# semihkacmaz/CoNFiLD

Measured on AMD Instinct MI355X. Metric: generated fields/sec (256-step sample + CNF decode), Case4 latent, 1/2/4/8 GPU, higher is better.
Workload: dtype f32

## Files before the change

confild_amd/_lib.py:

```python
from __future__ import annotations

import ctypes as C
import os
import threading

_HERE = os.path.dirname(os.path.abspath(__file__))
LIB_PATH = os.path.join(_HERE, "lib", "libconfild_hip.so")
if os.environ.get("CFD_LIB"):
    LIB_PATH = os.path.join(_HERE, "lib", os.path.basename(os.environ["CFD_LIB"]))

_lock = threading.Lock()
_lib = None

c_f32p = C.POINTER(C.c_float)
c_i64p = C.POINTER(C.c_int64)


class CfdError(RuntimeError):
    pass


class UNetCfg(C.Structure):
    _fields_ = [("image_size", C.c_int), ("in_channels", C.c_int), ("model_channels", C.c_int),
                ("out_channels", C.c_int), ("num_res_blocks", C.c_int), ("n_mult", C.c_int),
                ("channel_mult", C.c_int * 8), ("n_attn", C.c_int), ("attention_ds", C.c_int * 8),
                ("num_heads", C.c_int), ("num_head_channels", C.c_int)]


class SirenCfg(C.Structure):
    _fields_ = [("in_coord_features", C.c_int), ("in_latent_features", C.c_int), ("out_features", C.c_int),
                ("num_hidden_layers", C.c_int), ("hidden_features", C.c_int), ("w0", C.c_float)]


_SIGS = {
    "cfd_last_error": (C.c_char_p, []),
    "cfd_version": (C.c_char_p, []),
    "cfd_unet_create": (C.c_int, [C.POINTER(UNetCfg), C.c_int, C.POINTER(C.c_void_p)]),
    "cfd_unet_destroy": (None, [C.c_void_p]),
    "cfd_unet_num_params": (C.c_int, [C.c_void_p, C.POINTER(C.c_int)]),
    "cfd_unet_param_info": (C.c_int, [C.c_void_p, C.c_int, C.POINTER(C.c_char_p), C.POINTER(C.c_int),
                                      C.c_int64 * 4]),
    "cfd_unet_set_param": (C.c_int, [C.c_void_p, C.c_char_p, C.c_void_p, C.c_size_t]),
    "cfd_unet_set_time_freqs": (C.c_int, [C.c_void_p, C.c_void_p, C.c_int]),
    "cfd_unet_ready": (C.c_int, [C.c_void_p]),
    "cfd_unet_load_flat": (C.c_int, [C.c_void_p, C.c_void_p, C.c_size_t, C.c_void_p]),
    "cfd_unet_set_compute": (C.c_int, [C.c_void_p, C.c_int]),
    "cfd_unet_set_plan_batch": (C.c_int, [C.c_void_p, C.c_int]),
    "cfd_device_cu_count": (C.c_int, [C.c_int, C.POINTER(C.c_int)]),
    "cfd_stream_create_cu_range": (C.c_int, [C.c_int, C.c_int, C.c_int, C.POINTER(C.c_void_p)]),
    "cfd_stream_destroy": (C.c_int, [C.c_void_p]),
    "cfd_unet_check_finite": (C.c_int, [C.c_void_p, C.POINTER(C.c_int), C.c_void_p]),
    "cfd_upsample_conv": (C.c_int, [C.c_void_p, C.c_void_p, C.c_void_p, C.c_void_p, C.c_int, C.c_int, C.c_int,
                                    C.c_int, C.c_int, C.c_int, C.c_int, C.POINTER(C.c_int), C.c_void_p]),
    "cfd_unet_workspace_bytes": (C.c_int, [C.c_void_p, C.c_int, C.POINTER(C.c_size_t)]),
    "cfd_unet_forward": (C.c_int, [C.c_void_p, C.c_void_p, C.c_void_p, C.c_void_p, C.c_int, C.c_void_p,
                                   C.c_size_t, C.c_void_p]),
    "cfd_unet_tape_bytes": (C.c_int, [C.c_void_p, C.c_int, C.POINTER(C.c_size_t)]),
    "cfd_unet_vjp_workspace_bytes": (C.c_int, [C.c_void_p, C.c_int, C.POINTER(C.c_size_t)]),
    "cfd_unet_forward_tape": (C.c_int, [C.c_void_p, C.c_void_p, C.c_void_p, C.c_void_p, C.c_int, C.c_void_p,
                                        C.c_size_t, C.c_void_p, C.c_size_t, C.c_void_p]),
    "cfd_unet_input_vjp": (C.c_int, [C.c_void_p, C.c_void_p, C.c_void_p, C.c_int, C.c_void_p, C.c_size_t,
                                     C.c_void_p, C.c_size_t, C.c_void_p]),
    "cfd_unet_set_tape_mode": (C.c_int, [C.c_void_p, C.c_int]),
    "cfd_sched_create": (C.c_int, [C.c_void_p, C.c_int, C.c_int, C.POINTER(C.c_void_p)]),
    "cfd_sched_destroy": (None, [C.c_void_p]),
    "cfd_sched_step": (C.c_int, [C.c_void_p, C.c_int, C.c_int, C.c_void_p, C.c_void_p, C.c_void_p, C.c_void_p,
                                 C.c_uint64, C.c_uint64, C.c_uint64, C.c_void_p, C.c_void_p, C.c_int64, C.c_int,
                                 C.c_void_p]),
    "cfd_sched_step_known": (C.c_int, [C.c_void_p, C.c_int, C.c_int, C.c_void_p, C.c_void_p, C.c_void_p, C.c_void_p,
                                       C.c_uint64, C.c_uint64, C.c_uint64, C.c_void_p, C.c_void_p, C.c_int64,
                                       C.c_int, C.c_void_p, C.c_int64, C.c_void_p, C.c_int64, C.c_void_p,
                                       C.c_void_p, C.c_uint64, C.c_void_p]),
    "cfd_sched_step_jump": (C.c_int, [C.c_void_p, C.c_int, C.c_int, C.c_void_p, C.c_void_p, C.c_void_p, C.c_void_p,
                                      C.c_uint64, C.c_uint64, C.c_uint64, C.c_void_p, C.c_void_p, C.c_int64,
                                      C.c_int, C.c_void_p, C.c_int64, C.c_void_p, C.c_int64, C.c_void_p,
                                      C.c_void_p, C.c_uint64, C.c_float, C.c_float, C.c_void_p, C.c_uint64,
                                      C.c_void_p]),
    "cfd_sampler_set_jumps": (C.c_int, [C.c_void_p, C.c_void_p]),
    "cfd_sampler_set_known": (C.c_int, [C.c_void_p, C.c_void_p, C.c_int64, C.c_void_p, C.c_int64, C.c_void_p,
                                        C.c_void_p]),
    "cfd_sampler_captures": (C.c_int, [C.c_void_p, C.POINTER(C.c_uint64)]),
    "cfd_dps_latent_residual_workspace_bytes": (C.c_int, [C.c_int64, C.c_int, C.POINTER(C.c_size_t)]),
    "cfd_dps_latent_residual": (C.c_int, [C.c_void_p, C.c_int, C.c_void_p, C.c_void_p, C.c_void_p, C.c_void_p,
                                          C.c_int64, C.c_void_p, C.c_int64, C.c_void_p, C.c_void_p, C.c_void_p,
                                          C.c_int64, C.c_int, C.c_void_p, C.c_size_t, C.c_void_p]),
    "cfd_sampler_create": (C.c_int, [C.c_void_p, C.c_void_p, C.c_int, C.c_int, C.c_int, C.c_int64, C.c_int,
                                     C.c_void_p, C.c_void_p, C.c_int, C.c_int, C.POINTER(C.c_void_p)]),
    "cfd_sampler_destroy": (None, [C.c_void_p]),
    "cfd_sampler_run": (C.c_int, [C.c_void_p, C.c_void_p, C.c_void_p, C.c_int, C.c_int, C.c_uint64, C.c_uint64,
                                  C.c_void_p]),
    "cfd_randn": (C.c_int, [C.c_void_p, C.c_int64, C.c_uint64, C.c_uint64, C.c_uint64, C.c_void_p]),
    "cfd_sine_probe": (C.c_int, [C.c_void_p, C.c_void_p, C.c_int64, C.c_int, C.c_void_p]),
    "cfd_latent_denorm": (C.c_int, [C.c_void_p, C.c_void_p, C.c_int64, C.c_void_p, C.c_void_p, C.c_int64,
                                    C.c_void_p]),
    "cfd_dps_residual": (C.c_int, [C.c_void_p, C.c_int64, C.c_void_p, C.c_void_p, C.c_void_p, C.c_int64, C.c_int,
                                   C.c_void_p]),
    "cfd_dps_latent_grad": (C.c_int, [C.c_void_p, C.c_int, C.c_void_p, C.c_void_p, C.c_void_p, C.c_void_p,
                                      C.c_void_p, C.c_void_p, C.c_int64, C.c_void_p, C.c_void_p, C.c_int64, C.c_int,
                                      C.c_void_p]),
    "cfd_dps_update": (C.c_int, [C.c_void_p, C.c_void_p, C.c_void_p, C.c_float, C.c_void_p, C.c_int64,
                                 C.c_void_p]),
    "cfd_dps_update_known": (C.c_int, [C.c_void_p, C.c_void_p, C.c_void_p, C.c_float, C.c_void_p, C.c_void_p,
                                       C.c_int64, C.c_int, C.c_void_p, C.c_int64, C.c_void_p, C.c_int64, C.c_void_p,
                                       C.c_void_p, C.c_uint64, C.c_uint64, C.c_uint64, C.c_void_p]),
    "cfd_siren_create": (C.c_int, [C.POINTER(SirenCfg), C.c_int, C.POINTER(C.c_void_p)]),
    "cfd_siren_destroy": (None, [C.c_void_p]),
    "cfd_siren_num_params": (C.c_int, [C.c_void_p, C.POINTER(C.c_int)]),
    "cfd_siren_param_info": (C.c_int, [C.c_void_p, C.c_int, C.POINTER(C.c_char_p), C.POINTER(C.c_int),
                                       C.c_int64 * 4]),
    "cfd_siren_set_param": (C.c_int, [C.c_void_p, C.c_char_p, C.c_void_p, C.c_size_t]),
    "cfd_siren_ready": (C.c_int, [C.c_void_p]),
    "cfd_siren_workspace_bytes": (C.c_int, [C.c_void_p, C.c_int, C.POINTER(C.c_size_t)]),
    "cfd_siren_set_compute": (C.c_int, [C.c_void_p, C.c_int]),
    "cfd_siren_get_compute": (C.c_int, [C.c_void_p, C.POINTER(C.c_int)]),
    "cfd_siren_forward": (C.c_int, [C.c_void_p, C.c_void_p, C.c_int64, C.c_void_p, C.c_int, C.c_void_p,
                                    C.c_void_p, C.c_void_p, C.c_void_p, C.c_int64, C.c_void_p, C.c_void_p,
                                    C.c_size_t, C.c_void_p]),
    "cfd_siren_jacobian_workspace_bytes": (C.c_int, [C.c_void_p, C.c_int, C.POINTER(C.c_size_t)]),
    "cfd_siren_forward_jacobian": (C.c_int, [C.c_void_p, C.c_void_p, C.c_int64, C.c_void_p, C.c_int, C.c_void_p,
                                             C.c_void_p, C.c_void_p, C.c_void_p, C.c_int64, C.c_void_p, C.c_void_p,
                                             C.c_void_p, C.c_size_t, C.c_void_p]),
    "cfd_siren_forward_jacobian_split": (C.c_int, [C.c_void_p, C.c_void_p, C.c_int64, C.c_void_p, C.c_int,
                                                   C.c_void_p, C.c_void_p, C.c_void_p, C.c_void_p, C.c_int64,
                                                   C.c_void_p, C.c_void_p, C.c_void_p, C.c_size_t, C.c_void_p]),
    "cfd_siren_hessian_workspace_bytes": (C.c_int, [C.c_void_p, C.c_int, C.POINTER(C.c_size_t)]),
    "cfd_siren_forward_hessian": (C.c_int, [C.c_void_p, C.c_void_p, C.c_int64, C.c_void_p, C.c_int, C.c_void_p,
                                            C.c_void_p, C.c_void_p, C.c_void_p, C.c_int64, C.c_void_p, C.c_void_p,
                                            C.c_void_p, C.c_int, C.c_void_p, C.c_size_t, C.c_void_p]),
    "cfd_siren_forward_hessian_split": (C.c_int, [C.c_void_p, C.c_void_p, C.c_int64, C.c_void_p, C.c_int,
                                                  C.c_void_p, C.c_void_p, C.c_void_p, C.c_void_p, C.c_int64,
                                                  C.c_void_p, C.c_void_p, C.c_void_p, C.c_int, C.c_void_p,
                                                  C.c_size_t, C.c_void_p]),
    "cfd_siren_vjp_workspace_bytes": (C.c_int, [C.c_void_p, C.c_int64, C.c_int, C.POINTER(C.c_size_t)]),
    "cfd_siren_tape_forward": (C.c_int, [C.c_void_p, C.c_void_p, C.c_int64, C.c_void_p, C.c_int, C.c_void_p,
                                         C.c_void_p, C.c_void_p, C.c_void_p, C.c_int64, C.c_void_p, C.c_void_p,
                                         C.c_size_t, C.c_void_p]),
    "cfd_siren_tape_vjp": (C.c_int, [C.c_void_p, C.c_void_p, C.c_int64, C.c_int, C.c_void_p, C.c_void_p,
                                     C.c_int64, C.c_void_p, C.c_void_p, C.c_size_t, C.c_void_p]),
    "cfd_siren_jtape_workspace_bytes": (C.c_int, [C.c_void_p, C.c_int64, C.c_int, C.POINTER(C.c_size_t)]),
    "cfd_siren_jtape_forward": (C.c_int, [C.c_void_p, C.c_void_p, C.c_int64, C.c_void_p, C.c_int, C.c_void_p,
                                          C.c_void_p, C.c_void_p, C.c_void_p, C.c_int64, C.c_void_p, C.c_void_p,
                                          C.c_void_p, C.c_size_t, C.c_void_p]),
    "cfd_siren_jtape_vjp": (C.c_int, [C.c_void_p, C.c_void_p, C.c_void_p, C.c_int64, C.c_int, C.c_void_p,
                                      C.c_void_p, C.c_int64, C.c_void_p, C.c_void_p, C.c_size_t, C.c_void_p]),
    "cfd_dps_residual_linear": (C.c_int, [C.c_void_p, C.c_int, C.c_void_p, C.c_void_p, C.c_void_p, C.c_int,
                                          C.c_void_p, C.c_int, C.c_void_p, C.c_void_p, C.c_void_p, C.c_void_p,
                                          C.c_int64, C.c_int, C.c_int, C.c_int, C.c_int, C.c_int, C.c_void_p]),
    "cfd_siren_dense_plan": (C.c_int, [C.POINTER(SirenCfg), C.c_int64, C.c_int, C.c_size_t, C.c_int, C.c_int,
                                       C.POINTER(C.c_size_t), C.POINTER(C.c_int64), C.POINTER(C.c_int)]),
    "cfd_siren_dense_workspace_bytes": (C.c_int, [C.c_void_p, C.c_int64, C.c_int, C.c_size_t,
                                                  C.POINTER(C.c_size_t)]),
    "cfd_siren_dense_grad": (C.c_int, [C.c_void_p, C.c_void_p, C.c_int64, C.c_void_p, C.c_int, C.c_int, C.c_void_p,
                                       C.c_void_p, C.c_void_p, C.c_void_p, C.c_int64, C.c_void_p, C.c_int,
                                       C.c_void_p, C.c_int, C.c_void_p, C.c_void_p, C.c_void_p, C.c_size_t,
                                       C.c_size_t, C.c_void_p]),
    "cfd_siren_dense_set_form": (C.c_int, [C.c_void_p, C.c_int, C.c_int]),
    "cfd_siren_jdense_plan": (C.c_int, [C.POINTER(SirenCfg), C.c_int64, C.c_int, C.c_int, C.c_size_t,
                                        C.POINTER(C.c_size_t), C.POINTER(C.c_int64), C.POINTER(C.c_int)]),
    "cfd_siren_jdense_workspace_bytes": (C.c_int, [C.c_void_p, C.c_int64, C.c_int, C.c_int, C.c_size_t,
                                                   C.POINTER(C.c_size_t)]),
    "cfd_siren_jdense_grad": (C.c_int, [C.c_void_p, C.c_void_p, C.c_int64, C.c_void_p, C.c_int, C.c_int, C.c_void_p,
                                        C.c_void_p, C.c_void_p, C.c_void_p, C.c_int64, C.c_void_p, C.c_int,
                                        C.c_void_p, C.c_int, C.c_int, C.c_void_p, C.c_int, C.c_void_p, C.c_int,
                                        C.c_void_p, C.c_void_p, C.c_void_p, C.c_size_t, C.c_size_t, C.c_void_p]),
    "cfd_siren_train_workspace_bytes": (C.c_int, [C.c_void_p, C.c_int64, C.c_int, C.POINTER(C.c_size_t)]),
    "cfd_siren_train_grad": (C.c_int, [C.c_void_p, C.c_void_p, C.c_int64, C.c_void_p, C.c_void_p, C.c_int,
                                       C.c_void_p, C.c_float, C.c_void_p, C.c_void_p, C.c_void_p, C.c_void_p,
                                       C.c_size_t, C.c_void_p]),
    "cfd_unet_param_grad_workspace_bytes": (C.c_int, [C.c_void_p, C.c_int, C.POINTER(C.c_size_t)]),
    "cfd_unet_param_grad": (C.c_int, [C.c_void_p, C.c_void_p, C.c_void_p, C.c_int, C.c_void_p, C.c_size_t,
                                      C.c_void_p, C.c_void_p, C.c_size_t, C.c_void_p]),
    "cfd_eps_mse": (C.c_int, [C.c_void_p, C.c_void_p, C.c_void_p, C.c_void_p, C.c_int64, C.c_int, C.c_float,
                              C.c_void_p, C.c_void_p]),
    "cfd_ema_update": (C.c_int, [C.c_void_p, C.c_void_p, C.c_int64, C.c_double, C.c_void_p]),
    "cfd_q_sample": (C.c_int, [C.c_void_p, C.c_void_p, C.c_void_p, C.c_void_p, C.c_void_p, C.c_int64, C.c_int,
                               C.c_void_p]),
    "cfd_adam_step": (C.c_int, [C.c_void_p, C.c_void_p, C.c_void_p, C.c_void_p, C.c_int64, C.c_double, C.c_double,
                                C.c_double, C.c_double, C.c_double, C.c_int64, C.c_void_p]),
}

EXPORTS = tuple(_SIGS)


def load(path: str = LIB_PATH):
    global _lib
    with _lock:
        if _lib is not None:
            return _lib
        if not os.path.exists(path):
            raise CfdError(f"{path} is missing: build it with `python -c 'import __graft_entry__ as g; g.build()'` "
                           "(or `make -C confild_amd/csrc`)")
        lib = C.CDLL(path)
        for name, (res, args) in _SIGS.items():
            if os.environ.get("CFD_LIB") and not hasattr(lib, name):
                continue
            fn = getattr(lib, name)
            fn.restype = res
            fn.argtypes = args
        _lib = lib
        return lib


def lib():
    import torch
    if not torch.cuda.is_available():
        raise CfdError("confild_amd needs an AMD GPU (MI355X); no HIP device is visible and there is no CPU path")
# ... 20 lines not shown
```

confild_amd/csrc/conv_x.hip:

```cpp
#include <algorithm>
#include <type_traits>

#include "k1h_lds.hpp"
#include "unet_kernels.hpp"

namespace cfd {

typedef float f16v __attribute__((ext_vector_type(16)));
typedef float f2 __attribute__((ext_vector_type(2)));
typedef _Float16 h2 __attribute__((ext_vector_type(2)));
typedef unsigned u4 __attribute__((ext_vector_type(4)));

__device__ __forceinline__ int xswz(int row, int chunk) { return row * 64 + ((chunk ^ ((row >> 2) & 3)) << 4); }

__device__ __forceinline__ void split4_mix_x(const f4& x, uint2& hi, uint2& lo) {
    hi.x = __builtin_bit_cast(unsigned, __builtin_convertvector((f2){x[0], x[1]}, h2));
    hi.y = __builtin_bit_cast(unsigned, __builtin_convertvector((f2){x[2], x[3]}, h2));
    asm("v_fma_mixlo_f16 %0, %1, 1.0, -%2 op_sel_hi:[0,0,1]" : "=&v"(lo.x) : "v"(x[0]), "v"(hi.x));
    asm("v_fma_mixhi_f16 %0, %1, 1.0, -%2 op_sel:[0,0,1] op_sel_hi:[0,0,1]" : "+v"(lo.x) : "v"(x[1]), "v"(hi.x));
    asm("v_fma_mixlo_f16 %0, %1, 1.0, -%2 op_sel_hi:[0,0,1]" : "=&v"(lo.y) : "v"(x[2]), "v"(hi.y));
    asm("v_fma_mixhi_f16 %0, %1, 1.0, -%2 op_sel:[0,0,1] op_sel_hi:[0,0,1]" : "+v"(lo.y) : "v"(x[3]), "v"(hi.y));
}

__device__ __forceinline__ float phase_scale(const ConvArgs& a, int ph) {
// ... 126 lines not shown
#pragma unroll
        for (int it = 0; it < AIT; ++it) {
            const int off = xswz(a_row[it], kq >> 1) + (kq & 1) * 8;
            uint2 hv, lv;
            split4_mix_x(ra[set][it], hv, lv);
            *(uint2*)(base + off) = hv;
            *(uint2*)(base + ABYTES + off) = lv;
        }
#pragma unroll
        for (int it = 0; it < BIT; ++it) {
            const int off = xswz(b_row[it], kq >> 1) + (kq & 1) * 8;
            *(uint2*)(base + 2 * ABYTES + off) = rbh[set][it];
            *(uint2*)(base + 2 * ABYTES + BBYTES + off) = rbl[set][it];
        }
    };

    f16v acc[TM][TN];
#pragma unroll
    for (int i = 0; i < TM; ++i)
#pragma unroll
        for (int j = 0; j < TN; ++j)
#pragma unroll
            for (int e = 0; e < 16; ++e) acc[i][j][e] = 0.f;

    const int l32 = lane & 31, hsel = lane >> 5;
    const int arow0 = wm * WTM + l32, brow0 = wn * WTN + l32;
    auto kstep = [&](int kt, int cur, int lset, int sset) __attribute__((always_inline)) {
            const bool more = kt + 1 < kt1;
            if (kt + PF < kt1) load_tile(kt + PF, lset);
            const char* base = lds + cur * STAGE;
#pragma unroll
            for (int s = 0; s < 2; ++s) {
                const int ch = 2 * s + hsel;
                h8v fah[TM], fal[TM], fbh[TN], fbl[TN];
#pragma unroll
                for (int i = 0; i < TM; ++i) {
                    const int off = xswz(arow0 + 32 * i, ch);
                    fah[i] = *(const h8v*)(base + off);
                    fal[i] = *(const h8v*)(base + ABYTES + off);
                }
#pragma unroll
                for (int j = 0; j < TN; ++j) {
                    const int off = xswz(brow0 + 32 * j, ch);
                    fbh[j] = *(const h8v*)(base + 2 * ABYTES + off);
                    fbl[j] = *(const h8v*)(base + 2 * ABYTES + BBYTES + off);
                }
#pragma unroll
                for (int i = 0; i < TM; ++i)
#pragma unroll
                    for (int j = 0; j < TN; ++j) {
                        acc[i][j] = __builtin_amdgcn_mfma_f32_32x32x16_f16(fal[i], fbh[j], acc[i][j], 0, 0, 0);
                        acc[i][j] = __builtin_amdgcn_mfma_f32_32x32x16_f16(fah[i], fbl[j], acc[i][j], 0, 0, 0);
                        acc[i][j] = __builtin_amdgcn_mfma_f32_32x32x16_f16(fah[i], fbh[j], acc[i][j], 0, 0, 0);
                    }
            }
            if (more) store_tile(cur ^ 1, sset);
            __syncthreads();
    };
    if (kt0 < kt1) {
        load_tile(kt0, 0);
        if constexpr (PF == 2) {
            if (kt0 + 1 < kt1) load_tile(kt0 + 1, 1);
        }
        store_tile(0, 0);
        __syncthreads();
        CFD_STAMP(a.stamps, 2, a.seq, 2);
        if constexpr (PF == 1) {
            int cur = 0;
            for (int kt = kt0; kt < kt1; ++kt) {
                kstep(kt, cur, 0, 0);
                cur ^= 1;
            }
        } else {
            for (int kt = kt0; kt < kt1; kt += 2) {
                kstep(kt, 0, 0, 1);
                if (kt + 1 < kt1) kstep(kt + 1, 1, 1, 0);
            }
        }
    }

    CFD_STAMP(a.stamps, 2, a.seq, 3);
#pragma unroll
    for (int i = 0; i < TM; ++i)
#pragma unroll
        for (int j = 0; j < TN; ++j) acc[i][j] *= PH ? phase_scale(a, ph) : a.acc_scale;
    const int n_base = n0 + wn * WTN + l32;
    const int m_base = m0 + wm * WTM + 4 * hsel;
    auto orow = [&](int mm, int& bb) __attribute__((always_inline)) {
        bb = mm / HWm;
        if constexpr (!PH) return mm;
        const int rem = mm - bb * HWm, y = rem / Wm, x = rem - y * Wm;
        return (bb * a.Hout + 2 * y + py) * a.Wout + 2 * x + px;
    };
    if (gridDim.z > 1) {
        float* part = a.part + (int64_t)bz * a.M * a.Cout;
#pragma unroll
        for (int i = 0; i < TM; ++i)
#pragma unroll
            for (int e = 0; e < 16; ++e) {
                const int mm = m_base + 32 * i + 8 * (e >> 2) + (e & 3);
                if (mm >= Mm) continue;
                int bb;
                const int m = orow(mm, bb);
#pragma unroll
                for (int j = 0; j < TN; ++j) {
                    const int n = n_base + 32 * j;
                    if (n < a.Cout) part[(int64_t)m * a.Cout + n] = acc[i][j][e];
                }
            }
#ifdef CFD_STAMPS
        __builtin_amdgcn_s_waitcnt(0);
#endif
        CFD_STAMP(a.stamps, 2, a.seq, 4);
        return;
    }
#pragma unroll
    for (int i = 0; i < TM; ++i)
#pragma unroll
        for (int e = 0; e < 16; ++e) {
            const int mm = m_base + 32 * i + 8 * (e >> 2) + (e & 3);
            if (mm >= Mm) continue;
            int bb;
            const int m = orow(mm, bb);
#pragma unroll
            for (int j = 0; j < TN; ++j) {
                const int n = n_base + 32 * j;
                if (n >= a.Cout) continue;
                float v = a.bias ? acc[i][j][e] + a.bias[n] : acc[i][j][e];
                if (a.emb) v = v + a.emb[(int64_t)bb * a.emb_stride + n];
                if (a.res) v = a.res[(int64_t)m * a.Cout + n] + v;
                a.out[(int64_t)m * a.Cout + n] = v;
            }
        }
}

template <int V>
using IC = std::integral_constant<int, V>;

struct Tile3 {
    int x, y, z;
};
__device__ __forceinline__ Tile3 xcd_tile_v(int order) {
    if (!order) return Tile3{(int)blockIdx.x, (int)blockIdx.y, (int)blockIdx.z};
    const unsigned gx = gridDim.x, gy = gridDim.y, gz = gridDim.z;
    const unsigned T = gx * gy * gz, L = blockIdx.x + gx * (blockIdx.y + gy * blockIdx.z);
    const unsigned q = T >> 3, r = T & 7, x = L & 7, sl = L >> 3;
    const unsigned Lp = x < r ? x * (q + 1) + sl : r * (q + 1) + (x - r) * q + sl;
    const bool o2 = order == 2;
    const unsigned d1 = o2 ? gx : gz, d2 = o2 ? gz : gy;
    const unsigned lo = Lp % d1, rest = Lp / d1, mid = rest % d2, hi = rest / d2;
    return o2 ? Tile3{(int)lo, (int)hi, (int)mid} : Tile3{(int)hi, (int)mid, (int)lo};
}

template <int BM, int TW, int BN, bool PH>
__device__ __forceinline__ void conv_h16_body(const ConvArgs& a) {
    constexpr int WGN = BN / 64, WGM = BM / 64, NTG = 64 * WGM * WGN;
    static_assert(BN == 64 || BN == 128, "K1h: 64 or 128 output channels per workgroup");
    static_assert(TW == 16 || TW == 32 || TW == 64, "K1h: a 16-pixel fragment block lies in one tile row");
    constexpr int HWD = TW + 2;
    constexpr int TR = BM / TW, NPX = k1h_npx(BM, TW), NPXD = k1h_npx_staged(BM, TW);
    constexpr int HPLANE = NPX * 64;
    constexpr int HIT = (NPXD * 8 + NTG - 1) / NTG;
    constexpr int NTAP = PH ? 4 : 9, TXN = PH ? 2 : 3;
    constexpr int BPLANE = BN * 64, BSTAGE = 2 * BPLANE;
    constexpr int BIT = BN * 4 / NTG;
    constexpr int GBYTES = 2 * HPLANE + 2 * BSTAGE;
    static_assert(BM % TW == 0 && BIT == 1 && BM % 64 == 0, "tile");
    static_assert(k1h_a_imm(TW, 3, 2) + HPLANE + 3 * 64 + 64 < 65536, "fragment offsets are instruction offsets");
    __shared__ __attribute__((aligned(16))) char lds[GBYTES];

    CFD_STAMP(a.stamps, 3, a.seq, 0);
    const int tid = threadIdx.x, lane = tid & 63;
    const int wave = __builtin_amdgcn_readfirstlane(tid >> 6);
    const int wm = wave / WGN, wn = wave % WGN;
    const int gt = tid;
    char* const halo = lds;
    char* const ring = halo + 2 * HPLANE;
    const Tile3 wg = xcd_tile_v(a.xcd);
    int bx = wg.x;
    const int by = wg.y, bz = wg.z;
    const int ph = PH ? bx & 3 : 0, py = ph >> 1, px = ph & 1;
    if constexpr (PH) bx >>= 2;
    const int n0 = by * BN;
    const int W = PH ? a.Win : a.Wout, Hh = PH ? a.Hin : a.Hout, HWo = Hh * W;
    const int tps = HWo / BM, tpr = W / TW;
    const int bimg = bx / tps, tl = bx - bimg * tps;
    const int y0 = (tl / tpr) * TR, x0 = (tl - (tl / tpr) * tpr) * TW;
    const int64_t mrow0 = PH ? ((int64_t)bimg * a.Hout + 2 * y0 + py) * a.Wout + 2 * x0 + px
                             : (int64_t)bimg * HWo + (int64_t)y0 * W + x0;
    CFD_DASSERT(mrow0 + (int64_t)(PH ? 2 : 1) * ((int64_t)(TR - 1) * a.Wout + TW - 1) < a.M && HWo % BM == 0 &&
                W % TW == 0);

    const int srows = __builtin_amdgcn_readfirstlane(a.Hin * a.Win * (a.M / (a.Hout * a.Wout)));
    const __amdgpu_buffer_rsrc_t rs1 = __builtin_amdgcn_make_buffer_rsrc((void*)a.src1, 0, srows * a.C1 * 4, 0x00020000);
    const __amdgpu_buffer_rsrc_t rs2 = __builtin_amdgcn_make_buffer_rsrc(
        (void*)(a.src2 ? (const void*)a.src2 : (const void*)a.src1), 0, a.src2 ? srows * a.C2 * 4 : 0, 0x00020000);
    const int wbytes = a.Cout * NTAP * a.Ctot * 2;
    const char* const wh0 = PH ? (const char*)a.wph + (int64_t)ph * wbytes : (const char*)a.wbf;
    const char* const wl0 = PH ? (const char*)a.wpl + (int64_t)ph * wbytes : (const char*)a.wlo;
    const __amdgpu_buffer_rsrc_t rwh = __builtin_amdgcn_make_buffer_rsrc((void*)wh0, 0, wbytes, 0x00020000);
    const __amdgpu_buffer_rsrc_t rwl = __builtin_amdgcn_make_buffer_rsrc((void*)wl0, 0, wbytes, 0x00020000);

    const int kq = gt & 7;
    int hpix[HIT], hst[HIT];
#pragma unroll
    for (int it = 0; it < HIT; ++it) {
        const int hp = (gt + it * NTG) >> 3;
        int pix = -1;
        hst[it] = 0;
        if (hp < NPXD) {
            const int hr = hp / HWD, hc = hp - hr * HWD;
            const int iy = y0 - 1 + hr + py, ix = x0 - 1 + hc + px;
            if ((!PH || (hc < TW + 1 && hr < TR + 1)) && iy >= 0 && iy < Hh && ix >= 0 && ix < W)
                pix = a.up && !PH ? (bimg * a.Hin + (iy >> 1)) * a.Win + (ix >> 1) : (bimg * a.Hin + iy) * a.Win + ix;
            hst[it] = k1h_stage_off(TW, hp, kq);
            CFD_DASSERT(hst[it] >= 0 && hst[it] + 8 <= HPLANE);
        }
        CFD_DASSERT(pix < srows);
        hpix[it] = pix;
    }
    const int bq = gt & 3;
    const int nrow = n0 + (gt >> 2);
    const unsigned bvoff = nrow < a.Cout ? (unsigned)((nrow * NTAP * a.Ctot + 8 * bq) * 2) : 0x80000000u;
    const int wst = k1h_wstage_off(gt >> 2, bq);

    const int nch = a.Ctot / 32;
    const int per = (nch + gridDim.z - 1) / gridDim.z;
    const int c0 = bz * per, cend = min(nch, c0 + per);
    const int nrounds = max(cend - c0, 0);

    f4 rh[HIT];
    u4 wx_h, wx_l, wy_h, wy_l;
    auto load_halo = [&](int c) __attribute__((always_inline)) {
        const int cb = 32 * c;
        const bool second = cb >= a.C1;
        const unsigned csrc = 4u * (unsigned)(second ? a.C2 + 0 : a.C1 + 0);
        const unsigned cofs = c < nch ? 4u * ((second ? cb - a.C1 : cb) + 4 * kq) : 0x80000000u;
        if (second) {
#pragma unroll
            for (int it = 0; it < HIT; ++it) {
                const unsigned off = hpix[it] >= 0 ? __umul24((unsigned)hpix[it], csrc) + cofs : 0x80000000u;
                rh[it] = __builtin_bit_cast(f4, __builtin_amdgcn_raw_buffer_load_b128(rs2, off, 0, 0));
            }
        } else {
#pragma unroll
            for (int it = 0; it < HIT; ++it) {
                const unsigned off = hpix[it] >= 0 ? __umul24((unsigned)hpix[it], csrc) + cofs : 0x80000000u;
                rh[it] = __builtin_bit_cast(f4, __builtin_amdgcn_raw_buffer_load_b128(rs1, off, 0, 0));
            }
        }
    };
    auto store_halo = [&]() __attribute__((always_inline)) {
#pragma unroll
        for (int it = 0; it < HIT; ++it) {
            if (gt + it * NTG < NPXD * 8) {
                uint2 hv, lv;
                split4_mix_x(rh[it], hv, lv);
                *(uint2*)(halo + hst[it]) = hv;
                *(uint2*)(halo + HPLANE + hst[it]) = lv;
            }
        }
    };
    auto load_w = [&](int c, int t, u4& rbh, u4& rbl) __attribute__((always_inline)) {
        const int soff = (t * a.Ctot + 32 * min(c, cend - 1)) * 2;
        rbh = __builtin_bit_cast(u4, __builtin_amdgcn_raw_buffer_load_b128(rwh, bvoff, soff, 0));
        rbl = __builtin_bit_cast(u4, __builtin_amdgcn_raw_buffer_load_b128(rwl, bvoff, soff, 0));
    };
    auto store_w = [&](int stage, const u4& rbh, const u4& rbl) __attribute__((always_inline)) {
        char* base = ring + stage * BSTAGE + wst;
        *(u4*)base = rbh;
        *(u4*)(base + BPLANE) = rbl;
    };

    f4 acc[4][4];
#pragma unroll
    for (int i = 0; i < 4; ++i)
#pragma unroll
        for (int j = 0; j < 4; ++j) acc[i][j] = f4{0.f, 0.f, 0.f, 0.f};

    const int li = lane & 15, g = lane >> 4;
    const char* abase[TXN];
#pragma unroll
    for (int tx = 0; tx < TXN; ++tx) abase[tx] = halo + k1h_a_base(TW, wm, li, g, tx);
    const char* const bbase = ring + k1h_b_base(wn, li, g);
    CFD_DASSERT(k1h_a_base(TW, wm, li, g, TXN - 1) + k1h_a_imm(TW, 3, PH ? 1 : 2) + 16 <= HPLANE);

    auto step = [&](int r, auto tc, auto qc, u4& ldh, u4& ldl, const u4& sth, const u4& stl)
        __attribute__((always_inline)) {
        constexpr int T = decltype(tc)::value, Q = decltype(qc)::value;
        constexpr int ty = PH ? T >> 1 : T / 3, tx = PH ? T & 1 : T - 3 * ty;
        const int c = c0 + r;
        load_w(T + 2 < NTAP ? c : c + 1, (T + 2) % NTAP, ldh, ldl);
        if constexpr (T == 0) load_halo(r + 1 < nrounds ? c + 1 : nch);
        const char* const ap = abase[tx];
        const char* const bp = bbase + Q * BSTAGE;
        h8v fbh[4], fbl[4];
#pragma unroll
        for (int j = 0; j < 4; ++j) {
            fbh[j] = *(const h8v*)(bp + k1h_b_imm(j));
            fbl[j] = *(const h8v*)(bp + BPLANE + k1h_b_imm(j));
        }
#pragma unroll
        for (int i = 0; i < 4; ++i) {
            const h8v fah = *(const h8v*)(ap + k1h_a_imm(TW, i, ty));
            const h8v fal = *(const h8v*)(ap + HPLANE + k1h_a_imm(TW, i, ty));
#pragma unroll
            for (int j = 0; j < 4; ++j) acc[i][j] = __builtin_amdgcn_mfma_f32_16x16x32_f16(fal, fbh[j], acc[i][j], 0, 0, 0);
#pragma unroll
            for (int j = 0; j < 4; ++j) acc[i][j] = __builtin_amdgcn_mfma_f32_16x16x32_f16(fah, fbl[j], acc[i][j], 0, 0, 0);
#pragma unroll
            for (int j = 0; j < 4; ++j) acc[i][j] = __builtin_amdgcn_mfma_f32_16x16x32_f16(fah, fbh[j], acc[i][j], 0, 0, 0);
        }
        store_w(Q ^ 1, sth, stl);
        __syncthreads();
        if constexpr (T == NTAP - 1) {
            store_halo();
            __syncthreads();
        }
        __builtin_amdgcn_sched_barrier(0);
    };
    auto round = [&](int r, auto q0c) __attribute__((always_inline)) {
        constexpr int Q0 = decltype(q0c)::value;
        auto tap = [&](auto tc) __attribute__((always_inline)) {
            constexpr int Q = (Q0 + decltype(tc)::value) & 1;
            if constexpr (Q == 0) step(r, tc, IC<0>{}, wx_h, wx_l, wy_h, wy_l);
            else step(r, tc, IC<1>{}, wy_h, wy_l, wx_h, wx_l);
        };
        tap(IC<0>{}), tap(IC<1>{}), tap(IC<2>{}), tap(IC<3>{});
        if constexpr (!PH) tap(IC<4>{}), tap(IC<5>{}), tap(IC<6>{}), tap(IC<7>{}), tap(IC<8>{});
    };

    if (nrounds > 0) {
        load_w(c0, 0, wx_h, wx_l);
        load_w(c0, 1, wy_h, wy_l);
        load_halo(c0);
        store_w(0, wx_h, wx_l);
        store_halo();
        __syncthreads();
        CFD_STAMP(a.stamps, 3, a.seq, 2);
        if constexpr (NTAP & 1) {
            int r = 0;
            for (; r + 2 <= nrounds; r += 2) {
                round(r, IC<0>{});
                round(r + 1, IC<1>{});
            }
            if (r < nrounds) round(r, IC<0>{});
        } else {
            for (int r = 0; r < nrounds; ++r) round(r, IC<0>{});
        }
    }

    CFD_STAMP(a.stamps, 3, a.seq, 3);
    const float scl = PH ? phase_scale(a, ph) : a.acc_scale;
#pragma unroll
    for (int i = 0; i < 4; ++i)
#pragma unroll
        for (int j = 0; j < 4; ++j) acc[i][j] *= scl;
    auto pix_of = [&](int p) __attribute__((always_inline)) {
        if constexpr (PH) return mrow0 + (int64_t)(p / TW) * (2 * a.Wout) + 2 * (p % TW);
        else return mrow0 + (int64_t)(p / TW) * W + (p % TW);
    };
    if (a.ldsepi) {
        static_assert(64 * BN * 4 <= GBYTES, "epilogue stage fits the LDS");
        float* stg = (float*)lds;
        const bool split = gridDim.z > 1;
        float* dstb = split ? a.part + (int64_t)bz * a.M * a.Cout : a.out;
        constexpr int Q = BN / 4;
        __syncthreads();
        for (int r = 0; r < WGM; ++r) {
            if (wm == r) {
#pragma unroll
                for (int i = 0; i < 4; ++i)
#pragma unroll
                    for (int j = 0; j < 4; ++j)
#pragma unroll
                        for (int e = 0; e < 4; ++e)
                            stg[k1h_epi(BN, 16 * i + 4 * g + e, wn * 64 + 16 * j + li)] = acc[i][j][e];
            }
            __syncthreads();
            for (int q = tid; q < 64 * Q; q += NTG) {
                const int p = q / Q, c = (q - p * Q) * 4;
                const int n = n0 + c;
                if (n < a.Cout) {
                    const int64_t m = pix_of(r * 64 + p);
                    f4 v = *(const f4*)(stg + k1h_epi(BN, p, c));
                    if (!split) {
                        if (a.bias) v = v + *(const f4*)(a.bias + n);
                        if (a.emb) v = v + *(const f4*)(a.emb + (int64_t)bimg * a.emb_stride + n);
                        if (a.res) v = *(const f4*)(a.res + m * a.Cout + n) + v;
                    }
                    *(f4*)(dstb + m * a.Cout + n) = v;
                }
            }
            __syncthreads();
        }
#ifdef CFD_STAMPS
        __builtin_amdgcn_s_waitcnt(0);
#endif
        CFD_STAMP(a.stamps, 3, a.seq, 4);
        return;
    }
    const int n_base = n0 + wn * 64 + li;
    const int p_base = wm * 64 + 4 * g;
    if (gridDim.z > 1) {
        float* part = a.part + (int64_t)bz * a.M * a.Cout;
#pragma unroll
        for (int i = 0; i < 4; ++i)
#pragma unroll
            for (int e = 0; e < 4; ++e) {
                const int64_t m = pix_of(p_base + 16 * i + e);
#pragma unroll
                for (int j = 0; j < 4; ++j) {
                    const int n = n_base + 16 * j;
                    if (n < a.Cout) part[m * a.Cout + n] = acc[i][j][e];
                }
            }
#ifdef CFD_STAMPS
        __builtin_amdgcn_s_waitcnt(0);
#endif
        CFD_STAMP(a.stamps, 3, a.seq, 4);
        return;
    }
#pragma unroll
    for (int i = 0; i < 4; ++i)
#pragma unroll
        for (int e = 0; e < 4; ++e) {
            const int64_t m = pix_of(p_base + 16 * i + e);
#pragma unroll
            for (int j = 0; j < 4; ++j) {
                const int n = n_base + 16 * j;
                if (n >= a.Cout) continue;
                float v = a.bias ? acc[i][j][e] + a.bias[n] : acc[i][j][e];
                if (a.emb) v = v + a.emb[(int64_t)bimg * a.emb_stride + n];
                if (a.res) v = a.res[m * a.Cout + n] + v;
                a.out[m * a.Cout + n] = v;
            }
        }
#ifdef CFD_STAMPS
    __builtin_amdgcn_s_waitcnt(0);
#endif
    CFD_STAMP(a.stamps, 3, a.seq, 4);
}

template <int BM, int TW, bool BF = false, bool SB = false, int BN = 128, bool PH = false, int SHAPE = 32>
__global__ __launch_bounds__(BM * (BN / 64), 1) void conv_h_kernel(ConvArgs a) {
    static_assert(SHAPE == 32 || (SHAPE == 16 && !BF && !SB), "K1h: 16x16x32 is the split-f16 form's");
    if constexpr (SHAPE == 16) {
        conv_h16_body<BM, TW, BN, PH>(a);
        return;
    }
    static_assert(!SB || BF, "a bf16 source needs the bf16 kernel");
    static_assert(!PH || !BF, "the phase form is split-f16 only");
    constexpr unsigned SES = SB ? 2u : 4u;
    constexpr int WGN = BN / 64, WGM = BM / 64, NTG = 64 * WGM * WGN;
    static_assert(BN == 64 || BN == 128, "K1h: 64 or 128 output channels per workgroup");
    constexpr int PL = BF ? 1 : 2;
    constexpr int HW2 = TW < 32 ? (TW + 2 + 3) / 4 * 4 : TW + 2;
    constexpr int TR = BM / TW, NPX = (TR + 2) * HW2;
    auto hswz = [](int px, int hr, int chunk) __attribute__((always_inline)) {
        if constexpr (TW == 16) return px * 64 + ((chunk ^ (((px >> 2) + 3 * hr) & 3)) << 4);
        else return xswz(px, chunk);
    };
    constexpr int HPLANE = NPX * 64;
    constexpr int HIT = (NPX * 8 + NTG - 1) / NTG;
    constexpr int NTAP = PH ? 4 : 9;
    constexpr int TG = BF ? 3 : 1, SPR = NTAP / TG;
    constexpr int BPLANE = BN * 64, BSTAGE = PL * BPLANE * TG;
    constexpr int BIT = BN * 4 / NTG;
    constexpr int GBYTES = PL * HPLANE + 2 * BSTAGE;
    static_assert(BM % TW == 0 && BIT >= 1, "tile");
    __shared__ __attribute__((aligned(16))) char lds[GBYTES];

    CFD_STAMP(a.stamps, 3, a.seq, 0);
    const int tid = threadIdx.x, lane = tid & 63;
    const int wave = __builtin_amdgcn_readfirstlane(tid >> 6);
    const int wm = wave / WGN, wn = wave % WGN;
    const int gt = tid;
    char* const halo = lds;
    char* const ring = halo + PL * HPLANE;
    int bx, by, bz;
    xcd_tile(a.xcd, bx, by, bz);
    const int ph = PH ? bx & 3 : 0, py = ph >> 1, px = ph & 1;
    if constexpr (PH) bx >>= 2;
    const int n0 = by * BN;
    const int W = PH ? a.Win : a.Wout, Hh = PH ? a.Hin : a.Hout, HWo = Hh * W;
    const int tps = HWo / BM, tpr = W / TW;
    const int bimg = bx / tps, tl = bx - bimg * tps;
    const int y0 = (tl / tpr) * TR, x0 = (tl - (tl / tpr) * tpr) * TW;
    const int64_t mrow0 = PH ? ((int64_t)bimg * a.Hout + 2 * y0 + py) * a.Wout + 2 * x0 + px
                             : (int64_t)bimg * HWo + (int64_t)y0 * W + x0;
    CFD_DASSERT(mrow0 + (int64_t)(PH ? 2 : 1) * ((int64_t)(TR - 1) * a.Wout + TW - 1) < a.M && HWo % BM == 0 &&
                W % TW == 0);

    const int srows = __builtin_amdgcn_readfirstlane(a.Hin * a.Win * (a.M / (a.Hout * a.Wout)));
    const __amdgpu_buffer_rsrc_t rs1 = __builtin_amdgcn_make_buffer_rsrc((void*)a.src1, 0, srows * a.C1 * SES, 0x00020000);
    const __amdgpu_buffer_rsrc_t rs2 = __builtin_amdgcn_make_buffer_rsrc(
        (void*)(a.src2 ? (const void*)a.src2 : (const void*)a.src1), 0, a.src2 ? srows * a.C2 * SES : 0, 0x00020000);
    const int wbytes = a.Cout * NTAP * a.Ctot * 2;
    const char* const wh0 = PH ? (const char*)a.wph + (int64_t)ph * wbytes : (const char*)a.wbf;
    const char* const wl0 = PH ? (const char*)a.wpl + (int64_t)ph * wbytes : (const char*)a.wlo;
    const __amdgpu_buffer_rsrc_t rwh = __builtin_amdgcn_make_buffer_rsrc((void*)wh0, 0, wbytes, 0x00020000);
    const __amdgpu_buffer_rsrc_t rwl = __builtin_amdgcn_make_buffer_rsrc((void*)wl0, 0, wbytes, 0x00020000);

    const int kq = gt & 7;
    int hpix[HIT];
#pragma unroll
    for (int it = 0; it < HIT; ++it) {
        const int hp = (gt + it * NTG) >> 3;
        int pix = -1;
        if (hp < NPX) {
            const int hr = hp / HW2, hc = hp - hr * HW2;
            const int iy = y0 - 1 + hr + py, ix = x0 - 1 + hc + px;
            if (hc < TW + (PH ? 1 : 2) && (!PH || hr < TR + 1) && iy >= 0 && iy < Hh && ix >= 0 && ix < W)
                pix = a.up && !PH ? (bimg * a.Hin + (iy >> 1)) * a.Win + (ix >> 1) : (bimg * a.Hin + iy) * a.Win + ix;
        }
        CFD_DASSERT(pix < srows);
        hpix[it] = pix;
    }
    const int bq = gt & 3;
    unsigned bvoff[BIT];
#pragma unroll
    for (int it = 0; it < BIT; ++it) {
        const int n = n0 + (gt >> 2) + it * (NTG / 4);
        bvoff[it] = n < a.Cout ? (unsigned)((n * NTAP * a.Ctot + 8 * bq) * 2) : 0x80000000u;
    }

    const int nch = a.Ctot / 32;
    const int per = (nch + gridDim.z - 1) / gridDim.z;
    const int c0 = bz * per, cend = min(nch, c0 + per);
    const int nrounds = max(cend - c0, 0);
    auto chunk_of = [&](int r) __attribute__((always_inline)) { return c0 + r; };

    typedef typename std::conditional<SB, uint2, f4>::type HT;
    HT rh[HIT];
    constexpr int BW = BIT * TG;
    u4 wx_h[BW], wx_l[BW], wy_h[BW], wy_l[BW];
    auto load_halo = [&](int c) __attribute__((always_inline)) {
        const int cb = 32 * c;
        const bool second = cb >= a.C1;
        const unsigned csrc = SES * (unsigned)(second ? a.C2 + 0 : a.C1 + 0);
        const unsigned cofs = SES * ((second ? cb - a.C1 : cb) + 4 * kq);
        if (second) {
#pragma unroll
            for (int it = 0; it < HIT; ++it) {
                const unsigned off = hpix[it] >= 0 ? __umul24((unsigned)hpix[it], csrc) + cofs : 0x80000000u;
                if constexpr (SB)
                    rh[it] = __builtin_bit_cast(uint2, __builtin_amdgcn_raw_buffer_load_b64(rs2, off, 0, 0));
// ... 28 lines not shown
                    *(uint2*)(halo + HPLANE + off) = lv;
                }
            }
        }
    };
    auto load_w = [&](int s, u4 (&rbh)[BW], u4 (&rbl)[BW]) __attribute__((always_inline)) {
        const int r = s / SPR, c = chunk_of(r);
        if (c >= cend) return;
#pragma unroll
        for (int u = 0; u < TG; ++u) {
            const int soff = (((s - SPR * r) * TG + u) * a.Ctot + 32 * c) * 2;
#pragma unroll
            for (int it = 0; it < BIT; ++it) {
                rbh[u * BIT + it] = __builtin_bit_cast(u4, __builtin_amdgcn_raw_buffer_load_b128(rwh, bvoff[it], soff, 0));
                if constexpr (!BF)
                    rbl[u * BIT + it] = __builtin_bit_cast(u4, __builtin_amdgcn_raw_buffer_load_b128(rwl, bvoff[it], soff, 0));
            }
        }
    };
    auto store_w = [&](int stage, const u4 (&rbh)[BW], const u4 (&rbl)[BW]) __attribute__((always_inline)) {
#pragma unroll
        for (int u = 0; u < TG; ++u) {
            char* base = ring + stage * BSTAGE + u * PL * BPLANE;
#pragma unroll
            for (int it = 0; it < BIT; ++it) {
                const int off = xswz((gt >> 2) + it * (NTG / 4), bq);
                *(u4*)(base + off) = rbh[u * BIT + it];
                if constexpr (!BF) *(u4*)(base + BPLANE + off) = rbl[u * BIT + it];
            }
        }
    };

    f16v acc[2][2];
#pragma unroll
    for (int i = 0; i < 2; ++i)
#pragma unroll
        for (int j = 0; j < 2; ++j)
#pragma unroll
            for (int e = 0; e < 16; ++e) acc[i][j][e] = 0.f;

    const int l32 = lane & 31, hsel = lane >> 5;
    int hb[2], hrb[2];
#pragma unroll
    for (int i = 0; i < 2; ++i) {
        const int p = wm * 64 + 32 * i + l32;
        hb[i] = (p / TW) * HW2 + (p % TW);
        hrb[i] = p / TW;
    }
    const int brow0 = wn * 64 + l32;
    const int nsteps = nrounds * SPR;

    auto step = [&](int s, u4 (&ldh)[BW], u4 (&ldl)[BW], const u4 (&sth)[BW], const u4 (&stl)[BW])
        __attribute__((always_inline)) {
        const int r = s / SPR, t = s - SPR * r;
        const int c = chunk_of(r);
        if (s + 2 < nsteps) load_w(s + 2, ldh, ldl);
        if (t == 0 && chunk_of(r + 1) < cend) load_halo(chunk_of(r + 1));
        if (c < cend) {
            const char* wb = ring + (s & 1) * BSTAGE;
            if constexpr (BF) {
                const int ty = t;
#pragma unroll
                for (int u = 0; u < TG; ++u) {
                    const int tofs = ty * HW2 + u;
                    const char* wbu = wb + u * BPLANE;
#pragma unroll
                    for (int s2 = 0; s2 < 2; ++s2) {
                        const int ch = 2 * s2 + hsel;
                        bf16x8 fa[2], fb[2];
#pragma unroll
                        for (int i = 0; i < 2; ++i) fa[i] = *(const bf16x8*)(halo + hswz(hb[i] + tofs, hrb[i] + ty, ch));
#pragma unroll
                        for (int jj = 0; jj < 2; ++jj) fb[jj] = *(const bf16x8*)(wbu + xswz(brow0 + 32 * jj, ch));
#pragma unroll
                        for (int i = 0; i < 2; ++i)
#pragma unroll
                            for (int jj = 0; jj < 2; ++jj)
                                acc[i][jj] = __builtin_amdgcn_mfma_f32_32x32x16_bf16(fa[i], fb[jj], acc[i][jj], 0, 0, 0);
                    }
                }
            } else {
            const int ty = PH ? t >> 1 : t / 3;
            const int tofs = ty * HW2 + (PH ? t & 1 : t - 3 * ty);
#pragma unroll
            for (int s2 = 0; s2 < 2; ++s2) {
                const int ch = 2 * s2 + hsel;
                h8v fah[2], fal[2], fbh[2], fbl[2];
#pragma unroll
                for (int i = 0; i < 2; ++i) {
                    CFD_DASSERT(hb[i] + tofs < NPX);
                    const int off = hswz(hb[i] + tofs, hrb[i] + ty, ch);
                    fah[i] = *(const h8v*)(halo + off);
                    fal[i] = *(const h8v*)(halo + HPLANE + off);
                }
#pragma unroll
                for (int jj = 0; jj < 2; ++jj) {
                    const int off = xswz(brow0 + 32 * jj, ch);
                    fbh[jj] = *(const h8v*)(wb + off);
                    fbl[jj] = *(const h8v*)(wb + BPLANE + off);
                }
#pragma unroll
                for (int i = 0; i < 2; ++i)
#pragma unroll
                    for (int jj = 0; jj < 2; ++jj) {
                        acc[i][jj] = __builtin_amdgcn_mfma_f32_32x32x16_f16(fal[i], fbh[jj], acc[i][jj], 0, 0, 0);
                        acc[i][jj] = __builtin_amdgcn_mfma_f32_32x32x16_f16(fah[i], fbl[jj], acc[i][jj], 0, 0, 0);
                        acc[i][jj] = __builtin_amdgcn_mfma_f32_32x32x16_f16(fah[i], fbh[jj], acc[i][jj], 0, 0, 0);
                    }
            }
            }
        }
        if (s + 1 < nsteps && chunk_of((s + 1) / SPR) < cend) store_w((s + 1) & 1, sth, stl);
        __syncthreads();
        if (t == SPR - 1 && s + 1 < nsteps) {
            if (chunk_of(r + 1) < cend) store_halo();
            __syncthreads();
        }
    };

    if (nsteps > 0) {
        load_w(0, wx_h, wx_l);
        if (nsteps > 1) load_w(1, wy_h, wy_l);
        load_halo(chunk_of(0));
        store_w(0, wx_h, wx_l);
        store_halo();
        __syncthreads();
        CFD_STAMP(a.stamps, 3, a.seq, 2);
        for (int s = 0; s < nsteps; s += 2) {
            step(s, wx_h, wx_l, wy_h, wy_l);
            if (s + 1 < nsteps) step(s + 1, wy_h, wy_l, wx_h, wx_l);
        }
    }

    CFD_STAMP(a.stamps, 3, a.seq, 3);
    if constexpr (!BF) {
#pragma unroll
        for (int i = 0; i < 2; ++i)
#pragma unroll
            for (int j = 0; j < 2; ++j) acc[i][j] *= PH ? phase_scale(a, ph) : a.acc_scale;
    }
    const int n_base = n0 + wn * 64 + l32;
    const int p_base = wm * 64 + 4 * hsel;
    auto pix_of = [&](int p) __attribute__((always_inline)) {
        if constexpr (PH) return mrow0 + (int64_t)(p / TW) * (2 * a.Wout) + 2 * (p % TW);
        else return mrow0 + (int64_t)(p / TW) * W + (p % TW);
    };
    {
        if (a.ldsepi) {
            static_assert(64 * BN * 4 <= (int)sizeof(lds), "epilogue stage fits the LDS");
            float* stg = (float*)lds;
            const bool split = gridDim.z > 1;
            float* dstb = split ? a.part + (int64_t)bz * a.M * a.Cout : a.out;
            constexpr int Q = BN / 4;
            __syncthreads();
            for (int r = 0; r < WGM; ++r) {
                if (wm == r) {
#pragma unroll
                    for (int i = 0; i < 2; ++i)
#pragma unroll
                        for (int e = 0; e < 16; ++e)
#pragma unroll
                            for (int j = 0; j < 2; ++j)
                                stg[(32 * i + 8 * (e >> 2) + (e & 3) + 4 * hsel) * BN + wn * 64 + 32 * j + l32] =
                                    acc[i][j][e];
                }
                __syncthreads();
                for (int q = tid; q < 64 * Q; q += NTG) {
                    const int p = q / Q, c = (q - p * Q) * 4;
                    const int n = n0 + c;
                    if (n < a.Cout) {
                        const int64_t m = pix_of(r * 64 + p);
                        f4 v = *(const f4*)(stg + p * BN + c);
                        if (!split) {
                            if (a.bias) v = v + *(const f4*)(a.bias + n);
                            if (a.emb) v = v + *(const f4*)(a.emb + (int64_t)bimg * a.emb_stride + n);
                            if (a.res) v = *(const f4*)(a.res + m * a.Cout + n) + v;
                        }
                        *(f4*)(dstb + m * a.Cout + n) = v;
                    }
                }
                __syncthreads();
            }
#ifdef CFD_STAMPS
            __builtin_amdgcn_s_waitcnt(0);
#endif
            CFD_STAMP(a.stamps, 3, a.seq, 4);
            return;
        }
    }
    if (gridDim.z > 1) {
        float* part = a.part + (int64_t)bz * a.M * a.Cout;
#pragma unroll
        for (int i = 0; i < 2; ++i)
#pragma unroll
            for (int e = 0; e < 16; ++e) {
                const int64_t m = pix_of(p_base + 32 * i + 8 * (e >> 2) + (e & 3));
#pragma unroll
                for (int j = 0; j < 2; ++j) {
                    const int n = n_base + 32 * j;
                    if (n < a.Cout) part[(int64_t)m * a.Cout + n] = acc[i][j][e];
                }
            }
#ifdef CFD_STAMPS
        __builtin_amdgcn_s_waitcnt(0);
#endif
        CFD_STAMP(a.stamps, 3, a.seq, 4);
        return;
    }
#pragma unroll
    for (int i = 0; i < 2; ++i)
#pragma unroll
        for (int e = 0; e < 16; ++e) {
            const int64_t m = pix_of(p_base + 32 * i + 8 * (e >> 2) + (e & 3));
#pragma unroll
            for (int j = 0; j < 2; ++j) {
                const int n = n_base + 32 * j;
                if (n >= a.Cout) continue;
                float v = a.bias ? acc[i][j][e] + a.bias[n] : acc[i][j][e];
                if (a.emb) v = v + a.emb[(int64_t)bimg * a.emb_stride + n];
                if (a.res) v = a.res[(int64_t)m * a.Cout + n] + v;
                a.out[(int64_t)m * a.Cout + n] = v;
            }
        }
#ifdef CFD_STAMPS
    __builtin_amdgcn_s_waitcnt(0);
#endif
    CFD_STAMP(a.stamps, 3, a.seq, 4);
}

int conv_h_tw(const ConvArgs& a) {
    const bool geo = !a.tmode && a.ks == 3 && a.stride == 1 && a.pad == 1 && a.C1 % 32 == 0 && a.C2 % 32 == 0 &&
                     (a.up ? a.Hout == 2 * a.Hin && a.Wout == 2 * a.Win : a.Hout == a.Hin && a.Wout == a.Win) &&
                     a.M % (a.Hout * a.Wout) == 0;
    if (!geo) return 0;
    for (int tw = 64; tw >= 16; tw >>= 1)
        if (a.Wout % tw == 0 && a.Hout % (256 / tw) == 0) return tw;
    return 0;
}

int conv_hp_tw(const ConvArgs& a) {
    const bool geo = !a.tmode && a.up && a.ks == 3 && a.stride == 1 && a.pad == 1 && a.C1 % 32 == 0 &&
                     a.C2 % 32 == 0 && a.Hout == 2 * a.Hin && a.Wout == 2 * a.Win && a.M % (a.Hout * a.Wout) == 0;
    if (!geo) return 0;
    for (int tw = 64; tw >= 16; tw >>= 1)
        if (a.Win % tw == 0 && a.Hin % (256 / tw) == 0) return tw;
    return 0;
}

int k1h_shape(int tw, int bn, bool phase, bool adjoint) {
    (void)tw, (void)bn, (void)phase;
#ifdef CFD_K1H_MFMA32
    (void)adjoint;
    return 32;
#else
    return adjoint ? 32 : 16;
#endif
}

template <int BN, bool PH, int SHAPE>
static void launch_h_(const ConvArgs& a, int tw, dim3 g, hipStream_t st) {
    const dim3 blk(256 * (BN / 64));
    if (tw == 64) hipLaunchKernelGGL((conv_h_kernel<256, 64, false, false, BN, PH, SHAPE>), g, blk, 0, st, a);
    else if (tw == 32) hipLaunchKernelGGL((conv_h_kernel<256, 32, false, false, BN, PH, SHAPE>), g, blk, 0, st, a);
    else hipLaunchKernelGGL((conv_h_kernel<256, 16, false, false, BN, PH, SHAPE>), g, blk, 0, st, a);
}
template <int BN, bool PH>
static void launch_h(const ConvArgs& a, int tw, int shape, dim3 g, hipStream_t st) {
    if (shape == 16) launch_h_<BN, PH, 16>(a, tw, g, st);
    else launch_h_<BN, PH, 32>(a, tw, g, st);
}

int launch_conv_x(const ConvArgs& a, int variant, int splits, hipStream_t st, bool adjoint) {
    CFD_REQUIRE(a.wbf && !a.tmode, CFD_ESTATE, "conv_x: split-f16 or bf16 forward only");
    CFD_REQUIRE(a.Ctot % 32 == 0 && a.C1 % 4 == 0 && a.C2 % 4 == 0, CFD_ESHAPE, "conv_x needs channels % 32 == 0");
    CFD_REQUIRE(splits == 1 || a.part, CFD_ESTATE, "split-K needs a partial buffer");
    {
        const int64_t srows = (int64_t)a.Hin * a.Win * (a.M / (a.Hout * a.Wout));
        CFD_REQUIRE(srows < (1 << 24) && srows * std::max(a.C1, a.C2) * 4 < (1ll << 31) &&
                        (int64_t)a.Cout * a.K * 2 < (1ll << 31) && a.ks * a.ks <= 9,
                    CFD_ESHAPE, "conv_x: operands beyond 2 GiB");
    }
    auto grid = [&](int bm, int bn) __attribute__((always_inline)) {
        return dim3((unsigned)ceil_div(a.M, bm), (unsigned)ceil_div(a.Cout, bn), splits);
    };
    if (variant == 22) {
        const int tw = conv_h_tw(a);
        CFD_REQUIRE(tw > 0 && !a.wlo, CFD_ESHAPE, "conv_h bf16: 3x3 stride-1 with a 16/32/64-divisible width");
        const dim3 g = grid(256, 128);
        if (a.src_bf16) {
            if (tw == 64) hipLaunchKernelGGL((conv_h_kernel<256, 64, true, true>), g, dim3(512), 0, st, a);
            else if (tw == 32) hipLaunchKernelGGL((conv_h_kernel<256, 32, true, true>), g, dim3(512), 0, st, a);
            else hipLaunchKernelGGL((conv_h_kernel<256, 16, true, true>), g, dim3(512), 0, st, a);
        } else {
            if (tw == 64) hipLaunchKernelGGL((conv_h_kernel<256, 64, true>), g, dim3(512), 0, st, a);
            else if (tw == 32) hipLaunchKernelGGL((conv_h_kernel<256, 32, true>), g, dim3(512), 0, st, a);
            else hipLaunchKernelGGL((conv_h_kernel<256, 16, true>), g, dim3(512), 0, st, a);
        }
        check_launch("conv_h_kernel");
        return splits;
    }
    CFD_REQUIRE(!a.src_bf16, CFD_ESTATE, "internal: a bf16 convolution source needs the K1hb kernel");
    if (variant == 20 || variant == 32 || variant == 33) {
        const int tw = conv_h_tw(a);
        CFD_REQUIRE(tw > 0 && a.wlo, CFD_ESHAPE, "conv_h: split-f16 3x3 stride-1 with a 16/32/64-divisible width");
        static const int smalln = smalln_below();
        const dim3 g = grid(256, 128);
        const bool n64 = (int64_t)g.x * g.y * g.z < smalln && a.Cout % 64 == 0;
        const int shape = variant == 20 ? k1h_shape(tw, n64 ? 64 : 128, false, adjoint) : variant == 32 ? 32 : 16;
        if (n64) {
            launch_h<64, false>(a, tw, shape, grid(256, 64), st);
            check_launch("conv_h_kernel");
            return splits;
        }
        launch_h<128, false>(a, tw, shape, g, st);
        check_launch("conv_h_kernel");
        return splits;
    }
    CFD_REQUIRE(a.wlo, CFD_ESTATE, "internal: K1x runs split-f16 operands only");
    if ((variant >= 24 && variant <= 26) || variant == 34 || variant == 35) {
        CFD_REQUIRE(a.wph && a.wpl && a.up && a.ks == 3 && a.stride == 1 && a.pad == 1 && a.Hout == 2 * a.Hin &&
                        a.Wout == 2 * a.Win,
                    CFD_ESTATE, "internal: the phase form needs an Upsample convolution and its phase packs");
        if (variant == 24 || variant == 34 || variant == 35) {
            const int tw = conv_hp_tw(a);
            CFD_REQUIRE(tw > 0, CFD_ESHAPE, "conv_h phase form: a 16/32/64-divisible low-resolution width");
            const dim3 g = grid(256, 128);
            launch_h<128, true>(a, tw, variant == 24 ? k1h_shape(tw, 128, true, adjoint) : variant == 34 ? 32 : 16, g, st);
            check_launch("conv_h_kernel (phase)");
            return splits;
        }
        const int bm = variant == 26 ? 256 : 128;
        const dim3 g(4u * (unsigned)ceil_div(a.M / 4, bm), (unsigned)ceil_div(a.Cout, 128), splits);
        if (variant == 26) hipLaunchKernelGGL((conv_x_kernel<256, 128, 4, 2, 1, true>), g, dim3(512), 0, st, a);
        else hipLaunchKernelGGL((conv_x_kernel<128, 128, 2, 2, 1, true>), g, dim3(256), 0, st, a);
        check_launch("conv_x_kernel (phase)");
        return splits;
    }
    switch (variant) {
        case 1: hipLaunchKernelGGL((conv_x_kernel<128, 128, 2, 2>), grid(128, 128), dim3(256), 0, st, a); break;
        case 2: hipLaunchKernelGGL((conv_x_kernel<256, 128, 4, 2>), grid(256, 128), dim3(512), 0, st, a); break;
        default: CFD_REQUIRE(false, CFD_EARG, "conv_x variant");
    }
    check_launch("conv_x_kernel");
    return splits;
}

}
```

confild_amd/csrc/unet.hip:

```cpp
#include <algorithm>
#include <cstring>
#include <cmath>
#include <functional>
#include <map>
#include <string>
#include <vector>

#include "sampler.hpp"
#include "unet_kernels.hpp"
#include "unet_train.hpp"

namespace cfd {

enum class Pack { Raw, Conv3, Conv1, EmbW, EmbB };

struct UParam {
    std::string key;
    std::vector<int64_t> shape;
    Pack pack = Pack::Raw;
    size_t offset = 0;
    size_t count = 0;
    int emb_row = 0;
    bool set = false;
    int tpack = 0;
// ... 130 lines not shown
    const auto& c = h->cfg;
    const int mc = c.model_channels;
    h->tdim = 4 * mc;
    add_param(h, "time_embed.0.weight", {h->tdim, mc}, Pack::Raw);
    add_param(h, "time_embed.0.bias", {h->tdim}, Pack::Raw);
    add_param(h, "time_embed.2.weight", {h->tdim, h->tdim}, Pack::Raw);
    add_param(h, "time_embed.2.bias", {h->tdim}, Pack::Raw);
    int ch = c.channel_mult[0] * mc;
    add_conv(h, "input_blocks.0.0", c.in_channels, ch, 3);
    h->steps.push_back({cfd::Step::In, 0, "input_blocks.0.0", c.in_channels, ch});
    h->steps.push_back({cfd::Step::Push});
    std::vector<int> chans{ch};
    int ds = 1, idx = 1;
    for (int level = 0; level < c.n_mult; ++level) {
        for (int r = 0; r < c.num_res_blocks; ++r) {
            const int cout = c.channel_mult[level] * mc;
            const std::string pre = "input_blocks." + std::to_string(idx);
            int ri = add_res(h, pre + ".0", ch, cout);
            h->steps.push_back({cfd::Step::Res, ri});
            ch = cout;
            if (has_attn(h, ds)) h->steps.push_back({cfd::Step::Attn, add_attn(h, pre + ".1", ch)});
            h->steps.push_back({cfd::Step::Push});
            chans.push_back(ch);
            ++idx;
        }
        if (level != c.n_mult - 1) {
            const std::string pre = "input_blocks." + std::to_string(idx) + ".0.op";
            add_conv(h, pre, ch, ch, 3);
            h->steps.push_back({cfd::Step::Down, 0, pre, ch, ch});
            h->steps.push_back({cfd::Step::Push});
            chans.push_back(ch);
            ds *= 2;
            ++idx;
        }
    }
    h->steps.push_back({cfd::Step::Res, add_res(h, "middle_block.0", ch, ch)});
    h->steps.push_back({cfd::Step::Attn, add_attn(h, "middle_block.1", ch)});
    h->steps.push_back({cfd::Step::Res, add_res(h, "middle_block.2", ch, ch)});
    idx = 0;
    for (int level = c.n_mult - 1; level >= 0; --level) {
        for (int i = 0; i < c.num_res_blocks + 1; ++i) {
            const int ich = chans.back();
            chans.pop_back();
            const int cout = mc * c.channel_mult[level];
            const std::string pre = "output_blocks." + std::to_string(idx);
            h->steps.push_back({cfd::Step::Cat});
            h->steps.push_back({cfd::Step::Res, add_res(h, pre + ".0", ch + ich, cout)});
            ch = cout;
            int j = 1;
            if (has_attn(h, ds)) {
                h->steps.push_back({cfd::Step::Attn, add_attn(h, pre + ".1", ch)});
                j = 2;
            }
            if (level && i == c.num_res_blocks) {
                const std::string up = pre + "." + std::to_string(j) + ".conv";
                add_conv(h, up, ch, ch, 3, false, true);
                h->steps.push_back({cfd::Step::Up, 0, up, ch, ch});
                ds /= 2;
            }
            ++idx;
        }
    }
    add_norm(h, "out.0", ch);
    add_conv(h, "out.2", c.channel_mult[0] * mc, c.out_channels, 3);
    h->steps.push_back({cfd::Step::Out, 0, "out", ch, c.out_channels});
    size_t off = 0;
    for (auto& p : h->params) {
        if (p.pack == Pack::EmbW || p.pack == Pack::EmbB) continue;
        p.offset = off;
        off += (p.count + 3) & ~size_t(3);
    }
    h->arena_floats = off;
    size_t toff = 0;
    for (auto& p : h->params) {
        if (!p.tpack) continue;
        p.toffset = toff;
        toff += ((p.tpack == 2 ? p.count / 9 * 16 : p.count) + 3) & ~size_t(3);
    }
    h->arena_t_floats = toff;
    size_t poff = 0;
    for (auto& p : h->params) {
        if (p.tpack != 2 || p.shape[0] < cfd::kPhaseMinCout) continue;
        p.phase = true;
        p.poffset = poff;
        poff += (p.count / 9 * 16 + 7) & ~size_t(7);
    }
    h->arena_p_elems = poff;
}

const void* PB(const cfd_unet* h, const std::string& key) {
    if (h->compute == CFD_COMPUTE_F32) return nullptr;
    auto it = h->index.find(key);
    CFD_REQUIRE(it != h->index.end(), CFD_EKEY, "internal: missing param " + key);
    return (h->compute == CFD_COMPUTE_BF16 ? h->arena_bf : h->arena_hi) + h->params[it->second].offset;
}

const void* PL(const cfd_unet* h, const std::string& key, float* inv) {
    *inv = 1.f;
    if (h->compute != CFD_COMPUTE_SPLIT_F16) return nullptr;
    auto it = h->index.find(key);
    CFD_REQUIRE(it != h->index.end(), CFD_EKEY, "internal: missing param " + key);
    *inv = h->params[it->second].split_inv;
    return h->arena_lo + h->params[it->second].offset;
}

uint16_t to_bf16(float f) {
    uint32_t u;
    std::memcpy(&u, &f, 4);
    if ((u & 0x7fffffffu) > 0x7f800000u) return (uint16_t)((u >> 16) | 0x40u);
    return (uint16_t)((u + 0x7fffu + ((u >> 16) & 1u)) >> 16);
}

void PTS(const cfd_unet* h, const std::string& key, cfd::ConvArgs* a) {
    if (h->compute != CFD_COMPUTE_SPLIT_F16) return;
    auto it = h->index.find(key);
    CFD_REQUIRE(it != h->index.end() && h->params[it->second].tpack, CFD_EKEY, "internal: missing conv " + key);
    const auto& p = h->params[it->second];
    a->wbf = h->arena_thi + p.toffset;
    a->wlo = h->arena_tlo + p.toffset;
    a->acc_scale = p.tsplit_inv;
}

void PP(const cfd_unet* h, const std::string& key, cfd::ConvArgs* a) {
    if (h->compute != CFD_COMPUTE_SPLIT_F16) return;
    auto it = h->index.find(key);
    CFD_REQUIRE(it != h->index.end(), CFD_EKEY, "internal: missing param " + key);
    const auto& p = h->params[it->second];
    if (!p.phase) return;
    a->wph = h->arena_phi + p.poffset;
    a->wpl = h->arena_plo + p.poffset;
    for (int ph = 0; ph < 4; ++ph) a->ph_scale[ph] = p.psplit_inv[ph];
}

const float* PT(const cfd_unet* h, const std::string& key) {
    auto it = h->index.find(key);
    CFD_REQUIRE(it != h->index.end() && h->params[it->second].tpack, CFD_EKEY, "internal: missing conv " + key);
    return h->arena_t + h->params[it->second].toffset;
}

const float* P(const cfd_unet* h, const std::string& key) {
    auto it = h->index.find(key);
    CFD_REQUIRE(it != h->index.end(), CFD_EKEY, "internal: missing param " + key);
    return h->arena + h->params[it->second].offset;
}

struct Act {
    const float* a = nullptr;
    int Ca = 0;
    const float* b = nullptr;
    int Cb = 0;
    int H = 0, W = 0;
    int C() const { return Ca + Cb; }
    bool bf16 = false;
};

struct Workspace {
    char* base;
    size_t off = 0;
    bool dry;
    float* take(size_t nfloats) {
        off = (off + 255) & ~size_t(255);
        float* p = dry ? nullptr : (float*)(base + off);
        off += nfloats * sizeof(float);
        return p;
    }
};

struct Rec {
    Act in;
    const float* h1 = nullptr;
    float *ss1 = nullptr, *st1 = nullptr;
    float *ss2 = nullptr, *st2 = nullptr;
    float *qkv = nullptr, *o = nullptr, *lse = nullptr;
    const float *act1 = nullptr, *act2 = nullptr;
    unsigned *amx1 = nullptr, *amx2 = nullptr;
    int skip_hs = -1;
    int push_hs = -1;
};

struct Tape {
    Workspace* tws;
    std::vector<Rec>* recs;
    bool keep_gnout = false;
    float* temb = nullptr;
    float* th1 = nullptr;
    float* emb = nullptr;
};

struct Sizes {
    size_t max_act = 0, max_qkv = 0, max_cat = 0, max_att = 0;
    size_t max_kvf = 0;
    size_t max_abw = 0;
    size_t max_apart = 0;
    std::vector<size_t> hs;
};

int plan_batch(const cfd_unet* h);

Sizes sizes(const cfd_unet* h) {
    const auto& c = h->cfg;
    const int mc = c.model_channels, S = c.image_size;
    Sizes z;
    int ch = c.channel_mult[0] * mc, hw = S, cmax = 0;
    z.max_act = (size_t)hw * hw * ch;
    z.hs.push_back((size_t)hw * hw * ch);
    for (int l = 0; l < c.n_mult; ++l) cmax = std::max(cmax, c.channel_mult[l] * mc);
    for (int l = 0; l < c.n_mult; ++l) {
        const int co = c.channel_mult[l] * mc;
        z.max_act = std::max(z.max_act, (size_t)hw * hw * std::max(co, ch));
        z.max_qkv = std::max(z.max_qkv, (size_t)hw * hw * 3 * co);
        z.max_cat = std::max(z.max_cat, (size_t)hw * hw * (co + cmax));
        z.max_att = std::max(z.max_att, (size_t)hw * hw * co);
        z.max_kvf = std::max(z.max_kvf, cfd::attention_split_floats(hw * hw, co));
        if (has_attn(h, 1 << l) || l == c.n_mult - 1) {
            z.max_abw = std::max(z.max_abw, cfd::attention_bwd_split_floats(hw * hw, co));
            const int heads = c.num_head_channels == -1 ? c.num_heads : co / c.num_head_channels;
            z.max_apart = std::max(z.max_apart, cfd::attention_part_floats(hw * hw, co, co / heads, plan_batch(h)));
        }
        for (int r = 0; r < c.num_res_blocks; ++r) z.hs.push_back((size_t)hw * hw * co);
        ch = co;
        if (l != c.n_mult - 1) {
            hw /= 2;
            z.hs.push_back((size_t)hw * hw * ch);
        }
    }
    z.max_cat = std::max(z.max_cat, z.max_act);
    return z;
}

constexpr size_t kSplitPer8 = size_t(16) << 20;
int plan_batch(const cfd_unet* h) { return h->plan_b > 0 ? h->plan_b : 8; }
size_t split_cap(const cfd_unet* h, int B) {
    const int pb = plan_batch(h);
    return kSplitPer8 * (size_t)std::max(1, (B + pb - 1) / pb);
}

cfd::ConvPlan plan_checked(const cfd_unet* h, const cfd::ConvArgs& a0, size_t slab_floats) {
    cfd::ConvArgs a = a0;
    a.plan_b = plan_batch(h);
    const cfd::ConvPlan p = cfd::plan_conv(a, kSplitPer8);
    CFD_REQUIRE(p.splits == 1 || (size_t)p.splits * a.M * a.Cout <= slab_floats, CFD_ESTATE,
                "internal: split-K slab too small");
    return p;
}

void run(const cfd_unet* h, const float* x, const int64_t* t, float* eps, int B, Workspace& ws, hipStream_t st,
         Tape* tape = nullptr, bool launch_req = true) {
    const auto& c = h->cfg;
    const int mc = c.model_channels, S = c.image_size;
    const Sizes z = sizes(h);
    const bool launch = launch_req && !ws.dry && !(tape && tape->tws->dry);
    const size_t kSplitCap = split_cap(h, B);
    float* temb = tape ? tape->tws->take((size_t)B * mc) : ws.take((size_t)B * mc);
    float* h1 = tape ? tape->tws->take((size_t)B * h->tdim) : ws.take((size_t)B * h->tdim);
    float* emb = tape ? tape->tws->take((size_t)B * h->tdim) : ws.take((size_t)B * h->tdim);
    if (tape) {
        tape->temb = temb;
        tape->th1 = h1;
        tape->emb = emb;
    }
    float* embo = ws.take((size_t)B * h->emb_total);
    double* gnpart = (double*)ws.take((size_t)B * cfd::kGnMaxChunks * 32 * 2 * 2);
    float* gnss = ws.take((size_t)B * 1024 * 2);
    float* nbuf = ws.take((size_t)B * z.max_cat);
    float* splitk = ws.take(kSplitCap);
    float* kvws = ws.take((size_t)B * z.max_kvf);
    float* apart = z.max_apart ? ws.take((size_t)B * z.max_apart) : nullptr;
    float* pool[3];
    for (auto& p : pool) p = ws.take((size_t)B * z.max_act);
    float* tmp = ws.take((size_t)B * z.max_act);
    float* skipb = ws.take((size_t)B * z.max_act);
    float* qkv = tape ? nullptr : ws.take((size_t)B * z.max_qkv);
    float* abuf = tape ? nullptr : ws.take((size_t)B * z.max_act);
    std::vector<float*> hsbuf;
    for (size_t n : z.hs) hsbuf.push_back(tape ? tape->tws->take((size_t)B * n) : ws.take((size_t)B * n));
    constexpr int kGnSlots = 256;
    unsigned* gslots = tape ? (unsigned*)tape->tws->take(kGnSlots) : nullptr;
    int ngs = 0;
    if (ws.dry && !tape) return;
    auto keep = [&](size_t nfloats) -> float* { return tape->tws->take(nfloats); };
    if (tape && tape->keep_gnout && launch) CFD_HIP(hipMemsetAsync(gslots, 0, sizeof(unsigned) * kGnSlots, st));
    std::vector<Rec>* recs = tape ? tape->recs : nullptr;
    if (recs) recs->assign(h->steps.size(), Rec{});

    auto pick = [&](const float* busy1, const float* busy2) -> float* {
        if (!launch && (ws.dry || !busy1)) return pool[0];
        for (auto p : pool)
            if (p != busy1 && p != busy2) return p;
        throw cfd::Error{CFD_ESTATE, "internal: buffer pool exhausted"};
    };

    if (launch) {
        cfd::launch_temb(t, h->freqs, temb, mc, B, st);
        cfd::launch_linear(temb, P(h, "time_embed.0.weight"), P(h, "time_embed.0.bias"), h1, B, mc, h->tdim, 0, st);
        cfd::launch_linear(h1, P(h, "time_embed.2.weight"), P(h, "time_embed.2.bias"), emb, B, h->tdim, h->tdim, 1,
                           st);
        cfd::launch_linear(emb, h->emb_w, h->emb_b, embo, B, h->tdim, h->emb_total, 1, st);
    }

    struct Pending {
        cfd::ConvArgs a{};
        int splits = 0;
    } pend;
    auto flush = [&]() {
        if (pend.splits > 1 && launch) cfd::launch_splitk_reduce(pend.a, pend.splits, st);
        pend.splits = 0;
    };

    auto gn = [&](const Act& in, const std::string& pre, int silu, float** ss, float** stats,
                  bool keep_raw = true, bool bf16_out = false, const float** actp = nullptr,
                  unsigned** amxp = nullptr) -> Act {
        cfd::GnArgs g{};
        g.src1 = in.a;
        g.src2 = in.b;
        g.gamma = P(h, pre + ".weight");
        g.beta = P(h, pre + ".bias");
        g.part = gnpart;
        g.ss = gnss;
        if (tape) {
            *ss = g.ss = keep((size_t)B * in.C() * 2);
            *stats = g.stats = keep((size_t)B * 64);
        }
        g.out = nbuf;
        if (tape && actp && tape->keep_gnout) {
            CFD_REQUIRE(!bf16_out && ngs < kGnSlots, CFD_ESTATE, "internal: kept GroupNorm output");
            g.out = keep((size_t)B * in.H * in.W * in.C());
            g.amax_out = gslots + ngs++;
            *actp = g.out;
            *amxp = g.amax_out;
        }
        g.C1 = in.Ca;
        g.C2 = in.Cb;
        g.Ctot = in.C();
        g.HW = in.H * in.W;
        g.eps = 1e-5f;
        g.plan_b = plan_batch(h);
        g.silu = silu;
        if (pend.splits > 1 && pend.a.out == in.a && pend.a.Cout == in.Ca && cfd::gn_takes_splitk(g, B)) {
            g.kpart = pend.a.part;
            g.ksplits = pend.splits;
            g.kbias = pend.a.bias;
            g.kemb = pend.a.emb;
            g.kemb_stride = pend.a.emb_stride;
            g.kres = pend.a.res;
            g.kx = keep_raw || cfd::gn2_applies(g) ? pend.a.out : nullptr;
            pend.splits = 0;
        } else {
            flush();
        }
        static const int gn_log = getenv("CFD_CONV_LOG") ? atoi(getenv("CFD_CONV_LOG")) : 0;
        if (gn_log && launch)
            fprintf(stderr, "GN %s %dx%d C=%d+%d ksplits=%d kres=%d kx=%d silu=%d\n", pre.c_str(), in.H, in.W, g.C1,
                    g.C2, g.kpart ? g.ksplits : 0, g.kres ? 1 : 0, g.kx ? 1 : 0, silu);
        g.out_bf16 = bf16_out ? 1 : 0;
        if (launch) cfd::launch_gn(g, B, st);
        Act r{g.out, in.C(), nullptr, 0, in.H, in.W};
        r.bf16 = bf16_out;
        return r;
    };
    auto conv_args = [&](const Act& in, const std::string& pre, int cout, int ks, int stride, int up,
                         const float* embp, const float* resp, float* out) {
        cfd::ConvArgs a{};
        a.src1 = in.a;
        a.src2 = in.b;
        a.C1 = in.Ca;
        a.C2 = in.Cb;
        a.Ctot = in.C();
        a.w = P(h, pre + ".weight");
        a.wbf = PB(h, pre + ".weight");
        a.wlo = PL(h, pre + ".weight", &a.acc_scale);
        if (up) PP(h, pre + ".weight", &a);
        a.bias = P(h, pre + ".bias");
        a.emb = embp;
        a.emb_stride = h->emb_total;
        a.res = resp;
        a.out = out;
        a.part = splitk;
        a.Hin = in.H;
        a.Win = in.W;
        a.Hout = up ? in.H * 2 : (stride == 2 ? (in.H + 1) / 2 : in.H);
        a.Wout = up ? in.W * 2 : (stride == 2 ? (in.W + 1) / 2 : in.W);
        a.stride = stride;
        a.ks = ks;
        a.pad = ks == 3 ? 1 : 0;
        a.up = up;
        a.Cout = cout;
        a.M = B * a.Hout * a.Wout;
        a.K = ks * ks * a.Ctot;
        a.src_bf16 = in.bf16 ? 1 : 0;
        return a;
    };
    static const int gn_bf16out = getenv("CFD_GN_BF16OUT") ? atoi(getenv("CFD_GN_BF16OUT")) : 1;
    auto feeds_k1hb = [&](const Act& in, const std::string& pre, int cout) -> bool {
        if (!gn_bf16out || h->compute != CFD_COMPUTE_BF16) return false;
        Act n{nbuf, in.C(), nullptr, 0, in.H, in.W};
        const cfd::ConvArgs a = conv_args(n, pre, cout, 3, 1, 0, nullptr, nullptr, nullptr);
        return a.wbf && !a.wlo && cfd::conv_runs_k1hb(a, plan_checked(h, a, kSplitCap));
    };
    using Tweak = std::function<void(cfd::ConvArgs&, const cfd::ConvPlan&)>;
    auto conv = [&](const Act& in, const std::string& pre, int cout, int ks, int stride, int up,
                    const float* embp, const float* resp, float* out, const Tweak& tweak = {}) {
        cfd::ConvArgs a = conv_args(in, pre, cout, ks, stride, up, embp, resp, out);
        flush();
        const cfd::ConvPlan plan = plan_checked(h, a, kSplitCap);
        if (tweak) tweak(a, plan);
        CFD_REQUIRE(!a.src_bf16 || cfd::conv_runs_k1hb(a, plan), CFD_ESTATE,
                    "internal: bf16 GroupNorm output feeds a convolution other than K1hb at " + pre);
        static const int conv_log = getenv("CFD_CONV_LOG") ? atoi(getenv("CFD_CONV_LOG")) : 0;
        if (conv_log && launch)
            fprintf(stderr, "CONV %s %dx%d C=%d+%d->%d ks=%d s=%d up=%d M=%d kx=%d bm=%d bn=%d nw=%d splits=%d\n",
                    pre.c_str(), a.Hin, a.Win, a.C1, a.C2, a.Cout, a.ks, a.stride, a.up, a.M, plan.kx, plan.bm,
                    plan.bn, plan.nw, plan.splits);
        if (launch) {
            const int sp = cfd::launch_conv(a, plan, st, true);
            if (sp > 1) {
                pend.a = a;
                pend.splits = sp;
            }
        }
    };

    std::vector<std::pair<Act, int>> stack;
    Act cur;
    size_t hs_i = 0;
    int pending_skip = -1;
    for (size_t si = 0; si < h->steps.size(); ++si) {
        const auto& s = h->steps[si];
        Rec rec;
        rec.in = cur;
        const bool to_skip = si + 1 < h->steps.size() && h->steps[si + 1].kind == cfd::Step::Push;
        auto dest = [&](const float* busy1, const float* busy2, size_t nfl) -> float* {
            if (to_skip) return hsbuf[hs_i];
            return tape ? keep(nfl) : pick(busy1, busy2);
        };
        switch (s.kind) {
            case cfd::Step::In: {
                cfd::ConvArgs a{};
                a.src1 = x;
                a.C1 = c.in_channels;
                a.Ctot = c.in_channels;
                a.w = P(h, s.conv + ".weight");
                a.bias = P(h, s.conv + ".bias");
                a.out = hsbuf[0];
                a.Hin = a.Hout = S;
                a.Win = a.Wout = S;
                a.Cout = s.cout;
                a.M = B * S * S;
                if (launch) cfd::launch_conv_in(a, st);
                cur = Act{hsbuf[0], s.cout, nullptr, 0, S, S};
                break;
            }
            case cfd::Step::Push: {
                float* dst = hsbuf[hs_i];
                if (cur.a != dst) {
                    flush();
                    if (launch)
                        CFD_HIP(hipMemcpyAsync(dst, cur.a, sizeof(float) * (size_t)B * cur.H * cur.W * cur.Ca,
                                               hipMemcpyDeviceToDevice, st));
                    cur.a = dst;
                }
                rec.push_hs = (int)hs_i;
                stack.push_back({cur, (int)hs_i});
                ++hs_i;
                break;
            }
            case cfd::Step::Cat: {
                const auto skip = stack.back();
                stack.pop_back();
                CFD_REQUIRE(cur.b == nullptr && skip.first.H == cur.H, CFD_ESTATE, "internal: concat shape");
                cur.b = skip.first.a;
                cur.Cb = skip.first.Ca;
                pending_skip = skip.second;
                break;
            }
            case cfd::Step::Res: {
                const auto& r = h->res[s.idx];
                CFD_REQUIRE(cur.C() == r.cin, CFD_ESTATE, "internal: ResBlock input channels at " + r.pre);
                rec.skip_hs = pending_skip;
                pending_skip = -1;
                const size_t nout = (size_t)B * cur.H * cur.W * r.cout;
                const Act xin = gn(cur, r.pre + ".in_layers.0", 1, &rec.ss1, &rec.st1, true,
                                   feeds_k1hb(cur, r.pre + ".in_layers.2", r.cout), &rec.act1, &rec.amx1);
                const float* resp = nullptr;
                if (r.cin != r.cout) {
                    resp = skipb;
                } else {
                    CFD_REQUIRE(cur.b == nullptr, CFD_ESTATE, "identity skip on a concatenated input");
                    resp = cur.a;
                }
                float* hb = tape ? keep(nout) : tmp;
                conv(xin, r.pre + ".in_layers.2", r.cout, 3, 1, 0, embo + r.emb_off, nullptr, hb);
                rec.h1 = hb;
                const Act th{hb, r.cout, nullptr, 0, cur.H, cur.W};
                const Act hn = gn(th, r.pre + ".out_layers.0", 1, &rec.ss2, &rec.st2, tape != nullptr,
                                  feeds_k1hb(th, r.pre + ".out_layers.3", r.cout), &rec.act2, &rec.amx2);
                float* out = dest(cur.a, cur.b, nout);
                if (r.cin != r.cout)
                    conv(cur, r.pre + ".skip_connection", r.cout, 1, 1, 0, nullptr, nullptr, skipb);
                conv(hn, r.pre + ".out_layers.3", r.cout, 3, 1, 0, nullptr, resp, out);
                cur = Act{out, r.cout, nullptr, 0, cur.H, cur.W};
                break;
            }
            case cfd::Step::Attn: {
                const auto& at = h->attn[s.idx];
                const int T = cur.H * cur.W;
                const Act xn = gn(cur, at.pre + ".norm", 0, &rec.ss1, &rec.st1, true, false, &rec.act1, &rec.amx1);
                float* qb = tape ? keep((size_t)B * T * 3 * at.C) : qkv;
                float* ob = tape ? keep((size_t)B * T * at.C) : abuf;
                const float attn_scale = (float)(1.0 / std::sqrt(std::sqrt((double)at.ch)));
                const bool split_attn = h->compute != CFD_COMPUTE_F32 && (at.ch == 32 || at.ch == 64 || at.ch == 128);
                bool kv_packed = false;
                conv(xn, at.pre + ".qkv", 3 * at.C, 1, 1, 0, nullptr, nullptr, qb,
                     [&](cfd::ConvArgs& a, const cfd::ConvPlan& plan) {
                         if (!split_attn || h->compute == CFD_COMPUTE_F32 || !cfd::conv_kv_pack_ok(a, plan, T))
                             return;
                         a.kvf = kvws;
                         a.kv_voff = cfd::attention_split_voff(T, at.ch, at.heads, B);
                         a.kv_ch = at.ch;
                         a.kv_heads = at.heads;
                         a.kv_T = T;
                         a.kv_scale = attn_scale;
                         kv_packed = true;
                     });
                cfd::AttnArgs aa{qb, ob, T, at.C, attn_scale, nullptr};
                aa.part = apart;
                if (tape) aa.lse = keep((size_t)B * at.heads * T);
                rec.qkv = qb;
                rec.o = ob;
                rec.lse = aa.lse;
                flush();
                if (launch) {
                    if (split_attn)
                        cfd::launch_attention_split(aa, at.ch, at.heads, B, plan_batch(h), kvws, st, kv_packed);
                    else
                        cfd::launch_attention(aa, at.ch, at.heads, B, st);
                }
                float* out = dest(cur.a, nullptr, (size_t)B * T * at.C);
                conv(Act{ob, at.C, nullptr, 0, cur.H, cur.W}, at.pre + ".proj_out", at.C, 1, 1, 0, nullptr, cur.a,
                     out);
                cur = Act{out, at.C, nullptr, 0, cur.H, cur.W};
                break;
            }
            case cfd::Step::Down: {
                const int Ho = (cur.H + 1) / 2, Wo = (cur.W + 1) / 2;
                float* out = dest(cur.a, nullptr, (size_t)B * Ho * Wo * s.cout);
                conv(cur, s.conv, s.cout, 3, 2, 0, nullptr, nullptr, out);
                cur = Act{out, s.cout, nullptr, 0, Ho, Wo};
                break;
            }
            case cfd::Step::Up: {
                float* out = tape ? keep((size_t)B * 4 * cur.H * cur.W * s.cout) : pick(cur.a, nullptr);
                conv(cur, s.conv, s.cout, 3, 1, 1, nullptr, nullptr, out);
                cur = Act{out, s.cout, nullptr, 0, cur.H * 2, cur.W * 2};
                break;
            }
            case cfd::Step::Out: {
                const Act on = gn(cur, "out.0", 1, &rec.ss1, &rec.st1, true, false, &rec.act1, &rec.amx1);
                cfd::ConvArgs a{};
                a.src1 = on.a;
                a.C1 = on.Ca;
                a.Ctot = on.Ca;
                a.w = P(h, "out.2.weight");
                a.bias = P(h, "out.2.bias");
                a.out = eps;
                a.Hin = a.Hout = cur.H;
                a.Win = a.Wout = cur.W;
                a.Cout = c.out_channels;
                a.M = B * cur.H * cur.W;
                a.K = 9 * cur.Ca;
                a.nonfinite = h->nonfinite;
                flush();
                if (launch) cfd::launch_conv_out(a, st);
                break;
            }
        }
        if (recs) (*recs)[si] = rec;
    }
    flush();
}


struct ParamGrad {
    float* grad = nullptr;
    const float* x = nullptr;
    const float *temb = nullptr, *th1 = nullptr, *emb = nullptr;
};

constexpr int kRangeSlots = 1024;

void run_vjp(const cfd_unet* h, const float* d_eps, float* d_x, int B, const std::vector<Rec>& recs, Workspace& ws,
             hipStream_t st, const ParamGrad* pg = nullptr, bool pg_ws = false) {
    const auto& c = h->cfg;
    const int S = c.image_size;
    const Sizes z = sizes(h);
    const size_t kSplitCap = split_cap(h, B);
    float* splitk = ws.take(kSplitCap);
    double* gnpart = (double*)ws.take((size_t)B * cfd::kGnMaxChunks * 32 * 2 * 2);
    float* gnfin = ws.take((size_t)B * 64);
    float* gpool[4];
    for (auto& p : gpool) p = ws.take((size_t)B * z.max_cat);
    float* dqkv = ws.take((size_t)B * z.max_qkv);
    float* dd = ws.take((size_t)B * z.max_att);
    float* abws = ws.take((size_t)B * z.max_abw);
    std::vector<float*> dhs;
    for (size_t n : z.hs) dhs.push_back(ws.take((size_t)B * n));
    float *wpart = nullptr, *cpart = nullptr, *crow = nullptr, *demb = nullptr, *dth1 = nullptr, *gpp = nullptr;
    float* wact = nullptr;
    unsigned* wamax = nullptr;
    float* wbpart = nullptr;
    size_t wcap = 0, ccap = 0, bcap = 0;
    if (pg_ws) {
        int cmax = 0;
        for (int l = 0; l < c.n_mult; ++l) cmax = std::max(cmax, c.channel_mult[l] * c.model_channels);
        wcap = (size_t)16 * 3 * cmax * 2 * cmax * 9;
        ccap = (size_t)(256 + B) * std::max(3 * cmax, h->tdim);
        wpart = ws.take(wcap);
        cpart = ws.take(ccap);
        wact = ws.take((size_t)B * z.max_cat);
        crow = ws.take((size_t)B * std::max(3 * cmax, h->tdim));
        demb = ws.take((size_t)B * h->tdim);
        dth1 = ws.take((size_t)B * h->tdim);
        gpp = ws.take((size_t)B * cfd::kGnMaxChunks * 2 * cmax * 2);
        wamax = (unsigned*)ws.take(kRangeSlots);
        bcap = (size_t)64 * 3 * cmax;
        wbpart = ws.take(bcap);
    }
    if (ws.dry) return;
    for (size_t si = 0; si < h->steps.size(); ++si)
        CFD_REQUIRE(h->steps[si].kind != cfd::Step::Attn || (recs[si].in.H * recs[si].in.W) % 16 == 0, CFD_ESHAPE,
                    "attention backward needs T % 16 == 0");
    std::vector<size_t> goff;
    {
        size_t o = 0;
        for (const auto& p : h->params) {
            goff.push_back(o);
            o += p.count;
        }
    }
    auto GP = [&](const std::string& key) -> float* {
        auto it = h->index.find(key);
        CFD_REQUIRE(it != h->index.end(), CFD_EKEY, "internal: no parameter " + key);
        return pg->grad + goff[it->second];
    };
    int nslot = 0;
    const bool split_w = pg && h->compute == CFD_COMPUTE_SPLIT_F16;
    auto slot = [&]() -> unsigned* {
        if (!split_w) return nullptr;
        CFD_REQUIRE(nslot < kRangeSlots, CFD_ESTATE, "internal: range slots exhausted");
        return wamax + nslot++;
    };
    auto wgrad = [&](const float* dy, int cout, const Act& X, const float* ss, int silu, int Hout, int Wout, int ks,
                     int stride, int pad, int up, const std::string& pre, unsigned* ymax = nullptr,
                     unsigned* xmax = nullptr) -> unsigned* {
        CFD_REQUIRE(pg_ws && cfd::colsum_part_floats((int64_t)B * Hout * Wout, cout, 1) <= ccap &&
                        (size_t)cout * X.C() * ks * ks <= wcap && (size_t)X.H * X.W * X.C() <= z.max_cat,
                    CFD_ESTATE, "internal: weight-gradient scratch");
        cfd::WgradArgs a{};
        a.part_cap = (int64_t)wcap;
        a.act = wact;
        a.dy = dy;
        a.src1 = X.a;
        a.src2 = X.b;
        a.C1 = X.Ca;
        a.C2 = X.Cb;
        a.Ctot = X.C();
        a.ss = ss;
        a.silu = silu;
        a.part = wpart;
        if (split_w) {
            a.xmax_known = xmax ? 1 : 0;
            a.amax_x = xmax ? xmax : slot();
            a.ymax_known = ymax ? 1 : 0;
            a.amax_y = ymax ? ymax : slot();
        }
        a.P = (int64_t)B * Hout * Wout;
        a.Cout = cout;
        a.Hin = X.H;
        a.Win = X.W;
        a.Hout = Hout;
        a.Wout = Wout;
        a.ks = ks;
        a.stride = stride;
        a.pad = pad;
        a.up = up;
        a.bpart = wbpart;
        a.bpart_cap = (int64_t)bcap;
        a.Gb = GP(pre + ".bias");
        if (!cfd::launch_conv_wgrad(a, GP(pre + ".weight"), st)) {
            cfd::launch_colsum(dy, a.P, cout, 1, cpart, crow, st);
            cfd::launch_rows_accum(crow, 1, cout, GP(pre + ".bias"), st);
        }
        return a.amax_y;
    };
    if (pg) CFD_HIP(hipMemsetAsync(demb, 0, sizeof(float) * B * h->tdim, st));
    if (split_w) CFD_HIP(hipMemsetAsync(wamax, 0, sizeof(unsigned) * kRangeSlots, st));

    auto gfree = [&](const float* b1, const float* b2 = nullptr, const float* b3 = nullptr) -> float* {
        for (auto p : gpool)
            if (p != b1 && p != b2 && p != b3) return p;
        throw cfd::Error{CFD_ESTATE, "internal: gradient pool exhausted"};
    };
    auto dconv = [&](const float* dy, int cin, int Hin, int Win, const std::string& key, int cout, int Hout, int Wout,
                     int ks, int stride, int pad, int tmode, float* out) {
        {
            auto it = h->index.find(key);
            CFD_REQUIRE(it != h->index.end(), CFD_EKEY, "internal: missing conv " + key);
// ... 686 lines not shown
            CFD_HIP(hipMalloc(&h->rp_part, sizeof(float) * 2 * blocks));
            size_t nup = 0;
            for (const auto& p : h->params) nup += p.phase ? 1 : 0;
            CFD_HIP(hipMalloc(&h->rp_amax, sizeof(float) * (2 * np + 4 * nup)));
            CFD_HIP(hipMemcpy(h->rp_desc, desc.data(), sizeof(cfd::RepackDesc) * np, hipMemcpyHostToDevice));
            CFD_HIP(hipMemcpy(h->rp_first, first.data(), sizeof(int64_t) * (np + 1), hipMemcpyHostToDevice));
            h->rp_blocks = blocks;
        }
        const auto* desc = (const cfd::RepackDesc*)h->rp_desc;
        hipLaunchKernelGGL(cfd::rp_amax_kernel, dim3((unsigned)h->rp_blocks), dim3(256), 0, st, flat, desc,
                           h->rp_first, np, h->rp_part);
        cfd::check_launch("rp_amax_kernel");
        hipLaunchKernelGGL(cfd::rp_reduce_kernel, dim3(np), dim3(256), 0, st, h->rp_part, h->rp_first, h->rp_amax);
        cfd::check_launch("rp_reduce_kernel");
        hipLaunchKernelGGL(cfd::rp_pack_kernel, dim3((unsigned)h->rp_blocks), dim3(256), 0, st, flat, desc,
                           h->rp_first, np, h->rp_amax, h->arena, h->arena_bf, (_Float16*)h->arena_hi,
                           (_Float16*)h->arena_lo, h->arena_t, (_Float16*)h->arena_thi, (_Float16*)h->arena_tlo,
                           h->emb_w, h->emb_b, h->tdim);
        cfd::check_launch("rp_pack_kernel");
        if (h->rp_tiles) {
            hipLaunchKernelGGL(cfd::rp_tpack_kernel, dim3((unsigned)h->rp_tiles), dim3(256), 0, st, flat, desc,
                               h->rp_tfirst, np, h->rp_amax, h->arena_t, (_Float16*)h->arena_thi,
                               (_Float16*)h->arena_tlo);
            cfd::check_launch("rp_tpack_kernel");
        }
        std::vector<int> ups;
        for (int k = 0; k < np; ++k)
            if (h->params[k].phase) ups.push_back(k);
        unsigned* pamax = (unsigned*)(h->rp_amax + 2 * (size_t)np);
        if (!ups.empty()) CFD_HIP(hipMemsetAsync(pamax, 0, sizeof(unsigned) * 4 * ups.size(), st));
        {
            int64_t src = 0;
            size_t u = 0;
            for (int k = 0; k < np; ++k) {
                const auto& p = h->params[k];
                if (p.phase) {
                    const int64_t ci = p.shape[1], np4 = (int64_t)p.count / 9 * 4;
                    const dim3 g((unsigned)std::min<int64_t>(1024, cfd::ceil_div(np4, 256)), 4);
                    hipLaunchKernelGGL(cfd::rp_phase_amax_kernel, g, dim3(256), 0, st, flat + src, ci, np4,
                                       pamax + 4 * u);
                    cfd::check_launch("rp_phase_amax_kernel");
                    hipLaunchKernelGGL(cfd::rp_phase_pack_kernel, g, dim3(256), 0, st, flat + src, ci, np4,
                                       pamax + 4 * u, (_Float16*)h->arena_phi + p.poffset,
                                       (_Float16*)h->arena_plo + p.poffset);
                    cfd::check_launch("rp_phase_pack_kernel");
                    ++u;
                }
                src += (int64_t)p.count;
            }
        }
        std::vector<float> amax(2 * (size_t)np + 4 * ups.size());
        CFD_HIP(hipMemcpyAsync(amax.data(), h->rp_amax, sizeof(float) * amax.size(), hipMemcpyDeviceToHost, st));
        CFD_HIP(hipStreamSynchronize(st));
        for (size_t u = 0; u < ups.size(); ++u)
            for (int ph = 0; ph < 4; ++ph) {
                const float am = amax[2 * (size_t)np + 4 * u + ph];
                int ex = 0;
                if (am > 0.f) std::frexp(am, &ex);
                h->params[ups[u]].psplit_inv[ph] = std::ldexp(1.0f, ex);
            }
        for (int k = 0; k < np; ++k) {
            auto& p = h->params[k];
            if (p.pack == Pack::Conv1 || p.pack == Pack::Conv3) {
                int ex = 0;
                if (amax[2 * k] > 0.f) std::frexp(amax[2 * k], &ex);
                p.split_inv = std::ldexp(1.0f, ex);
            }
            if (p.tpack) {
                int ex = 0;
                if (amax[2 * k + 1] > 0.f) std::frexp(amax[2 * k + 1], &ex);
                p.tsplit_inv = std::ldexp(1.0f, ex);
            }
            p.set = true;
        }
        ++h->version;
    });
}

extern "C" int cfd_upsample_conv(const float* x, const float* w_host, const float* bias_host, float* out, int B,
                                 int H, int W, int Cin, int Cout, int plan_b, int device, int* kx, void* stream) {
    return cfd::guard([&] {
        CFD_REQUIRE(x && w_host && bias_host && out, CFD_EARG, "null argument");
        CFD_REQUIRE(B > 0 && H > 0 && W > 0 && Cin > 0 && Cin % 32 == 0 && Cout > 0 && Cout % 4 == 0 && plan_b >= 0 &&
                        plan_b <= 64,
                    CFD_ESHAPE, "upsample conv: Cin % 32 == 0, Cout % 4 == 0, plan batch 0 .. 64");
        cfd::DeviceGuard dg(device);
        hipStream_t st = (hipStream_t)stream;
        const size_t n = (size_t)Cout * Cin * 9;
        std::vector<float> pk(n);
        for (int64_t o = 0; o < Cout; ++o)
            for (int64_t i = 0; i < Cin; ++i)
                for (int tap = 0; tap < 9; ++tap) pk[(o * 9 + tap) * Cin + i] = w_host[(o * Cin + i) * 9 + tap];
        float amax = 0.f;
        for (float v : pk) amax = std::max(amax, std::fabs(v));
        int ex = 0;
        if (amax > 0.f) std::frexp(amax, &ex);
        const float s = std::ldexp(1.0f, -ex);
        std::vector<_Float16> hi(n), lo(n), phi, plo;
        for (size_t e = 0; e < n; ++e) {
            const float v = pk[e] * s;
            hi[e] = (_Float16)v;
            lo[e] = (_Float16)(v - (float)hi[e]);
        }
        cfd::ConvArgs a{};
        cfd::phase_pack_host(w_host, Cout, Cin, phi, plo, a.ph_scale);
        struct Bufs {
            void* p[7] = {};
            ~Bufs() { for (void* q : p) (void)hipFree(q); }
        } d;
        const size_t bytes[6] = {n * 4, n * 2, n * 2, phi.size() * 2, plo.size() * 2, (size_t)Cout * 4};
        const void* srcs[6] = {pk.data(), hi.data(), lo.data(), phi.data(), plo.data(), bias_host};
        for (int k = 0; k < 6; ++k) {
            CFD_HIP(hipMalloc(&d.p[k], bytes[k]));
            CFD_HIP(hipMemcpy(d.p[k], srcs[k], bytes[k], hipMemcpyHostToDevice));
        }
        a.src1 = x;
        a.C1 = a.Ctot = Cin;
        a.w = (const float*)d.p[0];
        a.wbf = d.p[1];
        a.wlo = d.p[2];
        a.wph = d.p[3];
        a.wpl = d.p[4];
        a.acc_scale = std::ldexp(1.0f, ex);
        a.bias = (const float*)d.p[5];
        a.out = out;
        a.Hin = H;
        a.Win = W;
        a.Hout = 2 * H;
        a.Wout = 2 * W;
        a.stride = 1;
        a.ks = 3;
        a.pad = 1;
        a.up = 1;
        a.Cout = Cout;
        a.M = B * a.Hout * a.Wout;
        a.K = 9 * Cin;
        a.plan_b = plan_b > 0 ? plan_b : 8;
        const cfd::ConvPlan plan = cfd::plan_conv(a, kSplitPer8);
        if (plan.splits > 1) {
            CFD_HIP(hipMalloc(&d.p[6], sizeof(float) * plan.splits * (size_t)a.M * Cout));
            a.part = (float*)d.p[6];
        }
        if (kx) *kx = plan.kx;
        static const int conv_log = getenv("CFD_CONV_LOG") ? atoi(getenv("CFD_CONV_LOG")) : 0;
        if (conv_log)
            fprintf(stderr, "CONV upsample_conv %dx%d C=%d+%d->%d ks=%d s=%d up=%d M=%d kx=%d bm=%d bn=%d nw=%d splits=%d\n",
                    a.Hin, a.Win, a.C1, a.C2, a.Cout, a.ks, a.stride, a.up, a.M, plan.kx, plan.bm, plan.bn, plan.nw,
                    plan.splits);
        cfd::launch_conv(a, plan, st);
        CFD_HIP(hipStreamSynchronize(st));
    });
}

extern "C" int cfd_unet_set_compute(cfd_unet* h, int compute) {
    return cfd::guard([&] {
        CFD_REQUIRE(h, CFD_EARG, "null handle");
        CFD_REQUIRE(compute == CFD_COMPUTE_F32 || compute == CFD_COMPUTE_BF16 || compute == CFD_COMPUTE_SPLIT_F16,
                    CFD_EARG, "unknown compute mode");
        if (h->compute != compute) ++h->version;
        h->compute = compute;
    });
}

extern "C" int cfd_unet_set_plan_batch(cfd_unet* h, int nominal_batch) {
    return cfd::guard([&] {
        CFD_REQUIRE(h, CFD_EARG, "null handle");
        CFD_REQUIRE(nominal_batch >= 0 && nominal_batch <= 64, CFD_EARG, "plan batch must be 0 (default) .. 64");
        if (h->plan_b != nominal_batch) {
            ++h->version;
            h->ws_cache.clear();
        }
        h->plan_b = nominal_batch;
    });
}

extern "C" int cfd_unet_set_time_freqs(cfd_unet* h, const float* host, int n) {
    return cfd::guard([&] {
        CFD_REQUIRE(h && host && n == h->cfg.model_channels / 2, CFD_EARG, "freqs must have model_channels/2 entries");
        cfd::DeviceGuard dg(h->device);
        CFD_HIP(hipMemcpy(h->freqs, host, sizeof(float) * n, hipMemcpyHostToDevice));
    });
}

extern "C" int cfd_unet_ready(const cfd_unet* h) {
    return cfd::guard([&] {
        CFD_REQUIRE(h, CFD_EARG, "null handle");
        for (const auto& p : h->params) CFD_REQUIRE(p.set, CFD_ESTATE, "U-Net parameter not set: " + p.key);
    });
}

namespace cfd {
size_t unet_ws_bytes(const cfd_unet* h, int B) {
    auto it = h->ws_cache.find(B);
    if (it != h->ws_cache.end()) return it->second;
    Workspace ws{nullptr, 0, true};
    run(h, nullptr, nullptr, nullptr, B, ws, nullptr);
    h->ws_cache[B] = ws.off + 256;
    return ws.off + 256;
}
void unet_check_ready(const cfd_unet* h) {
    for (const auto& p : h->params) CFD_REQUIRE(p.set, CFD_ESTATE, "U-Net parameter not set: " + p.key);
}
int unet_compute(const cfd_unet* h) { return h->compute; }
uint64_t unet_version(const cfd_unet* h) { return h->version; }
int unet_device(const cfd_unet* h) { return h->device; }
int* unet_nonfinite(const cfd_unet* h) { return h->nonfinite; }
void unet_forward_raw(const cfd_unet* h, const float* x, const int64_t* t, float* eps, int B, void* workspace,
                      hipStream_t st) {
    Workspace ws{(char*)(((uintptr_t)workspace + 255) & ~uintptr_t(255)), 0, false};
    run(h, x, t, eps, B, ws, st);
}
}

extern "C" int cfd_unet_workspace_bytes(const cfd_unet* h, int B, size_t* bytes) {
    return cfd::guard([&] {
        CFD_REQUIRE(h && bytes && B > 0, CFD_EARG, "bad argument");
        *bytes = cfd::unet_ws_bytes(h, B);
    });
}

extern "C" int cfd_unet_forward(cfd_unet* h, const float* x, const int64_t* t, float* eps, int B, void* workspace,
                                size_t ws_bytes, void* stream) {
    return cfd::guard([&] {
        CFD_REQUIRE(h && x && t && eps && workspace, CFD_EARG, "null argument");
        CFD_REQUIRE(B > 0, CFD_EARG, "B must be positive");
        cfd::unet_check_ready(h);
        CFD_REQUIRE(ws_bytes >= cfd::unet_ws_bytes(h, B), CFD_EARG, "workspace too small");
        cfd::unet_forward_raw(h, x, t, eps, B, workspace, (hipStream_t)stream);
    });
}

namespace {
size_t tape_bytes_mode(const cfd_unet* h, int B, int mode) {
    Workspace ws{nullptr, 0, true}, tws{nullptr, 0, true};
    Tape tape{&tws, nullptr};
    tape.keep_gnout = mode == CFD_TAPE_PARAM_GRAD;
    run(h, nullptr, nullptr, nullptr, B, ws, nullptr, &tape, false);
    return tws.off + 256;
}
}

extern "C" int cfd_unet_tape_bytes(const cfd_unet* h, int B, size_t* bytes) {
    return cfd::guard([&] {
        CFD_REQUIRE(h && bytes && B > 0, CFD_EARG, "bad argument");
        *bytes = tape_bytes_mode(h, B, h->tape_mode);
    });
}

namespace {
constexpr size_t kMaxTapes = 64;

const cfd_unet::TapeRec& tape_rec(const cfd_unet* h, const void* tape, int B, size_t tape_bytes) {
    auto it = h->tapes.find(tape);
    CFD_REQUIRE(it != h->tapes.end(), CFD_ESTATE,
                "tape was not recorded by cfd_unet_forward_tape on this handle (or was forgotten: at most 64 live "
                "tapes per handle)");
    CFD_REQUIRE(it->second.B == B, CFD_EARG, "B differs from the batch the tape was recorded at");
    CFD_REQUIRE(it->second.plan == plan_batch(h), CFD_ESTATE,
                "the planned batch changed since the tape was recorded (cfd_unet_set_plan_batch)");
    CFD_REQUIRE(tape_bytes >= tape_bytes_mode(h, B, it->second.mode), CFD_EARG, "tape too small");
    return it->second;
}
}

extern "C" int cfd_unet_set_tape_mode(cfd_unet* h, int mode) {
    return cfd::guard([&] {
        CFD_REQUIRE(h, CFD_EARG, "null handle");
        CFD_REQUIRE(mode == CFD_TAPE_INPUT_VJP || mode == CFD_TAPE_PARAM_GRAD, CFD_EARG, "unknown tape mode");
        h->tape_mode = mode;
    });
}

extern "C" int cfd_unet_vjp_workspace_bytes(const cfd_unet* h, int B, size_t* bytes) {
    return cfd::guard([&] {
        CFD_REQUIRE(h && bytes && B > 0, CFD_EARG, "bad argument");
        Workspace ws{nullptr, 0, true};
        std::vector<Rec> none;
        run_vjp(h, nullptr, nullptr, B, none, ws, nullptr);
        *bytes = ws.off + 256;
    });
}

namespace {
char* align256(void* p) { return (char*)(((uintptr_t)p + 255) & ~uintptr_t(255)); }

void check_ready(const cfd_unet* h) {
    for (const auto& p : h->params) CFD_REQUIRE(p.set, CFD_ESTATE, "U-Net parameter not set: " + p.key);
}
}

extern "C" int cfd_unet_forward_tape(cfd_unet* h, const float* x, const int64_t* t, float* eps, int B,
                                     void* workspace, size_t ws_bytes, void* tape, size_t tape_bytes, void* stream) {
    return cfd::guard([&] {
        CFD_REQUIRE(h && x && t && eps && workspace && tape, CFD_EARG, "null argument");
        CFD_REQUIRE(h->compute != CFD_COMPUTE_BF16, CFD_ESTATE,
                    "the input-gradient path is fp32-accurate: call cfd_unet_set_compute(h, CFD_COMPUTE_F32) "
                    "or CFD_COMPUTE_SPLIT_F16 first");
        CFD_REQUIRE(B > 0, CFD_EARG, "B must be positive");
        check_ready(h);
        size_t need = 0;
        cfd_unet_workspace_bytes(h, B, &need);
        CFD_REQUIRE(ws_bytes >= need, CFD_EARG, "workspace too small");
        CFD_REQUIRE(tape_bytes >= tape_bytes_mode(h, B, h->tape_mode), CFD_EARG, "tape too small");
        Workspace ws{align256(workspace), 0, false}, tws{align256(tape), 0, false};
        Tape tp{&tws, nullptr};
        tp.keep_gnout = h->tape_mode == CFD_TAPE_PARAM_GRAD;
// ... 81 lines not shown
```

confild_amd/csrc/unet_kernels.hip:

```cpp
#include <algorithm>
#include <cstdlib>

#include "unet_kernels.hpp"

namespace cfd {

__global__ __launch_bounds__(256) void gn_partial_kernel(GnArgs a) {
    const int chunk = blockIdx.x;
    const int64_t b = blockIdx.y;
    const int Ctot = a.Ctot, cq = Ctot / 4, cpg = Ctot / 32;
    const int HW = a.HW;
    const int p0 = (int)((int64_t)HW * chunk / a.nchunks), p1 = (int)((int64_t)HW * (chunk + 1) / a.nchunks);
    const int rows = 256 / cq;
    const int q = threadIdx.x % cq, r0 = threadIdx.x / cq;
    __shared__ double red[2][1024];
    if (r0 < rows) {
        double s[4] = {0, 0, 0, 0}, s2[4] = {0, 0, 0, 0};
        const int c0 = 4 * q;
        for (int p = p0 + r0; p < p1; p += rows) {
            const int64_t pix = b * HW + p;
            const f4 v = c0 < a.C1 ? *(const f4*)(a.src1 + pix * a.C1 + c0)
                                   : *(const f4*)(a.src2 + pix * a.C2 + (c0 - a.C1));
#pragma unroll
            for (int j = 0; j < 4; ++j) {
// ... 266 lines not shown
    if (act) {
        f4 sc, sf;
#pragma unroll
        for (int j = 0; j < 4; ++j) {
            sc[j] = sh[0][4 * q + j];
            sf[j] = sh[1][4 * q + j];
        }
        const int64_t dst = b * HW * Ctot + c;
#pragma unroll
        for (int k = 0; k < IPT; ++k) {
            const int p = r0 + k * rows;
            if (p < HW) {
                f4 y;
#pragma unroll
                for (int j = 0; j < 4; ++j) {
                    y[j] = v[k][j] * sc[j] + sf[j];
                    if (a.silu) y[j] = silu_f(y[j]);
                }
                gn_store4(a, dst + (int64_t)p * Ctot, y);
                mx = fmaxf(mx, amax4(y));
            }
        }
    }
    if (a.amax_out) block_amax_atomic(mx, a.amax_out);
#ifdef CFD_STAMPS
    __builtin_amdgcn_s_waitcnt(0);
#endif
    CFD_STAMP(a.stamps, 4, a.seq, 4);
}

int gn2_chunks(int HW, int plan_b) {
    if (HW > kGn2BigHW) return kGn2BigChunks;
    const int pb = plan_b > 0 ? plan_b : 8;
    const int cap = std::min(kGn2BigChunks, std::max(64, 64 * 8 / pb));
    return (int)std::max<int64_t>(1, std::min<int64_t>(cap, HW / 16));
}

template <int NT>
__global__ __launch_bounds__(NT) void gn2_stats_kernel(GnArgs a) {
    const int chunk = blockIdx.x;
    const int64_t b = blockIdx.y;
    const int Ctot = a.Ctot, cq = Ctot / 4, cpg = Ctot / 32;
    const int HW = a.HW, NC = gridDim.x;
    const int p0 = (int)((int64_t)HW * chunk / NC), p1 = (int)((int64_t)HW * (chunk + 1) / NC);
    const int rows = NT / cq;
    const int q = threadIdx.x % cq, r0 = threadIdx.x / cq;
    const int c0 = 4 * q;
    const bool act = r0 < rows;
    const bool ksrc = a.kpart && c0 < a.C1;
    __shared__ double red[2][4 * NT];
    double s[4] = {0, 0, 0, 0}, s2[4] = {0, 0, 0, 0};
    f4 kb = {0.f, 0.f, 0.f, 0.f}, ke = {0.f, 0.f, 0.f, 0.f};
    if (ksrc) {
#pragma unroll
        for (int j = 0; j < 4; ++j) {
            if (a.kbias) kb[j] = a.kbias[c0 + j];
            if (a.kemb) ke[j] = a.kemb[b * a.kemb_stride + c0 + j];
        }
    }
    const int64_t slab = (int64_t)a.B * HW * a.C1;
    constexpr int U = 4;
    if (act) {
        for (int pb = p0 + r0; pb < p1; pb += U * rows) {
            f4 v[U];
            if (ksrc) {
                f4 rs[U];
#pragma unroll
                for (int u = 0; u < U; ++u) {
                    const int p = pb + u * rows;
                    const int64_t e = (b * HW + p) * a.C1 + c0;
                    rs[u] = a.kres && p < p1 ? *(const f4*)(a.kres + e) : f4{0.f, 0.f, 0.f, 0.f};
                    v[u] = p < p1 ? *(const f4*)(a.kpart + e) : f4{0.f, 0.f, 0.f, 0.f};
                }
                for (int sp = 1; sp < a.ksplits; ++sp) {
                    f4 w[U];
#pragma unroll
                    for (int u = 0; u < U; ++u) {
                        const int p = pb + u * rows;
                        w[u] = p < p1 ? *(const f4*)(a.kpart + sp * slab + (b * HW + p) * a.C1 + c0)
                                      : f4{0.f, 0.f, 0.f, 0.f};
                    }
#pragma unroll
                    for (int u = 0; u < U; ++u) v[u] += w[u];
                }
#pragma unroll
                for (int u = 0; u < U; ++u) {
                    const int p = pb + u * rows;
                    if (p >= p1) continue;
#pragma unroll
                    for (int j = 0; j < 4; ++j) {
                        float y = a.kbias ? v[u][j] + kb[j] : v[u][j];
                        if (a.kemb) y = y + ke[j];
                        if (a.kres) y = rs[u][j] + y;
                        v[u][j] = y;
                    }
                    *(f4*)(a.kx + (b * HW + p) * a.C1 + c0) = v[u];
                }
            } else {
#pragma unroll
                for (int u = 0; u < U; ++u) {
                    const int p = pb + u * rows;
                    const int64_t pix = b * HW + p;
                    v[u] = p >= p1 ? f4{0.f, 0.f, 0.f, 0.f}
                         : c0 < a.C1 ? *(const f4*)(a.src1 + pix * a.C1 + c0)
                                     : *(const f4*)(a.src2 + pix * a.C2 + (c0 - a.C1));
                }
            }
#pragma unroll
            for (int u = 0; u < U; ++u)
#pragma unroll
                for (int j = 0; j < 4; ++j) {
                    s[j] += v[u][j];
                    s2[j] += (double)v[u][j] * v[u][j];
                }
        }
#pragma unroll
        for (int j = 0; j < 4; ++j) {
            red[0][r0 * Ctot + c0 + j] = s[j];
            red[1][r0 * Ctot + c0 + j] = s2[j];
        }
    }
    __syncthreads();
    constexpr int GL = NT / 32;
    const int grp = threadIdx.x / GL, sub = threadIdx.x % GL;
    double ts = 0, ts2 = 0;
    for (int e = sub; e < rows * cpg; e += GL) {
        const int r = e / cpg, c = grp * cpg + (e - r * cpg);
        ts += red[0][r * Ctot + c];
        ts2 += red[1][r * Ctot + c];
    }
#pragma unroll
    for (int o = 1; o < GL; o <<= 1) {
        ts += __shfl_xor(ts, o);
        ts2 += __shfl_xor(ts2, o);
    }
    if (sub == 0) {
        double* dst = a.part + ((b * NC + chunk) * 32 + grp) * 2;
        dst[0] = ts;
        dst[1] = ts2;
    }
}

template <int NT>
__global__ __launch_bounds__(NT) void gn2_apply_kernel(GnArgs a) {
    const int chunk = blockIdx.x;
    const int64_t b = blockIdx.y;
    const int Ctot = a.Ctot, cq = Ctot / 4, cpg = Ctot / 32;
    const int HW = a.HW, NC = gridDim.x;
    __shared__ float ssh[2][1024];
    {
        constexpr int GL = NT / 32;
        const int grp = threadIdx.x / GL, sub = threadIdx.x % GL;
        double S = 0, S2 = 0;
        for (int k = sub; k < NC; k += GL) {
            const double2 v = *(const double2*)(a.part + ((b * NC + k) * 32 + grp) * 2);
            S += v.x;
            S2 += v.y;
        }
#pragma unroll
        for (int o = 1; o < GL; o <<= 1) {
            S += __shfl_xor(S, o);
            S2 += __shfl_xor(S2, o);
        }
        const double n = (double)HW * cpg;
        const double mean = S / n;
        const double var = fmax(S2 / n - mean * mean, 0.0);
        const float mf = (float)mean, rf = (float)(1.0 / sqrt(var + (double)a.eps));
        if (sub < cpg) {
            for (int cc = sub; cc < cpg; cc += GL) {
                const int c = grp * cpg + cc;
                const float sc = rf * a.gamma[c];
                const float sf = a.beta[c] - mf * sc;
                ssh[0][c] = sc;
                ssh[1][c] = sf;
                if (chunk == 0) {
                    a.ss[(b * Ctot + c) * 2 + 0] = sc;
                    a.ss[(b * Ctot + c) * 2 + 1] = sf;
                }
            }
        }
        if (a.stats && chunk == 0 && sub == 0) {
            a.stats[(b * 32 + grp) * 2 + 0] = mf;
            a.stats[(b * 32 + grp) * 2 + 1] = rf;
        }
    }
    __syncthreads();
    const int p0 = (int)((int64_t)HW * chunk / NC), p1 = (int)((int64_t)HW * (chunk + 1) / NC);
    const int rows = NT / cq;
    const int q = threadIdx.x % cq, r0 = threadIdx.x / cq;
    const int c0 = 4 * q;
    float mx = 0.f;
    if (r0 < rows) {
        f4 sc, sf;
#pragma unroll
        for (int j = 0; j < 4; ++j) {
            sc[j] = ssh[0][c0 + j];
            sf[j] = ssh[1][c0 + j];
        }
        const bool kin = a.kpart && c0 < a.C1;
        const float* xs = kin ? a.kx : c0 < a.C1 ? a.src1 : a.src2;
        const int ld = c0 < a.C1 ? a.C1 : a.C2, cx = c0 < a.C1 ? c0 : c0 - a.C1;
        constexpr int U = 4;
        for (int pb = p0 + r0; pb < p1; pb += U * rows) {
            f4 v[U];
#pragma unroll
            for (int u = 0; u < U; ++u) {
                const int p = pb + u * rows;
                v[u] = p < p1 ? *(const f4*)(xs + (b * HW + p) * ld + cx) : f4{0.f, 0.f, 0.f, 0.f};
            }
#pragma unroll
            for (int u = 0; u < U; ++u) {
                const int p = pb + u * rows;
                if (p >= p1) continue;
                f4 y;
#pragma unroll
                for (int j = 0; j < 4; ++j) {
                    y[j] = v[u][j] * sc[j] + sf[j];
                    if (a.silu) y[j] = silu_f(y[j]);
                }
                gn_store4(a, (b * HW + p) * Ctot + c0, y);
                mx = fmaxf(mx, amax4(y));
            }
        }
    }
    if (a.amax_out) block_amax_atomic(mx, a.amax_out);
}

__device__ __forceinline__ int lds_swz(int row, int chunk) { return row * 32 + 4 * (chunk ^ ((row ^ (row >> 1)) & 7)); }

__device__ __forceinline__ int lds_swz_bf(int row, int chunk) {
    return row * 64 + ((chunk + 2 * ((row >> 2) & 1)) & 3) * 16;
}

__device__ __forceinline__ void split4_mix(const f4& x, uint2& hi, uint2& lo) {
    typedef _Float16 h2_ __attribute__((ext_vector_type(2)));
    typedef float f2_ __attribute__((ext_vector_type(2)));
    hi.x = __builtin_bit_cast(unsigned, __builtin_convertvector((f2_){x[0], x[1]}, h2_));
    hi.y = __builtin_bit_cast(unsigned, __builtin_convertvector((f2_){x[2], x[3]}, h2_));
    asm("v_fma_mixlo_f16 %0, %1, 1.0, -%2 op_sel_hi:[0,0,1]" : "=&v"(lo.x) : "v"(x[0]), "v"(hi.x));
    asm("v_fma_mixhi_f16 %0, %1, 1.0, -%2 op_sel:[0,0,1] op_sel_hi:[0,0,1]" : "+v"(lo.x) : "v"(x[1]), "v"(hi.x));
    asm("v_fma_mixlo_f16 %0, %1, 1.0, -%2 op_sel_hi:[0,0,1]" : "=&v"(lo.y) : "v"(x[2]), "v"(hi.y));
    asm("v_fma_mixhi_f16 %0, %1, 1.0, -%2 op_sel:[0,0,1] op_sel_hi:[0,0,1]" : "+v"(lo.y) : "v"(x[3]), "v"(hi.y));
}


template <int BM, int BN, bool TMODE, int MODE, int NW = 4, bool BUFA = false, int PF = 1>
__global__ __launch_bounds__(64 * NW, NW == 4 ? 2 : 1) void conv_gemm_kernel(ConvArgs a) {
    constexpr bool BF = MODE == 1, SP = MODE == 2;
    constexpr int BK = 32;
    constexpr int WM = BM / (NW / 2), WN = BN / 2;
    constexpr int TM = WM / 16, TN = WN / 16;
    constexpr int RPP = 8 * NW;
    constexpr int AIT = BM / RPP, BIT = BN / RPP;
    static_assert(AIT >= 1 && BIT >= 1 && TM >= 1, "tile too small for the wave count");
    constexpr int AFL = BF ? BM * BK / 2 : BM * BK, BFL = BF ? BN * BK / 2 : BN * BK;
    __shared__ __attribute__((aligned(16))) float smem_ab[2 * AFL + 2 * BFL];
    float(*const As)[AFL] = (float(*)[AFL])smem_ab;
    float(*const Bs)[BFL] = (float(*)[BFL])(smem_ab + 2 * AFL);
    constexpr int EPI_FL = 2 * AFL + 2 * BFL;
    constexpr int EPI_PASSES = (BM * BN + EPI_FL - 1) / EPI_FL;
    constexpr bool LDSEPI_FITS = BM % EPI_PASSES == 0 && (BM / EPI_PASSES) % WM == 0 &&
                                 (BM / EPI_PASSES) * BN <= EPI_FL && (BM / EPI_PASSES) * BN / 4 % (64 * NW) == 0;
    __shared__ int pixtab[BUFA ? 9 * BM : 1];

    CFD_STAMP(a.stamps, 1, a.seq, 0);
    const int tid = threadIdx.x, lane = tid & 63, wave = tid >> 6;
    const int wm = wave >> 1, wn = wave & 1;
    int bx, by, bz;
    xcd_tile(a.xcd, bx, by, bz);
    const int m0 = bx * BM, n0 = by * BN;
    const int HWo = a.Hout * a.Wout;
    const int kq = tid & 7, rsub = tid >> 3;

    int a_b[AIT], a_oy[AIT], a_ox[AIT];
    bool a_ok[AIT];
#pragma unroll
    for (int it = 0; it < AIT; ++it) {
        const int m = m0 + rsub + it * RPP;
        a_ok[it] = m < a.M;
        const int mm = a_ok[it] ? m : 0;
        a_b[it] = mm / HWo;
        const int rem = mm - a_b[it] * HWo;
        a_oy[it] = rem / a.Wout;
        a_ox[it] = rem - a_oy[it] * a.Wout;
        if (TMODE) {
            a_oy[it] += a.pad;
            a_ox[it] += a.pad;
        } else if (!a.up) {
            a_oy[it] = a_oy[it] * a.stride - a.pad;
            a_ox[it] = a_ox[it] * a.stride - a.pad;
        } else {
            a_oy[it] -= a.pad;
            a_ox[it] -= a.pad;
        }
    }
    const float* wrow[BIT];
    const unsigned short* wrow_bf[BIT];
    const unsigned short* wrow_lo[BIT];
    bool b_ok[BIT];
#pragma unroll
    for (int it = 0; it < BIT; ++it) {
        const int n = n0 + rsub + it * RPP;
        b_ok[it] = n < a.Cout;
        if constexpr (BF || SP)
            wrow_bf[it] = (const unsigned short*)a.wbf + (int64_t)(b_ok[it] ? n : 0) * a.K + 4 * kq;
        else
            wrow[it] = a.w + (int64_t)(b_ok[it] ? n : 0) * a.K + 4 * kq;
        if constexpr (SP) wrow_lo[it] = (const unsigned short*)a.wlo + (int64_t)(b_ok[it] ? n : 0) * a.K + 4 * kq;
    }
    const int nkt = a.K / BK;
// ... 813 lines not shown
        for (int d = 0; d < ND; ++d) O[d] = O[d] * alpha;
        h8v ph, pl;
        split8_f16(p, ph, pl);
        const h8v* vl8 = &ring[stage][KP * 64 + lane];
#pragma unroll
        for (int d = 0; d < ND; ++d) {
            const h8v vh = vl8[(2 * d) * 64], vl = vl8[(2 * d + 1) * 64];
            O[d] = __builtin_amdgcn_mfma_f32_16x16x32_f16(vl, ph, O[d], 0, 0, 0);
            O[d] = __builtin_amdgcn_mfma_f32_16x16x32_f16(vh, pl, O[d], 0, 0, 0);
            O[d] = __builtin_amdgcn_mfma_f32_16x16x32_f16(vh, ph, O[d], 0, 0, 0);
        }
    }
    if (!active) return;
    const int tq = q0 + li;
    if constexpr (SPLIT) {
        if (tq < T) {
            const int64_t row = ((int64_t)kc_i * (gridDim.z / kcs) + b) * heads + h;
            float* op = a.part + (row * T + tq) * CH;
#pragma unroll
            for (int d = 0; d < ND; ++d) *(f4*)(op + 16 * d + 4 * g) = O[d];
            if (g == 0) {
                float* ml = a.part + (int64_t)kcs * (gridDim.z / kcs) * heads * T * CH;
                *(float2*)(ml + 2 * (row * T + tq)) = float2{mrun, lrun};
            }
        }
        return;
    }
    if (a.lse && g == 0 && tq < T)
        a.lse[((int64_t)b * gridDim.y + h) * T + tq] = (mrun + log2f(lrun)) * 0.69314718055994530942f;
    if (tq < T) {
        float* op = a.out + (b * (int64_t)T + tq) * a.C + (int64_t)h * CH;
        const float inv = 1.0f / lrun;
#pragma unroll
        for (int d = 0; d < ND; ++d) {
            f4 v = O[d] * inv;
            *(f4*)(op + 16 * d + 4 * g) = v;
        }
    }
}

template <int CH>
__global__ __launch_bounds__(256) void attn_combine_kernel(AttnArgs a, int heads, int B) {
    constexpr int Q = CH / 4;
    const int64_t i = (int64_t)blockIdx.x * blockDim.x + threadIdx.x;
    const int64_t rows = (int64_t)B * heads * a.T;
    if (i >= rows * Q) return;
    const int d4 = (int)(i % Q);
    const int64_t r = i / Q;
    const int kc = a.kc;
    const float* ml = a.part + (int64_t)kc * rows * CH;
    float M = -INFINITY;
    for (int c = 0; c < kc; ++c) M = fmaxf(M, ml[2 * (c * rows + r)]);
    float L = 0.f;
    f4 o = {0.f, 0.f, 0.f, 0.f};
    for (int c = 0; c < kc; ++c) {
        const float w = __builtin_amdgcn_exp2f(ml[2 * (c * rows + r)] - M);
        L += w * ml[2 * (c * rows + r) + 1];
        o += w * *(const f4*)(a.part + (c * rows + r) * CH + 4 * d4);
    }
    const int tq = (int)(r % a.T);
    const int64_t bh = r / a.T;
    const int h = (int)(bh % heads);
    const int64_t b = bh / heads;
    *(f4*)(a.out + (b * (int64_t)a.T + tq) * a.C + (int64_t)h * CH + 4 * d4) = o * (1.0f / L);
    if (a.lse && d4 == 0) a.lse[bh * a.T + tq] = (M + log2f(L)) * 0.69314718055994530942f;
}

__global__ void temb_kernel(const int64_t* __restrict__ t, const float* __restrict__ freqs, float* __restrict__ out,
                            int dim) {
    const int b = blockIdx.x;
    const int half = dim / 2;
    const float tf = (float)t[b];
    for (int i = threadIdx.x; i < dim; i += blockDim.x) {
        float v = 0.f;
        if (i < half) {
            v = cosf(tf * freqs[i]);
        } else if (i < 2 * half) {
            v = sinf(tf * freqs[i - half]);
        }
        out[(int64_t)b * dim + i] = v;
    }
}

template <int KW>
__global__ __launch_bounds__(256) void linear_kernel(const float* __restrict__ x, const float* __restrict__ W,
                                                     const float* __restrict__ bias, float* __restrict__ y, int B,
                                                     int K, int N, int act) {
    constexpr int BC = 8;
    extern __shared__ __attribute__((aligned(16))) float xs[];
    const int lane = threadIdx.x & 63;
    const int n = blockIdx.x * 4 + (threadIdx.x >> 6);
    const bool live = n < N;
    CFD_DASSERT(K <= 256 * KW && K % 4 == 0);
    f4 w[KW];
#pragma unroll
    for (int i = 0; i < KW; ++i) {
        const int k = 4 * (lane + 64 * i);
        w[i] = live && k < K ? *(const f4*)(W + (int64_t)n * K + k) : f4{0.f, 0.f, 0.f, 0.f};
    }
    const float bn = live ? bias[n] : 0.f;
    for (int b0 = 0; b0 < B; b0 += BC) {
        const int nb = min(BC, B - b0);
        __syncthreads();
        for (int i = threadIdx.x; i < nb * K; i += 256) {
            const float v = x[(int64_t)b0 * K + i];
            xs[i] = act ? silu_f(v) : v;
        }
        __syncthreads();
        if (!live) continue;
        for (int bb = 0; bb < nb; ++bb) {
            float s = 0.f;
#pragma unroll
            for (int i = 0; i < KW; ++i) {
                const int k = 4 * (lane + 64 * i);
                if (k < K) {
                    const f4 v = *(const f4*)(xs + bb * K + k);
                    s = fmaf(w[i][0], v[0], s);
                    s = fmaf(w[i][1], v[1], s);
                    s = fmaf(w[i][2], v[2], s);
                    s = fmaf(w[i][3], v[3], s);
                }
            }
            for (int o = 32; o > 0; o >>= 1) s += __shfl_xor(s, o);
            if (lane == 0) y[(int64_t)(b0 + bb) * N + n] = s + bn;
        }
    }
}

int gn_chunks(int HW) {
    const int64_t small = std::min<int64_t>(64, HW / 16);
    return (int)std::max<int64_t>(1, std::min<int64_t>(kGnMaxChunks, std::max<int64_t>(HW / 64, small)));
}

static unsigned long long* g_stamps = nullptr;
void stamps_set(unsigned long long* buf) { g_stamps = buf; }
unsigned long long* stamps_buf() { return g_stamps; }
static int g_seq = 0;

static int env_int(const char* name, int dflt) {
    const char* e = getenv(name);
    return e ? atoi(e) : dflt;
}

bool gn2_applies(const GnArgs& a) {
    const int pb = a.plan_b > 0 ? a.plan_b : 8;
    return (int64_t)a.HW * 8 >= (int64_t)4096 * pb && a.Ctot % 4 == 0 && a.C1 % 4 == 0 && a.C2 % 4 == 0 &&
           a.Ctot <= 1024;
}

static int gn_reg_ipt(const GnArgs& a) {
    return a.Ctot % 128 == 0 ? (int)ceil_div(a.HW, 512 / (a.Ctot / 128)) : 0;
}

bool gn_takes_splitk(const GnArgs& a, int B) {
    (void)B;
    if (gn2_applies(a)) return a.C1 % 4 == 0;
    if (a.Ctot % 128 != 0 || a.C1 % 4 != 0) return false;
    return gn_reg_ipt(a) <= 16;
}

void launch_gn(const GnArgs& a0, int B, hipStream_t st) {
    CFD_REQUIRE(a0.Ctot % 32 == 0 && a0.C1 % 4 == 0 && a0.C2 % 4 == 0 && a0.Ctot <= 1024, CFD_ESHAPE,
                "GroupNorm32 needs channels % 32 == 0 (<= 1024)");
    GnArgs a = a0;
    a.nchunks = gn_chunks(a.HW);
    a.B = B;
    a.stamps = g_stamps;
    a.seq = g_seq++;
    CFD_REQUIRE(!a.kpart || gn_takes_splitk(a, B), CFD_ESTATE, "internal: split-K source on a GroupNorm path without it");
    if (gn2_applies(a)) {
        CFD_REQUIRE(!a.kpart || a.kx, CFD_ESTATE, "internal: gn2 needs the split-K sum's destination");
        a.nchunks = gn2_chunks(a.HW, a.plan_b);
        if (gn2_threads(a.nchunks) == 1024) {
            hipLaunchKernelGGL(gn2_stats_kernel<1024>, dim3(a.nchunks, B), dim3(1024), 0, st, a);
            check_launch("gn2_stats_kernel");
            hipLaunchKernelGGL(gn2_apply_kernel<1024>, dim3(a.nchunks, B), dim3(1024), 0, st, a);
        } else {
            hipLaunchKernelGGL(gn2_stats_kernel<256>, dim3(a.nchunks, B), dim3(256), 0, st, a);
            check_launch("gn2_stats_kernel");
            hipLaunchKernelGGL(gn2_apply_kernel<256>, dim3(a.nchunks, B), dim3(256), 0, st, a);
        }
        check_launch("gn2_apply_kernel");
        return;
    }
    const int ipt = gn_reg_ipt(a);
    if (ipt > 0 && ipt <= 32) {
        const dim3 grid((unsigned)(32 * B));
        const int nq = a.Ctot / 128, r256 = 256 / nq, i256 = (a.HW + r256 - 1) / r256;
        if (i256 <= 4) {
            if (i256 <= 1)
                hipLaunchKernelGGL((gn_fused_reg_kernel<1, 256>), grid, dim3(256), 0, st, a);
            else if (i256 <= 2)
                hipLaunchKernelGGL((gn_fused_reg_kernel<2, 256>), grid, dim3(256), 0, st, a);
            else
                hipLaunchKernelGGL((gn_fused_reg_kernel<4, 256>), grid, dim3(256), 0, st, a);
            check_launch("gn_fused_reg_kernel");
            return;
        }
        if (ipt <= 4)
            hipLaunchKernelGGL((gn_fused_reg_kernel<2, 1024>), grid, dim3(1024), 0, st, a);
        else if (ipt <= 8)
            hipLaunchKernelGGL((gn_fused_reg_kernel<4, 1024>), grid, dim3(1024), 0, st, a);
        else if (ipt <= 16)
            hipLaunchKernelGGL((gn_fused_reg_kernel<8, 1024>), grid, dim3(1024), 0, st, a);
        else
            hipLaunchKernelGGL(gn_fused_reg_kernel<32>, grid, dim3(512), 0, st, a);
        check_launch("gn_fused_reg_kernel");
        return;
    }
    hipLaunchKernelGGL(gn_partial_kernel, dim3(a.nchunks, B), dim3(256), 0, st, a);
    check_launch("gn_partial_kernel");
    hipLaunchKernelGGL(gn_finalize_kernel, dim3(B), dim3(1024), 0, st, a);
    check_launch("gn_finalize_kernel");
    const int64_t nq = (int64_t)B * a.HW * a.Ctot / 4;
    hipLaunchKernelGGL(gn_apply_kernel, dim3((unsigned)std::min<int64_t>(4096, ceil_div(nq, 256))), dim3(256), 0, st, a);
    check_launch("gn_apply_kernel");
}


static int even_splits(int nch, int splits) {
    if (splits <= 1) return 1;
    const int per = (nch + splits - 1) / splits;
    return (nch + per - 1) / per;
}

constexpr int64_t kK1pMin128 = 144, kK1pMin64 = 192;

ConvPlan plan_conv(const ConvArgs& a, size_t part_cap_floats) {
    const int plan_b = a.plan_b > 0 ? a.plan_b : 8;
    ConvPlan p;
    const int64_t mn = (int64_t)plan_b * a.Hout * a.Wout;
    p.bn = a.Cout >= 128 ? 128 : 64;
    auto tiles = [&](int bm) { return ceil_div(mn, bm) * ceil_div(a.Cout, p.bn); };
    p.bm = 64;
    int wg_per_tile = 1;
    if (p.bn == 128) {
        p.bm = 128;
        p.nw = 8;
        wg_per_tile = 2;
    }
    const int nkt = a.K / 32;
    p.splits = 1;
    while (tiles(p.bm) * wg_per_tile * p.splits < 768 && nkt / (p.splits * 2) >= 4 && p.splits < 16)
        p.splits *= 2;
    if (a.ks == 1 && !a.tmode && tiles(p.bm) >= 128) p.splits = 1;
    while (p.splits > 1 && (size_t)p.splits * mn * a.Cout > part_cap_floats) p.splits /= 2;
    if (conv_p_applies(a) && !(ceil_div(mn, 32) * ceil_div(a.Cout, 64) < 32 && a.K >= 1024)) {
        ConvPlan q;
        const int64_t t128 = ceil_div(mn, 128) * ceil_div(a.Cout, 128), t64 = ceil_div(mn, 64) * ceil_div(a.Cout, 64);
        q.kx = t128 >= kK1pMin128 ? 40 : t64 >= kK1pMin64 ? 41 : 42;
        conv_p_tile(q.kx, q.bm, q.bn, q.nw);
        q.splits = 1;
        return q;
    }
    if (a.wlo && a.ks == 3 && a.stride == 1 && !a.tmode && a.Ctot <= 128 && (int64_t)a.Hout * a.Wout >= 36864)
        return p;
    const int64_t srows = mn / ((int64_t)a.Hout * a.Wout) * a.Hin * a.Win;
    const bool fits32 = srows < (1 << 23) && srows * std::max(a.C1, a.C2) * 4 < (1ll << 30) &&
                        (int64_t)a.Cout * a.K * 2 < (1ll << 31);
    auto halo_splits = [&](int64_t t) {
        const int nch = a.Ctot / 32;
        int sp = 1;
        while (t * sp < 256 && sp * 2 <= nch && sp < 16) sp *= 2;
        while (sp > 1 && (size_t)sp * mn * a.Cout > part_cap_floats) sp /= 2;
        return even_splits(nch, sp);
    };
#ifndef CFD_NO_UPPHASE
    if (a.up && a.wph && a.wpl && a.wbf && a.wlo && !a.tmode && a.ks == 3 && a.stride == 1 && a.pad == 1 &&
        a.Hout == 2 * a.Hin && a.Wout == 2 * a.Win && a.Cout >= kPhaseMinCout && fits32) {
        ConvPlan q;
        q.bn = 128;
        if (conv_hp_tw(a) > 0) {
            q.kx = 24;
            q.bm = 256;
            q.nw = 8;
            const int64_t t = ceil_div(mn, 256) * ceil_div(a.Cout, 128);
            const int nch = a.Ctot / 32;
            int sp = 1;
            while (t * sp * 2 <= 256 && sp * 2 <= nch && sp < 16) sp *= 2;
            while (sp > 1 && (size_t)sp * mn * a.Cout > part_cap_floats) sp /= 2;
            q.splits = even_splits(nch, sp);
            return q;
        }
        q.kx = mn / 4 >= 2048 ? 26 : 25;
        q.bm = q.kx == 26 ? 256 : 128;
        q.nw = q.kx == 26 ? 8 : 4;
        const int64_t t = 4 * ceil_div(mn / 4, q.bm) * ceil_div(a.Cout, 128);
        const int nkp = 4 * a.Ctot / 32;
        q.splits = 1;
        while (t * q.splits * 2 <= 256 && nkp / (q.splits * 2) >= 4 && q.splits < 32) q.splits *= 2;
        while (q.splits > 1 && (size_t)q.splits * mn * a.Cout > part_cap_floats) q.splits /= 2;
        return q;
    }
#endif
    if (a.wbf && !a.wlo && !a.tmode && a.ks == 3 && a.stride == 1 && a.Cout >= 128 && fits32 && conv_h_tw(a) > 0) {
        ConvPlan q;
        q.kx = 22;
        q.bm = 256;
        q.bn = 128;
        q.nw = 8;
        q.splits = halo_splits(ceil_div(mn, 256) * ceil_div(a.Cout, 128));
        return q;
    }
    if (a.wbf && a.wlo && !a.tmode && a.ks == 3 && a.stride == 1 && a.Cout >= 128 && fits32) {
        ConvPlan q;
        if (conv_h_tw(a) > 0) {
            q.kx = 20;
            q.bm = 256;
            q.bn = 128;
            q.nw = 8;
            q.splits = halo_splits(ceil_div(mn, 256) * ceil_div(a.Cout, 128));
            return q;
        }
        q.kx = mn >= 2048 ? 2 : 1;
        q.bm = q.kx == 2 ? 256 : 128;
        q.bn = 128;
        q.nw = q.kx == 2 ? 8 : 4;
        const int64_t t = ceil_div(mn, q.bm) * ceil_div(a.Cout, q.bn);
        q.splits = 1;
        while (t * q.splits < 256 && nkt / (q.splits * 2) >= 4 && q.splits < 32) q.splits *= 2;
        while (q.splits > 1 && (size_t)q.splits * mn * a.Cout > part_cap_floats) q.splits /= 2;
        return q;
    }
    return p;
}

int smalln_below() {
    const int v = env_int("CFD_CONV_SMALLN", 1);
    return v == 1 ? 128 : std::max(v, 0);
}

template <bool TMODE, int MODE, bool BUFA>
static void launch_conv_tiles_(const ConvArgs& a, const ConvPlan& p, dim3 grid, hipStream_t st) {
    if constexpr (MODE != 0 && BUFA) {
        static const int smalln = smalln_below();
        if (!TMODE && p.nw == 8 && p.bm == 128 && p.bn == 128 && (int64_t)grid.x * grid.y * grid.z < smalln &&
            a.Cout % 64 == 0) {
            const dim3 g64(grid.x, (unsigned)ceil_div(a.Cout, 64), grid.z);
            hipLaunchKernelGGL((conv_gemm_kernel<128, 64, false, MODE, 8, true>), g64, dim3(512), 0, st, a);
            return;
        }
        if (p.nw == 8 && p.bm == 128 && p.bn == 128 && p.pf == 2) {
            hipLaunchKernelGGL((conv_gemm_kernel<128, 128, TMODE, MODE, 8, true, 2>), grid, dim3(512), 0, st, a);
            return;
        }
        if (p.nw == 8 && p.bm == 128 && p.bn == 128 && p.pf == 3) {
            hipLaunchKernelGGL((conv_gemm_kernel<128, 128, TMODE, MODE, 8, true, 3>), grid, dim3(512), 0, st, a);
            return;
        }
    }
    if (p.nw == 8 && p.bm == 128 && p.bn == 128)
        hipLaunchKernelGGL((conv_gemm_kernel<128, 128, TMODE, MODE, 8, BUFA>), grid, dim3(512), 0, st, a);
    else if (p.bm == 128 && p.bn == 128)
        hipLaunchKernelGGL((conv_gemm_kernel<128, 128, TMODE, MODE, 4, BUFA>), grid, dim3(256), 0, st, a);
    else if (p.bm == 64 && p.bn == 128)
        hipLaunchKernelGGL((conv_gemm_kernel<64, 128, TMODE, MODE, 4, BUFA>), grid, dim3(256), 0, st, a);
    else if (p.bm == 128 && p.bn == 64)
        hipLaunchKernelGGL((conv_gemm_kernel<128, 64, TMODE, MODE, 4, BUFA>), grid, dim3(256), 0, st, a);
    else
        hipLaunchKernelGGL((conv_gemm_kernel<64, 64, TMODE, MODE, 4, BUFA>), grid, dim3(256), 0, st, a);
}

template <bool TMODE, int MODE>
static void launch_conv_tiles(const ConvArgs& a, const ConvPlan& p, dim3 grid, hipStream_t st) {
    if (a.bufaddr) return launch_conv_tiles_<TMODE, MODE, true>(a, p, grid, st);
    launch_conv_tiles_<TMODE, MODE, false>(a, p, grid, st);
}

void launch_splitk_reduce(const ConvArgs& a, int splits, hipStream_t st) {
    const int64_t total4 = (int64_t)a.M * a.Cout / 4;
    hipLaunchKernelGGL(splitk_reduce_kernel, dim3((unsigned)ceil_div(total4, 256)), dim3(256), 0, st, a, splits);
    check_launch("splitk_reduce_kernel");
}

static bool conv_x_falls_back(const ConvArgs& a) {
    static const int force_k1s = env_int("CFD_CONV_FORCE_K1S", 0);
    const int64_t srows = (int64_t)a.Hin * a.Win * (a.M / (a.Hout * a.Wout));
    return force_k1s || !(srows < (1 << 24) && a.M < (1 << 24) && srows * std::max(a.C1, a.C2) * 4 < (1ll << 31));
}

static bool conv_p_falls_back(const ConvArgs& a) {
    return !conv_p_applies(a) || (int64_t)a.Cout * a.K * 2 >= (1ll << 31);
}

bool conv_runs_k1hb(const ConvArgs& a, const ConvPlan& p) { return p.kx == 22 && !conv_x_falls_back(a); }

bool conv_kv_pack_ok(const ConvArgs& a, const ConvPlan& p, int T) {
    static const int ldsepi = env_int("CFD_CONV_LDSEPI", 1);
    return ldsepi && (p.kx < 0 || p.kx >= 40) && p.splits == 1 && a.wbf && !a.tmode && a.ks == 1 && a.bias &&
           !a.emb && !a.res && a.Cout % 8 == 0 && a.emb_stride % 4 == 0 && T % 32 == 0 && a.M % T == 0;
}

int launch_conv(const ConvArgs& a, const ConvPlan& p0, hipStream_t st, bool defer) {
    ConvPlan p = p0;
    if (p.kx >= 0 && (conv_x_falls_back(a) || (p.kx >= 40 && conv_p_falls_back(a)))) {
        p.kx = -1;
        p.bm = p.bn = 128;
        p.nw = 8;
    }
    CFD_REQUIRE(!a.src_bf16 || p.kx == 22, CFD_ESTATE, "internal: a bf16 convolution source needs the K1hb kernel");
    static const int pf = env_int("CFD_CONV_PF", 2);
    if (p.kx < 0) p.pf = pf >= 1 && pf <= 3 ? pf : 1;
    CFD_REQUIRE(a.Ctot % 32 == 0 && a.C1 % 4 == 0 && a.C2 % 4 == 0, CFD_ESHAPE, "conv_gemm needs channels % 32 == 0");
    CFD_REQUIRE(a.K == a.ks * a.ks * a.Ctot, CFD_ESHAPE, "conv K mismatch");
    CFD_REQUIRE(p.splits == 1 || (a.part && a.Cout % 4 == 0), CFD_ESTATE, "split-K needs a partial buffer");
    CFD_REQUIRE(!a.tmode || ((a.stride == 1 || a.stride == 2) && !a.up), CFD_ESHAPE, "transposed conv: stride 1|2");
    const dim3 grid((unsigned)ceil_div(a.M, p.bm), (unsigned)ceil_div(a.Cout, p.bn), p.splits);
    CFD_REQUIRE(!(a.tmode && a.wbf && !a.wlo), CFD_ESTATE, "bf16 input-gradient convolutions are not built");
    static const int xcd = env_int("CFD_CONV_XCD", 4);
    static const int ldsepi = env_int("CFD_CONV_LDSEPI", 1);
    ConvArgs b = a;
    b.stamps = g_stamps;
    b.seq = g_seq++;
    b.ldsepi = ldsepi && a.Cout % 4 == 0 && a.emb_stride % 4 == 0;
    const int xo = xcd == 4 ? (a.wbf && !a.wlo ? 1 : 3) : xcd;
    b.xcd = xo == 3 ? ((int64_t)a.Hout * a.Wout <= 256 ? 2 : 1) : xo < 0 || xo > 2 ? 1 : xo;
    {
        const int64_t srows = (int64_t)a.Hin * a.Win * (a.M / (a.Hout * a.Wout));
        const int64_t wes = (a.wbf || a.wlo) ? 2 : 4;
        b.bufaddr = a.ks * a.ks <= 9 && srows < (1 << 24) && a.M < (1 << 24) &&
                    srows * std::max(a.C1, a.C2) * 4 < (1ll << 31) && (int64_t)a.Cout * a.K * wes < (1ll << 31);
    }
    const ConvArgs& a_ = b;
    if (p.kx >= 40) {
        CFD_REQUIRE(p.splits == 1, CFD_ESTATE, "internal: K1p does not split over K");
        launch_conv_p(a_, p.kx, st);
        return 1;
    }
    if (p.kx >= 0) {
        launch_conv_x(a_, p.kx, p.splits, st, p.adjoint);
        if (p.splits > 1 && !defer) launch_splitk_reduce(a, p.splits, st);
        return p.splits;
    }
    if (a.tmode && a.wlo)
        launch_conv_tiles<true, 2>(a_, p, grid, st);
    else if (a.tmode)
        launch_conv_tiles<true, 0>(a_, p, grid, st);
    else if (a.wbf && a.wlo)
        launch_conv_tiles<false, 2>(a_, p, grid, st);
    else if (a.wbf)
        launch_conv_tiles<false, 1>(a_, p, grid, st);
    else
        launch_conv_tiles<false, 0>(a_, p, grid, st);
    check_launch("conv_gemm_kernel");
    if (p.splits > 1 && !defer) launch_splitk_reduce(a, p.splits, st);
    return p.splits;
}

void launch_conv_in(const ConvArgs& a, hipStream_t st) {
    if (a.Cout % 4 == 0 && a.C1 <= 4 && (size_t)9 * a.C1 * a.Cout * 4 <= 64 * 1024) {
        const int64_t n = (int64_t)a.M * (a.Cout / 4);
        hipLaunchKernelGGL(conv_in_vec_kernel, dim3((unsigned)std::min<int64_t>(2048, ceil_div(n, 256))), dim3(256),
                           sizeof(float) * 9 * a.C1 * a.Cout, st, a);
        check_launch("conv_in_vec_kernel");
        return;
    }
    const int64_t n = (int64_t)a.M * a.Cout;
    hipLaunchKernelGGL(conv_in_kernel, dim3((unsigned)ceil_div(n, 256)), dim3(256), 0, st, a);
    check_launch("conv_in_kernel");
}

void launch_conv_out(const ConvArgs& a, hipStream_t st) {
    CFD_REQUIRE(a.Cout <= 4, CFD_ESHAPE, "out_channels must be <= 4");
    const int LP = a.Ctot / 4;
    if (a.Ctot % 4 == 0 && a.C1 == a.Ctot && LP >= 1 && LP <= 64 && (LP & (LP - 1)) == 0 &&
        (size_t)a.Cout * a.K * 4 <= 64 * 1024) {
        const int64_t waves = ceil_div(a.M, 64 / LP);
        hipLaunchKernelGGL(conv_out_vec_kernel, dim3((unsigned)std::min<int64_t>(8192, ceil_div(waves, 4))), dim3(256),
                           sizeof(float) * a.Cout * a.K, st, a, LP);
        check_launch("conv_out_vec_kernel");
        return;
    }
    hipLaunchKernelGGL(conv_out_kernel, dim3((unsigned)ceil_div(a.M, 4)), dim3(256), 0, st, a);
    check_launch("conv_out_kernel");
}

void launch_attention(const AttnArgs& a, int CH, int heads, int B, hipStream_t st) {
    const dim3 grid((unsigned)ceil_div(a.T, 64), heads, B);
    switch (CH) {
        case 16: hipLaunchKernelGGL(attention_kernel<16>, grid, dim3(256), 0, st, a); break;
        case 32: hipLaunchKernelGGL(attention_kernel<32>, grid, dim3(256), 0, st, a); break;
        case 64: hipLaunchKernelGGL(attention_kernel<64>, grid, dim3(256), 0, st, a); break;
        case 128: hipLaunchKernelGGL(attention_kernel<128>, grid, dim3(256), 0, st, a); break;
        default: throw Error{CFD_ESHAPE, "attention head channels must be 16, 32, 64 or 128"};
    }
    check_launch("attention_kernel");
}

size_t attention_split_floats(int T, int C) { return (size_t)(T + 31) / 32 * 32 * C * 2; }

int64_t attention_split_voff(int T, int CH, int heads, int B) {
    const int T32 = (T + 31) / 32 * 32;
    return (int64_t)B * heads * (T32 / 16) * (CH / 32) * 128;
}

int attention_kv_chunks(int T, int heads, int plan_b) {
    const int nblk = (T + 31) / 32;
    const int64_t wgs = (int64_t)plan_b * heads * ceil_div(T, 64);
    int kc = 1;
    while (kc * 4 <= nblk && wgs * kc * 2 <= 256) kc *= 2;
    return kc;
}

size_t attention_part_floats(int T, int C, int CH, int plan_b) {
    const int heads = C / CH, kc = attention_kv_chunks(T, heads, plan_b);
    return kc == 1 ? 0 : (size_t)kc * T * (C + 2 * heads);
}

void launch_attention_split(const AttnArgs& a, int CH, int heads, int B, int plan_b, float* kvws, hipStream_t st,
                            bool packed) {
    CFD_REQUIRE(CH == 32 || CH == 64 || CH == 128, CFD_ESHAPE, "split attention needs head channels 32, 64 or 128");
    const int T32 = (a.T + 31) / 32 * 32;
    h8v* kf = (h8v*)kvws;
    h8v* vf = kf + attention_split_voff(a.T, CH, heads, B);
    if (!packed) {
        const int64_t slots = (int64_t)B * heads * ((T32 / 16) * (CH / 32) * 64 + (T32 / 32) * (CH / 16) * 64);
        hipLaunchKernelGGL(attn_kv_split_kernel, dim3((unsigned)ceil_div(slots, 256)), dim3(256), 0, st, a, CH, heads,
                           B, kf, vf);
        check_launch("attn_kv_split_kernel");
    }
    const int kc = attention_kv_chunks(a.T, heads, plan_b);
    if (kc > 1) {
        CFD_REQUIRE(a.part, CFD_ESTATE, "internal: key-chunked attention without a partial buffer");
        AttnArgs a2 = a;
        a2.kc = kc;
        a2.xcdmap = 0;
        const dim3 grid((unsigned)ceil_div(a.T, 64), heads, B * kc);
        switch (CH) {
            case 32: hipLaunchKernelGGL((attention_dma_kernel<32, 4, 3, true>), grid, dim3(256), 0, st, a2, kf, vf); break;
            case 64: hipLaunchKernelGGL((attention_dma_kernel<64, 4, 3, true>), grid, dim3(256), 0, st, a2, kf, vf); break;
            default: hipLaunchKernelGGL((attention_dma_kernel<128, 4, 3, true>), grid, dim3(256), 0, st, a2, kf, vf); break;
        }
        check_launch("attention_dma_kernel (key chunks)");
        const int64_t n = (int64_t)B * heads * a.T * (CH / 4);
        const dim3 g2((unsigned)ceil_div(n, 256));
        switch (CH) {
            case 32: hipLaunchKernelGGL(attn_combine_kernel<32>, g2, dim3(256), 0, st, a2, heads, B); break;
            case 64: hipLaunchKernelGGL(attn_combine_kernel<64>, g2, dim3(256), 0, st, a2, heads, B); break;
            default: hipLaunchKernelGGL(attn_combine_kernel<128>, g2, dim3(256), 0, st, a2, heads, B); break;
        }
        check_launch("attn_combine_kernel");
        return;
    }
    static const int xcdmap = env_int("CFD_ATTN_XCD", 1);
    AttnArgs a2 = a;
    a2.xcdmap = xcdmap && (heads * B) % 8 == 0 ? 1 : 0;
    const int w8 = a.T >= 512 && (int64_t)B * heads * ceil_div(a.T, 128) >= 256;
    const dim3 grid((unsigned)ceil_div(a.T, w8 ? 128 : 64), heads, B);
    const dim3 blk(w8 ? 512 : 256);
    switch (CH * 2 + w8) {
        case 64: hipLaunchKernelGGL((attention_dma_kernel<32, 4>), grid, blk, 0, st, a2, kf, vf); break;
        case 65: hipLaunchKernelGGL((attention_dma_kernel<32, 8>), grid, blk, 0, st, a2, kf, vf); break;
        case 128: hipLaunchKernelGGL((attention_dma_kernel<64, 4>), grid, blk, 0, st, a2, kf, vf); break;
        case 129: hipLaunchKernelGGL((attention_dma_kernel<64, 8>), grid, blk, 0, st, a2, kf, vf); break;
        case 256: hipLaunchKernelGGL((attention_dma_kernel<128, 4>), grid, blk, 0, st, a2, kf, vf); break;
        default: hipLaunchKernelGGL((attention_dma_kernel<128, 8>), grid, blk, 0, st, a2, kf, vf); break;
    }
    check_launch("attention_dma_kernel");
}

void launch_temb(const int64_t* t, const float* freqs, float* out, int dim, int B, hipStream_t st) {
    hipLaunchKernelGGL(temb_kernel, dim3(B), dim3(128), 0, st, t, freqs, out, dim);
    check_launch("temb_kernel");
}

void launch_linear(const float* x, const float* W, const float* bias, float* y, int B, int K, int N, int act,
                   hipStream_t st) {
    CFD_REQUIRE(K % 4 == 0 && K <= 2048, CFD_ESHAPE, "linear: K must be a multiple of 4, at most 2048");
    const dim3 g((unsigned)ceil_div(N, 4));
    const size_t lds = sizeof(float) * 8 * K;
    if (K <= 256) hipLaunchKernelGGL(linear_kernel<1>, g, dim3(256), lds, st, x, W, bias, y, B, K, N, act);
    else if (K <= 512) hipLaunchKernelGGL(linear_kernel<2>, g, dim3(256), lds, st, x, W, bias, y, B, K, N, act);
    else if (K <= 1024) hipLaunchKernelGGL(linear_kernel<4>, g, dim3(256), lds, st, x, W, bias, y, B, K, N, act);
    else hipLaunchKernelGGL(linear_kernel<8>, g, dim3(256), lds, st, x, W, bias, y, B, K, N, act);
    check_launch("linear_kernel");
}

}

extern "C" int cfd_stamps_set(void* buf) {
#ifdef CFD_STAMPS
    cfd::stamps_set((unsigned long long*)buf);
    return CFD_OK;
// ... 7 lines not shown
```

confild_amd/csrc/unet_kernels.hpp:

```cpp
#pragma once
#include <algorithm>
#include <cmath>
#include <vector>

#include "common.hpp"

namespace cfd {

struct GnArgs {
    const float* src1;
    const float* src2;
    const float* gamma;
    const float* beta;
    double* part;
    float* ss;
    float* out;
    float* stats;
    int C1, C2, Ctot, HW;
    float eps;
    int silu;
    int nchunks;
    int B;
    const float* kpart;
    const float* kbias;
    const float* kemb;
    const float* kres;
    float* kx;
    int ksplits, kemb_stride;
    unsigned long long* stamps;
    int seq;
    int out_bf16;
    unsigned* amax_out;
    int plan_b;
};

struct ConvArgs {
    const float* src1;
    const float* src2;
    const float* w;
    const void* wbf;
    const void* wlo;
    float acc_scale;
    const void* wph;
    const void* wpl;
    float ph_scale[4];
    const float* bias;
    const float* emb;
    const float* res;
    float* out;
    float* part;
    int C1, C2, Ctot;
    int Hin, Win, Hout, Wout;
    int stride, ks, pad, up;
    int tmode;
    int Cout;
    int emb_stride;
    int M, K;
    int xcd;
    int bufaddr;
    int ldsepi;
    int* nonfinite;
    int src_bf16;
    void* kvf;
    int64_t kv_voff;
    int kv_ch, kv_heads, kv_T;
    float kv_scale;
    unsigned long long* stamps;
    int seq;
    int plan_b;
};
constexpr int kPhaseMinCout = 128;

__host__ __device__ inline void phase_taps(int p, int t, int& lo, int& hi) {
    lo = t == 0 ? 0 : 1 + p;
    hi = t == 0 ? p : 2;
}
__host__ __device__ inline float phase_value(const float* w, int64_t ci, int ph, int64_t e) {
    const int64_t i = e % ci, ot = e / ci, o = ot >> 2;
    const int tap = (int)(ot & 3);
    int ylo, yhi, xlo, xhi;
    phase_taps(ph >> 1, tap >> 1, ylo, yhi);
    phase_taps(ph & 1, tap & 1, xlo, xhi);
    const float* base = w + (o * ci + i) * 9;
    double v = 0.0;
    for (int dy = ylo; dy <= yhi; ++dy)
        for (int dx = xlo; dx <= xhi; ++dx) v += (double)base[dy * 3 + dx];
    return (float)v;
}

inline void phase_pack_host(const float* w, int64_t co, int64_t ci, std::vector<_Float16>& phi,
                            std::vector<_Float16>& plo, float inv[4]) {
    const int64_t np4 = co * ci * 4;
    phi.resize((size_t)np4 * 4);
    plo.resize((size_t)np4 * 4);
    std::vector<float> pv((size_t)np4);
    for (int ph = 0; ph < 4; ++ph) {
        float amax = 0.f;
        for (int64_t e = 0; e < np4; ++e) {
            pv[e] = phase_value(w, ci, ph, e);
            amax = std::max(amax, std::fabs(pv[e]));
        }
        int ex = 0;
        if (amax > 0.f) std::frexp(amax, &ex);
        const float sc = std::ldexp(1.0f, -ex);
        inv[ph] = std::ldexp(1.0f, ex);
        for (int64_t e = 0; e < np4; ++e) {
            const float v = pv[e] * sc;
            phi[ph * np4 + e] = (_Float16)v;
            plo[ph * np4 + e] = (_Float16)(v - (float)phi[ph * np4 + e]);
        }
    }
}

void stamps_set(unsigned long long* buf);
unsigned long long* stamps_buf();

struct AttnArgs {
    const float* qkv;
    float* out;
    int T, C;
    float scale;
    float* lse;
    int xcdmap;
    int kc;
    float* part;
};

struct GnbArgs {
    const float* x1;
    const float* x2;
    const float* dz;
    const float* ss;
    const float* stats;
    const float* gamma;
    const float* addsrc;
    float* out1;
    float* out2;
    int acc1, acc2;
    double* part;
    float* fin;
    float* ppart;
    unsigned* amax_out;
    int C1, C2, Ctot, HW, silu, nchunks, B;
    int plan_b;
};

struct AttnBwdArgs {
    const float* qkv;
    const float* o;
    const float* dout;
    const float* lse;
    float* dd;
    float* dqkv;
    int T, C;
    float scale;
    h8v* packs;
    float* amax;
    int heads, xcdmap;
};

struct ConvPlan {
    int bm = 128, bn = 128, splits = 1;
    int nw = 4;
    int kx = -1;
    int pf = 1;
    bool adjoint = false;
};

constexpr int kGnMaxChunks = 512;
int gn_chunks(int HW);
constexpr int kGn2BigHW = 16384, kGn2BigChunks = 256;
static_assert(kGn2BigChunks <= kGnMaxChunks, "gn2 partials live in the kGnMaxChunks slab");
int gn2_chunks(int HW, int plan_b);
inline int gn2_threads(int nchunks) { return nchunks > 64 ? 1024 : 256; }
void launch_gn(const GnArgs& a, int B, hipStream_t st);
bool gn_takes_splitk(const GnArgs& a, int B);
bool gn2_applies(const GnArgs& a);
ConvPlan plan_conv(const ConvArgs& a, size_t part_cap_floats);
int launch_conv(const ConvArgs& a, const ConvPlan& p, hipStream_t st, bool defer = false);
void launch_splitk_reduce(const ConvArgs& a, int splits, hipStream_t st);
__device__ __forceinline__ void xcd_tile(int order, int& bx, int& by, int& bz) {
    bx = blockIdx.x;
    by = blockIdx.y;
    bz = blockIdx.z;
    if (!order) return;
    const unsigned gx = gridDim.x, gy = gridDim.y, gz = gridDim.z;
    const unsigned T = gx * gy * gz, L = blockIdx.x + gx * (blockIdx.y + gy * blockIdx.z);
    const unsigned q = T >> 3, r = T & 7, x = L & 7, sl = L >> 3;
    const unsigned Lp = x < r ? x * (q + 1) + sl : r * (q + 1) + (x - r) * q + sl;
    if (order == 2) {
        bx = Lp % gx;
        bz = (Lp / gx) % gz;
        by = Lp / (gx * gz);
    } else {
        bz = Lp % gz;
        by = (Lp / gz) % gy;
        bx = Lp / (gz * gy);
    }
}
int launch_conv_x(const ConvArgs& a, int variant, int splits, hipStream_t st, bool adjoint = false);
int conv_h_tw(const ConvArgs& a);
int conv_hp_tw(const ConvArgs& a);
int k1h_shape(int tw, int bn, bool phase, bool adjoint);
bool conv_p_applies(const ConvArgs& a);
void conv_p_tile(int variant, int& bm, int& bn, int& nw);
void launch_conv_p(const ConvArgs& a, int variant, hipStream_t st);
int smalln_below();
bool conv_runs_k1hb(const ConvArgs& a, const ConvPlan& p);
void launch_conv_in(const ConvArgs& a, hipStream_t st);
void launch_conv_out(const ConvArgs& a, hipStream_t st);
void launch_attention(const AttnArgs& a, int CH, int heads, int B, hipStream_t st);
size_t attention_split_floats(int T, int C);
int attention_kv_chunks(int T, int heads, int plan_b);
size_t attention_part_floats(int T, int C, int CH, int plan_b);
void launch_attention_split(const AttnArgs& a, int CH, int heads, int B, int plan_b, float* kvws, hipStream_t st,
                            bool packed);
int64_t attention_split_voff(int T, int CH, int heads, int B);
bool conv_kv_pack_ok(const ConvArgs& a, const ConvPlan& p, int T);
int launch_gn_bwd(const GnbArgs& a, int B, hipStream_t st);
void launch_attention_bwd(const AttnBwdArgs& a, int CH, int heads, int B, hipStream_t st);
size_t attention_bwd_split_floats(int T, int C);
bool attention_bwd_split_ok(int T, int CH);
void launch_attention_bwd_split(const AttnBwdArgs& a, int CH, int heads, int B, float* ws, hipStream_t st);
void launch_add(float* y, const float* x, int64_t n, hipStream_t st);
void launch_temb(const int64_t* t, const float* freqs, float* out, int dim, int B, hipStream_t st);
void launch_linear(const float* x, const float* W, const float* bias, float* y, int B, int K, int N, int act,
                   hipStream_t st);


__device__ __forceinline__ float kln2(float scale) { return scale * 1.44269504088896340736f; }
__device__ __forceinline__ void split8_f16(const float (&v)[8], h8v& hi, h8v& lo) {
#pragma clang fp contract(off)
#pragma unroll
    for (int t = 0; t < 8; ++t) {
        hi[t] = (_Float16)v[t];
        lo[t] = (_Float16)(v[t] - (float)hi[t]);
    }
}
constexpr int vmcnt_wait(int n) { return (n & 15) | (7 << 4) | (15 << 8) | (((n >> 4) & 3) << 14); }
}
```

include/confild.h:

```cpp
#ifndef CONFILD_H
#define CONFILD_H

#include <stddef.h>
#include <stdint.h>

#ifdef __cplusplus
extern "C" {
#endif

enum { CFD_OK = 0, CFD_EARG = 1, CFD_EHIP = 2, CFD_EKEY = 3, CFD_ESHAPE = 4, CFD_ESTATE = 5 };

const char* cfd_last_error(void);
const char* cfd_version(void);

typedef struct cfd_unet cfd_unet;

typedef struct {
    int image_size;
    int in_channels;
    int model_channels;
    int out_channels;
    int num_res_blocks;
    int n_mult;
    int channel_mult[8];
    int n_attn;
    int attention_ds[8];
    int num_heads;
    int num_head_channels;
} cfd_unet_cfg;

int  cfd_unet_create(const cfd_unet_cfg* cfg, int device, cfd_unet** out);
void cfd_unet_destroy(cfd_unet* h);
int  cfd_unet_num_params(const cfd_unet* h, int* n);
int  cfd_unet_param_info(const cfd_unet* h, int idx, const char** key, int* ndim, int64_t shape[4]);
int  cfd_unet_set_param(cfd_unet* h, const char* key, const float* host_data, size_t n);
int  cfd_unet_set_time_freqs(cfd_unet* h, const float* host_freqs, int n);
int  cfd_unet_ready(const cfd_unet* h);
int  cfd_unet_load_flat(cfd_unet* h, const float* flat, size_t n, void* stream);
int  cfd_unet_workspace_bytes(const cfd_unet* h, int B, size_t* bytes);
#define CFD_COMPUTE_F32       0
#define CFD_COMPUTE_BF16      1
#define CFD_COMPUTE_SPLIT_F16 2
int  cfd_unet_set_compute(cfd_unet* h, int compute);
int  cfd_unet_set_plan_batch(cfd_unet* h, int nominal_batch);
int  cfd_unet_forward(cfd_unet* h, const float* x, const int64_t* t, float* eps, int B,
                      void* workspace, size_t ws_bytes, void* stream);
int  cfd_unet_check_finite(cfd_unet* h, int* nonfinite, void* stream);
int  cfd_upsample_conv(const float* x, const float* w_host, const float* bias_host, float* out, int B, int H,
                       int W, int Cin, int Cout, int plan_b, int device, int* kx, void* stream);

int  cfd_unet_tape_bytes(const cfd_unet* h, int B, size_t* bytes);
int  cfd_unet_vjp_workspace_bytes(const cfd_unet* h, int B, size_t* bytes);
int  cfd_unet_forward_tape(cfd_unet* h, const float* x, const int64_t* t, float* eps, int B,
                           void* workspace, size_t ws_bytes, void* tape, size_t tape_bytes, void* stream);
int  cfd_unet_input_vjp(cfd_unet* h, const float* d_eps, float* d_x, int B, const void* tape,
                        size_t tape_bytes, void* workspace, size_t ws_bytes, void* stream);
#define CFD_TAPE_INPUT_VJP  0
#define CFD_TAPE_PARAM_GRAD 1
int  cfd_unet_set_tape_mode(cfd_unet* h, int mode);

typedef struct cfd_sched cfd_sched;
enum { CFD_COEF_SRA = 0, CFD_COEF_SRM1, CFD_COEF_M1, CFD_COEF_M2, CFD_COEF_SIGMA,
       CFD_COEF_SQRT_ABP, CFD_COEF_DIR, CFD_COEF_SIGMA_DDIM, CFD_NCOEF };
enum { CFD_STEP_DDPM = 0, CFD_STEP_DDIM = 1 };

int  cfd_sched_create(const float* host_coefs, int n_t, int device, cfd_sched** out);
void cfd_sched_destroy(cfd_sched* s);
int  cfd_sched_step(const cfd_sched* s, int kind, int clip, const float* x, const float* eps,
                    const int64_t* t, const float* noise, uint64_t seed, uint64_t counter,
                    uint64_t offset, float* x_out, float* xstart_out, int64_t n_per_sample, int B,
                    void* stream);
int  cfd_sched_step_known(const cfd_sched* s, int kind, int clip, const float* x, const float* eps,
                          const int64_t* t, const float* noise, uint64_t seed, uint64_t counter,
                          uint64_t offset, float* x_out, float* xstart_out, int64_t n_per_sample, int B,
                          const float* known, int64_t known_bstride, const float* mask, int64_t mask_bstride,
                          const float* table, const float* noise2, uint64_t counter2, void* stream);
int  cfd_sched_step_jump(const cfd_sched* s, int kind, int clip, const float* x, const float* eps,
                         const int64_t* t, const float* noise, uint64_t seed, uint64_t counter,
                         uint64_t offset, float* x_out, float* xstart_out, int64_t n_per_sample, int B,
                         const float* known, int64_t known_bstride, const float* mask, int64_t mask_bstride,
                         const float* table, const float* noise2, uint64_t counter2, float ja, float jb,
                         const float* noise3, uint64_t counter3, void* stream);
typedef struct cfd_sampler cfd_sampler;
int  cfd_sampler_create(const cfd_unet* unet, const cfd_sched* sched, int kind, int clip, int B,
                        int64_t n_per_sample, int n_steps, const int64_t* host_tidx, const int64_t* host_tmodel,
                        int graph, int unroll, cfd_sampler** out);
void cfd_sampler_destroy(cfd_sampler* sp);
int  cfd_device_cu_count(int device, int* n_cu);
int  cfd_stream_create_cu_range(int device, int first_cu, int n_cu, void** stream);
int  cfd_stream_destroy(void* stream);
int  cfd_sampler_run(cfd_sampler* sp, const float* x_in, float* x_out, int k0, int k1, uint64_t seed,
                     uint64_t offset, void* stream);
int  cfd_sampler_set_known(cfd_sampler* sp, const float* known, int64_t known_bstride, const float* mask,
                           int64_t mask_bstride, const float* table, void* stream);
int  cfd_sampler_captures(const cfd_sampler* sp, uint64_t* n);
int  cfd_sampler_set_jumps(cfd_sampler* sp, const float* host_jtab);
int  cfd_randn(float* out, int64_t n, uint64_t seed, uint64_t counter, uint64_t offset, void* stream);
int  cfd_sine_probe(const float* x, float* y, int64_t n, int which, void* stream);
int  cfd_latent_denorm(const float* x, float* y, int64_t n, const float* vmax, const float* vmin,
                       int64_t period, void* stream);

int  cfd_dps_residual(const float* y, int64_t y_batch_stride, const float* A, float* g_A, float* norm,
                      int64_t n_per_sample, int B, void* stream);
int  cfd_dps_latent_grad(const cfd_sched* s, int clip, const float* x, const float* eps, const int64_t* t,
                         const float* g_z, const float* vmax, const float* vmin, int64_t period,
                         float* d_eps, float* g_direct, int64_t n_per_sample, int B, void* stream);
int  cfd_dps_update(const float* sample, const float* g_direct, const float* g_unet, float scale,
                    float* x_out, int64_t n, void* stream);
int  cfd_dps_update_known(const float* sample, const float* g_direct, const float* g_unet, float scale,
                          float* x_out, const int64_t* t, int64_t n_per_sample, int B, const float* known,
                          int64_t known_bstride, const float* mask, int64_t mask_bstride, const float* table,
                          const float* noise2, uint64_t seed, uint64_t counter2, uint64_t offset, void* stream);
int  cfd_dps_latent_residual_workspace_bytes(int64_t n_per_sample, int B, size_t* bytes);
int  cfd_dps_latent_residual(const cfd_sched* s, int clip, const float* x, const float* eps, const int64_t* t,
                             const float* y, int64_t y_bstride, const float* mask, int64_t mask_bstride,
                             float* norm, float* d_eps, float* g_direct, int64_t n_per_sample, int B,
                             void* workspace, size_t ws_bytes, void* stream);

typedef struct cfd_siren cfd_siren;

typedef struct {
    int in_coord_features;
    int in_latent_features;
    int out_features;
    int num_hidden_layers;
    int hidden_features;
    float w0;
} cfd_siren_cfg;

int  cfd_siren_create(const cfd_siren_cfg* cfg, int device, cfd_siren** out);
void cfd_siren_destroy(cfd_siren* h);
int  cfd_siren_num_params(const cfd_siren* h, int* n);
int  cfd_siren_param_info(const cfd_siren* h, int idx, const char** key, int* ndim, int64_t shape[4]);
int  cfd_siren_set_param(cfd_siren* h, const char* key, const float* host_data, size_t n);
int  cfd_siren_ready(const cfd_siren* h);
int  cfd_siren_workspace_bytes(const cfd_siren* h, int b, size_t* bytes);
#define CFD_SIREN_F32       0
#define CFD_SIREN_SPLIT_F16 1
int  cfd_siren_set_compute(cfd_siren* h, int compute);
int  cfd_siren_get_compute(const cfd_siren* h, int* compute);
int  cfd_siren_forward(cfd_siren* h, const float* coords, int64_t N, const float* latents, int b,
                       const float* xmax, const float* xmin,
                       const float* ymax, const float* ymin, int64_t y_stride,
                       float* out, void* workspace, size_t ws_bytes, void* stream);
int  cfd_siren_jacobian_workspace_bytes(const cfd_siren* h, int b, size_t* bytes);
int  cfd_siren_forward_jacobian(cfd_siren* h, const float* coords, int64_t N, const float* latents, int b,
                                const float* xmax, const float* xmin,
                                const float* ymax, const float* ymin, int64_t y_stride,
                                float* out, float* jac,
                                void* workspace, size_t ws_bytes, void* stream);
int  cfd_siren_forward_jacobian_split(cfd_siren* h, const float* coords, int64_t N, const float* latents, int b,
                                      const float* xmax, const float* xmin,
                                      const float* ymax, const float* ymin, int64_t y_stride,
                                      float* out, float* jac,
                                      void* workspace, size_t ws_bytes, void* stream);
int  cfd_siren_hessian_workspace_bytes(const cfd_siren* h, int b, size_t* bytes);
int  cfd_siren_forward_hessian(cfd_siren* h, const float* coords, int64_t N, const float* latents, int b,
                               const float* xmax, const float* xmin,
                               const float* ymax, const float* ymin, int64_t y_stride,
                               float* out, float* jac, float* hess, int diag_only,
                               void* workspace, size_t ws_bytes, void* stream);
int  cfd_siren_forward_hessian_split(cfd_siren* h, const float* coords, int64_t N, const float* latents, int b,
                                     const float* xmax, const float* xmin,
                                     const float* ymax, const float* ymin, int64_t y_stride,
                                     float* out, float* jac, float* hess, int diag_only,
                                     void* workspace, size_t ws_bytes, void* stream);

int  cfd_siren_vjp_workspace_bytes(const cfd_siren* h, int64_t Ns, int R, size_t* bytes);
int  cfd_siren_tape_forward(cfd_siren* h, const float* coords, int64_t Ns, const float* latents, int R,
                            const float* xmax, const float* xmin,
                            const float* ymax, const float* ymin, int64_t y_stride,
                            float* out, void* workspace, size_t ws_bytes, void* stream);
int  cfd_siren_tape_vjp(cfd_siren* h, const float* g_out, int64_t Ns, int R,
                        const float* ymax, const float* ymin, int64_t y_stride,
                        float* g_latents, void* workspace, size_t ws_bytes, void* stream);

int  cfd_siren_jtape_workspace_bytes(const cfd_siren* h, int64_t Ns, int R, size_t* bytes);
int  cfd_siren_jtape_forward(cfd_siren* h, const float* coords, int64_t Ns, const float* latents, int R,
                             const float* xmax, const float* xmin,
                             const float* ymax, const float* ymin, int64_t y_stride,
                             float* out, float* jac, void* workspace, size_t ws_bytes, void* stream);
int  cfd_siren_jtape_vjp(cfd_siren* h, const float* g_out, const float* g_jac, int64_t Ns, int R,
                         const float* ymax, const float* ymin, int64_t y_stride,
                         float* g_latents, void* workspace, size_t ws_bytes, void* stream);
int  cfd_dps_residual_linear(const float* y, int y_per_sample, const float* out, const float* jac,
                             const float* wv, int wv_per_sensor, const float* wj, int wj_per_sensor,
                             float* g_out, float* g_jac, float* norm, float* A, int64_t Ns, int M, int c,
                             int d, int rows_per_sample, int B, void* stream);

#define CFD_DENSE_SLAB 64
#define CFD_DENSE_DEFAULT_BUDGET ((size_t)1 << 30)
int  cfd_siren_dense_plan(const cfd_siren_cfg* cfg, int64_t N, int R, size_t budget, int bwd_form,
                          int compute_form, size_t* bytes, int64_t* chunk_points, int* block_rows);
int  cfd_siren_dense_workspace_bytes(const cfd_siren* h, int64_t N, int R, size_t budget, size_t* bytes);
int  cfd_siren_dense_grad(cfd_siren* h, const float* coords, int64_t N,
                          const float* latents, int R, int rows_per_sample,
                          const float* xmax, const float* xmin,
                          const float* ymax, const float* ymin, int64_t y_stride,
                          const float* y, int y_rows,
                          const float* mask, int mask_rows,
                          float* g_latents, float* norm,
                          void* workspace, size_t ws_bytes, size_t budget, void* stream);
// ... 41 lines not shown
```

Measured before the change: 4.262.

## Emit GroupNorm statistics partials from the conv epilogue and skip the stats kernel

The K1h conv epilogue now accumulates per-channel-quad sums and sums of squares in double precision, reduces them across the workgroup in LDS, and writes per-tile partials. The GroupNorm two-pass path reads these partials, including across concatenated skip inputs, instead of launching its separate stats kernel. This removes one full read of the conv output and one kernel launch per eligible GroupNorm. In exchange the epilogue does extra double-precision arithmetic and a block-wide reduction, and the eligible convs are forced onto the LDS epilogue and the 64-wide tile path. A probe entry point is added for testing.

```diff
diff --git a/confild_amd/_lib.py b/confild_amd/_lib.py
--- a/confild_amd/_lib.py
+++ b/confild_amd/_lib.py
@@ -52,6 +52,7 @@
     "cfd_unet_check_finite": (C.c_int, [C.c_void_p, C.POINTER(C.c_int), C.c_void_p]),
     "cfd_upsample_conv": (C.c_int, [C.c_void_p, C.c_void_p, C.c_void_p, C.c_void_p, C.c_int, C.c_int, C.c_int,
                                     C.c_int, C.c_int, C.c_int, C.c_int, C.POINTER(C.c_int), C.c_void_p]),
+    "cfd_conv_gn_probe": (C.c_int, [C.c_void_p] * 11 + [C.c_int] * 9 + [C.POINTER(C.c_int), C.c_void_p]),
     "cfd_unet_workspace_bytes": (C.c_int, [C.c_void_p, C.c_int, C.POINTER(C.c_size_t)]),
     "cfd_unet_forward": (C.c_int, [C.c_void_p, C.c_void_p, C.c_void_p, C.c_void_p, C.c_int, C.c_void_p,
                                    C.c_size_t, C.c_void_p]),
diff --git a/confild_amd/csrc/conv_x.hip b/confild_amd/csrc/conv_x.hip
--- a/confild_amd/csrc/conv_x.hip
+++ b/confild_amd/csrc/conv_x.hip
@@ -302,6 +302,25 @@
     return o2 ? Tile3{(int)lo, (int)hi, (int)mid} : Tile3{(int)hi, (int)mid, (int)lo};
 }
 
+template <int BN, int NTG>
+__device__ __forceinline__ void k1h_gn_partials(char* lds, int tid, const double (&s)[4], const double (&s2)[4],
+                                                double* dst, int nq) {
+    constexpr int Q = BN / 4, R = NTG / Q;
+    static_assert(R == 16, "K1h statistics: 16 thread rows per channel quad");
+    double2* red = (double2*)lds;
+    red[tid] = double2{((s[0] + s[1]) + s[2]) + s[3], ((s2[0] + s2[1]) + s2[2]) + s2[3]};
+    __syncthreads();
+    if (tid < Q && tid < nq) {
+        double2 t = red[tid];
+#pragma unroll
+        for (int r = 1; r < R; ++r) {
+            t.x += red[r * Q + tid].x;
+            t.y += red[r * Q + tid].y;
+        }
+        *(double2*)(dst + 2 * tid) = t;
+    }
+}
+
 template <int BM, int TW, int BN, bool PH>
 __device__ __forceinline__ void conv_h16_body(const ConvArgs& a) {
     constexpr int WGN = BN / 64, WGM = BM / 64, NTG = 64 * WGM * WGN;
@@ -516,6 +535,8 @@
         const bool split = gridDim.z > 1;
         float* dstb = split ? a.part + (int64_t)bz * a.M * a.Cout : a.out;
         constexpr int Q = BN / 4;
+        const bool gst = a.gnp && !split;
+        double gs[4] = {0, 0, 0, 0}, gs2[4] = {0, 0, 0, 0};
         __syncthreads();
         for (int r = 0; r < WGM; ++r) {
             if (wm == r) {
@@ -540,9 +561,23 @@
                         if (a.res) v = *(const f4*)(a.res + m * a.Cout + n) + v;
                     }
                     *(f4*)(dstb + m * a.Cout + n) = v;
+                    if (gst) {
+#pragma unroll
+                        for (int j = 0; j < 4; ++j) {
+                            gs[j] += (double)v[j];
+                            gs2[j] += (double)v[j] * (double)v[j];
+                        }
+                    }
                 }
             }
             __syncthreads();
+        }
+        if (gst) {
+            static_assert(NTG * 16 <= GBYTES, "statistics stage fits the LDS");
+            const int tile = PH ? ph * tps + tl : tl, ntile = PH ? 4 * tps : tps;
+            const int cq = a.Cout >> 2;
+            k1h_gn_partials<BN, NTG>(lds, tid, gs, gs2, a.gnp + (((int64_t)bimg * ntile + tile) * cq + (n0 >> 2)) * 2,
+                                     cq - (n0 >> 2));
         }
 #ifdef CFD_STAMPS
         __builtin_amdgcn_s_waitcnt(0);
@@ -877,6 +912,8 @@
             const bool split = gridDim.z > 1;
             float* dstb = split ? a.part + (int64_t)bz * a.M * a.Cout : a.out;
             constexpr int Q = BN / 4;
+            const bool gst = a.gnp && !split;
+            double gs[4] = {0, 0, 0, 0}, gs2[4] = {0, 0, 0, 0};
             __syncthreads();
             for (int r = 0; r < WGM; ++r) {
                 if (wm == r) {
@@ -902,9 +939,23 @@
                             if (a.res) v = *(const f4*)(a.res + m * a.Cout + n) + v;
                         }
                         *(f4*)(dstb + m * a.Cout + n) = v;
+                        if (gst) {
+#pragma unroll
+                            for (int j = 0; j < 4; ++j) {
+                                gs[j] += (double)v[j];
+                                gs2[j] += (double)v[j] * (double)v[j];
+                            }
+                        }
                     }
                 }
                 __syncthreads();
+            }
+            if (gst) {
+                static_assert(NTG * 16 <= GBYTES, "statistics stage fits the LDS");
+                const int tile = PH ? ph * tps + tl : tl, ntile = PH ? 4 * tps : tps;
+                const int cq = a.Cout >> 2;
+                k1h_gn_partials<BN, NTG>(lds, tid, gs, gs2,
+                                         a.gnp + (((int64_t)bimg * ntile + tile) * cq + (n0 >> 2)) * 2, cq - (n0 >> 2));
             }
 #ifdef CFD_STAMPS
             __builtin_amdgcn_s_waitcnt(0);
@@ -995,10 +1046,13 @@
     else launch_h_<BN, PH, 32>(a, tw, g, st);
 }
 
-int launch_conv_x(const ConvArgs& a, int variant, int splits, hipStream_t st, bool adjoint) {
+int launch_conv_x(const ConvArgs& a, int variant, int splits, hipStream_t st, bool adjoint, int bn) {
     CFD_REQUIRE(a.wbf && !a.tmode, CFD_ESTATE, "conv_x: split-f16 or bf16 forward only");
     CFD_REQUIRE(a.Ctot % 32 == 0 && a.C1 % 4 == 0 && a.C2 % 4 == 0, CFD_ESHAPE, "conv_x needs channels % 32 == 0");
     CFD_REQUIRE(splits == 1 || a.part, CFD_ESTATE, "split-K needs a partial buffer");
+    CFD_REQUIRE(!a.gnp || (splits == 1 && a.ldsepi && a.Cout % 4 == 0 &&
+                           (variant == 20 || variant == 22 || variant == 24 || variant == 36)),
+                CFD_ESTATE, "internal: statistics partials need an unsplit K1h / K1hb launch through the LDS epilogue");
     {
         const int64_t srows = (int64_t)a.Hin * a.Win * (a.M / (a.Hout * a.Wout));
         CFD_REQUIRE(srows < (1 << 24) && srows * std::max(a.C1, a.C2) * 4 < (1ll << 31) &&
@@ -1025,12 +1079,13 @@
         return splits;
     }
     CFD_REQUIRE(!a.src_bf16, CFD_ESTATE, "internal: a bf16 convolution source needs the K1hb kernel");
-    if (variant == 20 || variant == 32 || variant == 33) {
+    if (variant == 20 || variant == 32 || variant == 33 || variant == 36) {
         const int tw = conv_h_tw(a);
         CFD_REQUIRE(tw > 0 && a.wlo, CFD_ESHAPE, "conv_h: split-f16 3x3 stride-1 with a 16/32/64-divisible width");
         static const int smalln = smalln_below();
         const dim3 g = grid(256, 128);
-        const bool n64 = (int64_t)g.x * g.y * g.z < smalln && a.Cout % 64 == 0;
+        const bool n64 = ((int64_t)g.x * g.y * g.z < smalln || ((bn == 64 || variant == 36) && smalln > 0)) &&
+                         a.Cout % 64 == 0;
         const int shape = variant == 20 ? k1h_shape(tw, n64 ? 64 : 128, false, adjoint) : variant == 32 ? 32 : 16;
         if (n64) {
             launch_h<64, false>(a, tw, shape, grid(256, 64), st);
diff --git a/confild_amd/csrc/unet.hip b/confild_amd/csrc/unet.hip
--- a/confild_amd/csrc/unet.hip
+++ b/confild_amd/csrc/unet.hip
@@ -306,6 +306,8 @@
     int H = 0, W = 0;
     int C() const { return Ca + Cb; }
     bool bf16 = false;
+    const double* pa = nullptr;
+    const double* pb = nullptr;
 };
 
 struct Workspace {
@@ -428,6 +430,28 @@
     float* abuf = tape ? nullptr : ws.take((size_t)B * z.max_act);
     std::vector<float*> hsbuf;
     for (size_t n : z.hs) hsbuf.push_back(tape ? tape->tws->take((size_t)B * n) : ws.take((size_t)B * n));
+    std::vector<char> gnw(2 * h->steps.size(), 0);
+    std::vector<double*> gnpb(2 * h->steps.size(), nullptr);
+    {
+        int hw = S;
+        auto part = [&](size_t k, int co) {
+            if (!cfd::gn_partials_wanted(hw * hw, co, plan_batch(h))) return;
+            gnw[k] = 1;
+            gnpb[k] = (double*)ws.take((size_t)B * (hw * hw / 256) * (co / 4) * 4);
+        };
+        for (size_t si = 0; si < h->steps.size(); ++si) {
+            const auto& s = h->steps[si];
+            if (s.kind == cfd::Step::Res) {
+                part(2 * si, h->res[s.idx].cout);
+                part(2 * si + 1, h->res[s.idx].cout);
+            } else if (s.kind == cfd::Step::Down) {
+                hw = (hw + 1) / 2;
+            } else if (s.kind == cfd::Step::Up) {
+                hw *= 2;
+                part(2 * si, s.cout);
+            }
+        }
+    }
     constexpr int kGnSlots = 256;
     unsigned* gslots = tape ? (unsigned*)tape->tws->take(kGnSlots) : nullptr;
     int ngs = 0;
@@ -502,10 +526,14 @@
         } else {
             flush();
         }
+        g.p1 = in.pa;
+        g.p2 = in.pb;
+        g.nt1 = g.nt2 = in.H * in.W / 256;
         static const int gn_log = getenv("CFD_CONV_LOG") ? atoi(getenv("CFD_CONV_LOG")) : 0;
         if (gn_log && launch)
-            fprintf(stderr, "GN %s %dx%d C=%d+%d ksplits=%d kres=%d kx=%d silu=%d\n", pre.c_str(), in.H, in.W, g.C1,
-                    g.C2, g.kpart ? g.ksplits : 0, g.kres ? 1 : 0, g.kx ? 1 : 0, silu);
+            fprintf(stderr, "GN %s %dx%d C=%d+%d ksplits=%d kres=%d kx=%d silu=%d gn2=%d stats=%d\n", pre.c_str(), in.H,
+                    in.W, g.C1, g.C2, g.kpart ? g.ksplits : 0, g.kres ? 1 : 0, g.kx ? 1 : 0, silu,
+                    cfd::gn2_applies(g) ? 1 : 0, cfd::gn2_applies(g) && !cfd::gn_takes_partials(g) ? 1 : 0);
         g.out_bf16 = bf16_out ? 1 : 0;
         if (launch) cfd::launch_gn(g, B, st);
         Act r{g.out, in.C(), nullptr, 0, in.H, in.W};
@@ -553,18 +581,22 @@
     };
     using Tweak = std::function<void(cfd::ConvArgs&, const cfd::ConvPlan&)>;
     auto conv = [&](const Act& in, const std::string& pre, int cout, int ks, int stride, int up,
-                    const float* embp, const float* resp, float* out, const Tweak& tweak = {}) {
+                    const float* embp, const float* resp, float* out, const Tweak& tweak = {}, bool gnw = false,
+                    double* gnpo = nullptr) -> const double* {
         cfd::ConvArgs a = conv_args(in, pre, cout, ks, stride, up, embp, resp, out);
         flush();
+        static double no_buffer[2];
+        a.gnp = gnw ? (gnpo ? gnpo : no_buffer) : nullptr;
         const cfd::ConvPlan plan = plan_checked(h, a, kSplitCap);
+        if (a.gnp && !cfd::conv_emits_gn_partials(a, plan)) a.gnp = nullptr;
         if (tweak) tweak(a, plan);
         CFD_REQUIRE(!a.src_bf16 || cfd::conv_runs_k1hb(a, plan), CFD_ESTATE,
                     "internal: bf16 GroupNorm output feeds a convolution other than K1hb at " + pre);
         static const int conv_log = getenv("CFD_CONV_LOG") ? atoi(getenv("CFD_CONV_LOG")) : 0;
         if (conv_log && launch)
-            fprintf(stderr, "CONV %s %dx%d C=%d+%d->%d ks=%d s=%d up=%d M=%d kx=%d bm=%d bn=%d nw=%d splits=%d\n",
+            fprintf(stderr, "CONV %s %dx%d C=%d+%d->%d ks=%d s=%d up=%d M=%d kx=%d bm=%d bn=%d nw=%d splits=%d gnp=%d\n",
                     pre.c_str(), a.Hin, a.Win, a.C1, a.C2, a.Cout, a.ks, a.stride, a.up, a.M, plan.kx, plan.bm,
-                    plan.bn, plan.nw, plan.splits);
+                    plan.bn, plan.nw, plan.splits, a.gnp ? 1 : 0);
         if (launch) {
             const int sp = cfd::launch_conv(a, plan, st, true);
             if (sp > 1) {
@@ -572,6 +604,7 @@
                 pend.splits = sp;
             }
         }
+        return a.gnp ? gnpo : nullptr;
     };
 
     std::vector<std::pair<Act, int>> stack;
@@ -624,6 +657,7 @@
                 CFD_REQUIRE(cur.b == nullptr && skip.first.H == cur.H, CFD_ESTATE, "internal: concat shape");
                 cur.b = skip.first.a;
                 cur.Cb = skip.first.Ca;
+                cur.pb = skip.first.pa;
                 pending_skip = skip.second;
                 break;
             }
@@ -643,16 +677,19 @@
                     resp = cur.a;
                 }
                 float* hb = tape ? keep(nout) : tmp;
-                conv(xin, r.pre + ".in_layers.2", r.cout, 3, 1, 0, embo + r.emb_off, nullptr, hb);
+                Act th{hb, r.cout, nullptr, 0, cur.H, cur.W};
+                th.pa = conv(xin, r.pre + ".in_layers.2", r.cout, 3, 1, 0, embo + r.emb_off, nullptr, hb, {},
+                             gnw[2 * si], gnpb[2 * si]);
                 rec.h1 = hb;
-                const Act th{hb, r.cout, nullptr, 0, cur.H, cur.W};
                 const Act hn = gn(th, r.pre + ".out_layers.0", 1, &rec.ss2, &rec.st2, tape != nullptr,
                                   feeds_k1hb(th, r.pre + ".out_layers.3", r.cout), &rec.act2, &rec.amx2);
                 float* out = dest(cur.a, cur.b, nout);
                 if (r.cin != r.cout)
                     conv(cur, r.pre + ".skip_connection", r.cout, 1, 1, 0, nullptr, nullptr, skipb);
-                conv(hn, r.pre + ".out_layers.3", r.cout, 3, 1, 0, nullptr, resp, out);
+                const double* po = conv(hn, r.pre + ".out_layers.3", r.cout, 3, 1, 0, nullptr, resp, out, {},
+                                        gnw[2 * si + 1], gnpb[2 * si + 1]);
                 cur = Act{out, r.cout, nullptr, 0, cur.H, cur.W};
+                cur.pa = po;
                 break;
             }
             case cfd::Step::Attn: {
@@ -704,8 +741,10 @@
             }
             case cfd::Step::Up: {
                 float* out = tape ? keep((size_t)B * 4 * cur.H * cur.W * s.cout) : pick(cur.a, nullptr);
-                conv(cur, s.conv, s.cout, 3, 1, 1, nullptr, nullptr, out);
+                const double* po = conv(cur, s.conv, s.cout, 3, 1, 1, nullptr, nullptr, out, {}, gnw[2 * si],
+                                        gnpb[2 * si]);
                 cur = Act{out, s.cout, nullptr, 0, cur.H * 2, cur.W * 2};
+                cur.pa = po;
                 break;
             }
             case cfd::Step::Out: {
@@ -1698,6 +1737,106 @@
     });
 }
 
+extern "C" int cfd_conv_gn_probe(const float* x, const float* w1_host, const float* b1_host, const float* w2_host,
+                                 const float* b2_host, const float* gamma, const float* beta, float* y1, float* y2,
+                                 float* out, float* ss, int B, int H, int W, int Cin, int C1, int C2, int plan_b,
+                                 int flags, int device, int* info, void* stream) {
+    return cfd::guard([&] {
+        CFD_REQUIRE(x && w1_host && b1_host && gamma && beta && y1 && out && ss && info, CFD_EARG, "null argument");
+        CFD_REQUIRE(C2 == 0 || (w2_host && b2_host && y2), CFD_EARG, "null argument (second convolution)");
+        CFD_REQUIRE(B > 0 && H > 0 && W > 0 && Cin > 0 && Cin % 32 == 0 && C1 > 0 && C1 % 4 == 0 && C2 >= 0 &&
+                        C2 % 4 == 0 && (C1 + C2) % 32 == 0 && C1 + C2 <= 1024 && plan_b >= 0 && plan_b <= 64,
+                    CFD_ESHAPE, "conv + GroupNorm probe: Cin % 32 == 0, C1 % 4 == C2 % 4 == 0, (C1 + C2) % 32 == 0");
+        cfd::DeviceGuard dg(device);
+        hipStream_t st = (hipStream_t)stream;
+        struct Bufs {
+            std::vector<void*> p;
+            ~Bufs() { for (void* q : p) (void)hipFree(q); }
+            void* dev(size_t bytes, const void* src = nullptr) {
+                void* q = nullptr;
+                CFD_HIP(hipMalloc(&q, std::max<size_t>(bytes, 16)));
+                p.push_back(q);
+                if (src) CFD_HIP(hipMemcpy(q, src, bytes, hipMemcpyHostToDevice));
+                return q;
+            }
+        } d;
+        const int pb = plan_b > 0 ? plan_b : 8, HW = H * W;
+        cfd::GnArgs g{};
+        auto run_conv = [&](const float* w_host, const float* bias_host, int Cout, float* y, int k) -> const double* {
+            const size_t n = (size_t)Cout * Cin * 9;
+            std::vector<float> pk(n);
+            for (int64_t o = 0; o < Cout; ++o)
+                for (int64_t i = 0; i < Cin; ++i)
+                    for (int tap = 0; tap < 9; ++tap) pk[(o * 9 + tap) * Cin + i] = w_host[(o * Cin + i) * 9 + tap];
+            float amax = 0.f;
+            for (float v : pk) amax = std::max(amax, std::fabs(v));
+            int ex = 0;
+            if (amax > 0.f) std::frexp(amax, &ex);
+            const float s = std::ldexp(1.0f, -ex);
+            std::vector<_Float16> hi(n), lo(n);
+            for (size_t e = 0; e < n; ++e) {
+                const float v = pk[e] * s;
+                hi[e] = (_Float16)v;
+                lo[e] = (_Float16)(v - (float)hi[e]);
+            }
+            cfd::ConvArgs a{};
+            a.src1 = x;
+            a.C1 = a.Ctot = Cin;
+            a.w = (const float*)d.dev(n * 4, pk.data());
+            a.wbf = d.dev(n * 2, hi.data());
+            a.wlo = d.dev(n * 2, lo.data());
+            a.acc_scale = std::ldexp(1.0f, ex);
+            a.bias = (const float*)d.dev((size_t)Cout * 4, bias_host);
+            a.out = y;
+            a.Hin = a.Hout = H;
+            a.Win = a.Wout = W;
+            a.stride = 1;
+            a.ks = 3;
+            a.pad = 1;
+            a.Cout = Cout;
+            a.M = B * HW;
+            a.K = 9 * Cin;
+            a.plan_b = pb;
+            double* part = nullptr;
+            if (cfd::gn_partials_wanted(HW, Cout, pb))
+                part = (double*)d.dev(sizeof(double) * 2 * (size_t)B * (HW / 256) * (Cout / 4));
+            a.gnp = flags & 2 ? nullptr : part;
+            cfd::ConvPlan plan = cfd::plan_conv(a, kSplitPer8);
+            if (flags & 1) plan.splits = 1;
+            if (a.gnp && !cfd::conv_emits_gn_partials(a, plan)) a.gnp = nullptr;
+            if (plan.splits > 1) a.part = (float*)d.dev(sizeof(float) * plan.splits * (size_t)a.M * Cout);
+            info[4 * k + 0] = plan.kx;
+            info[4 * k + 1] = plan.splits;
+            info[4 * k + 2] = a.gnp ? 1 : 0;
+            info[4 * k + 3] = plan.bn;
+            cfd::launch_conv(a, plan, st);
+            return a.gnp;
+        };
+        g.p1 = run_conv(w1_host, b1_host, C1, y1, 0);
+        for (int k = 4; k < 8; ++k) info[k] = 0;
+        if (C2) g.p2 = run_conv(w2_host, b2_host, C2, y2, 1);
+        g.src1 = y1;
+        g.src2 = C2 ? y2 : nullptr;
+        g.gamma = (const float*)d.dev((size_t)(C1 + C2) * 4, gamma);
+        g.beta = (const float*)d.dev((size_t)(C1 + C2) * 4, beta);
+        g.part = (double*)d.dev(sizeof(double) * (size_t)B * cfd::kGnMaxChunks * 32 * 2);
+        g.ss = ss;
+        g.out = out;
+        g.C1 = C1;
+        g.C2 = C2;
+        g.Ctot = C1 + C2;
+        g.HW = HW;
+        g.eps = 1e-5f;
+        g.silu = flags & 4 ? 0 : 1;
+        g.plan_b = pb;
+        g.nt1 = g.nt2 = HW / 256;
+        info[8] = cfd::gn2_applies(g) ? 1 : 0;
+        info[9] = cfd::gn2_applies(g) && !cfd::gn_takes_partials(g) ? 1 : 0;
+        cfd::launch_gn(g, B, st);
+        CFD_HIP(hipStreamSynchronize(st));
+    });
+}
+
 extern "C" int cfd_unet_set_compute(cfd_unet* h, int compute) {
     return cfd::guard([&] {
         CFD_REQUIRE(h, CFD_EARG, "null handle");
diff --git a/confild_amd/csrc/unet_kernels.hip b/confild_amd/csrc/unet_kernels.hip
--- a/confild_amd/csrc/unet_kernels.hip
+++ b/confild_amd/csrc/unet_kernels.hip
@@ -442,10 +442,30 @@
         constexpr int GL = NT / 32;
         const int grp = threadIdx.x / GL, sub = threadIdx.x % GL;
         double S = 0, S2 = 0;
-        for (int k = sub; k < NC; k += GL) {
-            const double2 v = *(const double2*)(a.part + ((b * NC + k) * 32 + grp) * 2);
-            S += v.x;
-            S2 += v.y;
+        if (a.p1) {
+            const int g0 = grp * cpg, g1 = g0 + cpg;
+            const int n1q = max(0, min(g1, a.C1) - g0) >> 2, n2q = (cpg >> 2) - n1q;
+            const int q1 = g0 >> 2, q2 = (max(g0, a.C1) - a.C1) >> 2;
+            const int it1 = a.nt1 * n1q, items = it1 + a.nt2 * n2q;
+            for (int e = sub; e < items; e += GL) {
+                const double2* src;
+                if (e < it1) {
+                    const int tl = e / n1q;
+                    src = (const double2*)a.p1 + (b * a.nt1 + tl) * (a.C1 >> 2) + q1 + (e - tl * n1q);
+                } else {
+                    const int e2 = e - it1, tl = e2 / n2q;
+                    src = (const double2*)a.p2 + (b * a.nt2 + tl) * (a.C2 >> 2) + q2 + (e2 - tl * n2q);
+                }
+                const double2 v = *src;
+                S += v.x;
+                S2 += v.y;
+            }
+        } else {
+            for (int k = sub; k < NC; k += GL) {
+                const double2 v = *(const double2*)(a.part + ((b * NC + k) * 32 + grp) * 2);
+                S += v.x;
+                S2 += v.y;
+            }
         }
 #pragma unroll
         for (int o = 1; o < GL; o <<= 1) {
@@ -1565,6 +1585,29 @@
     return a.Ctot % 128 == 0 ? (int)ceil_div(a.HW, 512 / (a.Ctot / 128)) : 0;
 }
 
+bool gn_partials_wanted(int HW, int C, int plan_b) {
+#ifdef CFD_NO_GN_EPI
+    (void)HW, (void)C, (void)plan_b;
+    return false;
+#else
+    GnArgs g{};
+    g.HW = HW;
+    g.C1 = g.Ctot = C;
+    g.plan_b = plan_b;
+    return C % 4 == 0 && HW % 256 == 0 && HW <= kGn2BigHW && gn2_applies(g);
+#endif
+}
+
+bool gn_takes_partials(const GnArgs& a) {
+#ifdef CFD_NO_GN_EPI
+    (void)a;
+    return false;
+#else
+    return gn2_applies(a) && !a.kpart && a.p1 && a.nt1 * 256 == a.HW && (!a.src2 || (a.p2 && a.nt2 * 256 == a.HW)) &&
+           a.Ctot % 128 == 0;
+#endif
+}
+
 bool gn_takes_splitk(const GnArgs& a, int B) {
     (void)B;
     if (gn2_applies(a)) return a.C1 % 4 == 0;
@@ -1584,18 +1627,25 @@
     if (gn2_applies(a)) {
         CFD_REQUIRE(!a.kpart || a.kx, CFD_ESTATE, "internal: gn2 needs the split-K sum's destination");
         a.nchunks = gn2_chunks(a.HW, a.plan_b);
+        const bool epi = gn_takes_partials(a);
+        if (!epi) a.p1 = a.p2 = nullptr;
         if (gn2_threads(a.nchunks) == 1024) {
-            hipLaunchKernelGGL(gn2_stats_kernel<1024>, dim3(a.nchunks, B), dim3(1024), 0, st, a);
-            check_launch("gn2_stats_kernel");
+            if (!epi) {
+                hipLaunchKernelGGL(gn2_stats_kernel<1024>, dim3(a.nchunks, B), dim3(1024), 0, st, a);
+                check_launch("gn2_stats_kernel");
+            }
             hipLaunchKernelGGL(gn2_apply_kernel<1024>, dim3(a.nchunks, B), dim3(1024), 0, st, a);
         } else {
-            hipLaunchKernelGGL(gn2_stats_kernel<256>, dim3(a.nchunks, B), dim3(256), 0, st, a);
-            check_launch("gn2_stats_kernel");
+            if (!epi) {
+                hipLaunchKernelGGL(gn2_stats_kernel<256>, dim3(a.nchunks, B), dim3(256), 0, st, a);
+                check_launch("gn2_stats_kernel");
+            }
             hipLaunchKernelGGL(gn2_apply_kernel<256>, dim3(a.nchunks, B), dim3(256), 0, st, a);
         }
         check_launch("gn2_apply_kernel");
         return;
     }
+    a.p1 = a.p2 = nullptr;
     const int ipt = gn_reg_ipt(a);
     if (ipt > 0 && ipt <= 32) {
         const dim3 grid((unsigned)(32 * B));
@@ -1723,6 +1773,12 @@
             q.bn = 128;
             q.nw = 8;
             q.splits = halo_splits(ceil_div(mn, 256) * ceil_div(a.Cout, 128));
+#ifdef CFD_GN_EPI_UNSPLIT
+            if (a.gnp && q.splits == 2 && a.Cout % 64 == 0 && ceil_div(mn, 256) * (a.Cout / 64) >= 256) {
+                q.splits = 1;
+                q.bn = 64;
+            }
+#endif
             return q;
         }
         q.kx = mn >= 2048 ? 2 : 1;
@@ -1802,6 +1858,16 @@
     static const int ldsepi = env_int("CFD_CONV_LDSEPI", 1);
     return ldsepi && (p.kx < 0 || p.kx >= 40) && p.splits == 1 && a.wbf && !a.tmode && a.ks == 1 && a.bias &&
            !a.emb && !a.res && a.Cout % 8 == 0 && a.emb_stride % 4 == 0 && T % 32 == 0 && a.M % T == 0;
+}
+
+bool conv_emits_gn_partials(const ConvArgs& a, const ConvPlan& p) {
+#ifdef CFD_NO_GN_EPI
+    (void)a, (void)p;
+    return false;
+#else
+    return (p.kx == 20 || p.kx == 22 || p.kx == 24) && p.splits == 1 && !p.adjoint && !conv_x_falls_back(a) &&
+           a.Cout % 4 == 0 && a.emb_stride % 4 == 0 && (int64_t)a.Hout * a.Wout % 256 == 0;
+#endif
 }
 
 int launch_conv(const ConvArgs& a, const ConvPlan& p0, hipStream_t st, bool defer) {
@@ -1826,6 +1892,9 @@
     b.stamps = g_stamps;
     b.seq = g_seq++;
     b.ldsepi = ldsepi && a.Cout % 4 == 0 && a.emb_stride % 4 == 0;
+    CFD_REQUIRE(!a.gnp || conv_emits_gn_partials(a, p), CFD_ESTATE,
+                "internal: statistics partials asked of a launch that cannot write them");
+    if (a.gnp) b.ldsepi = 1;
     const int xo = xcd == 4 ? (a.wbf && !a.wlo ? 1 : 3) : xcd;
     b.xcd = xo == 3 ? ((int64_t)a.Hout * a.Wout <= 256 ? 2 : 1) : xo < 0 || xo > 2 ? 1 : xo;
     {
@@ -1841,7 +1910,7 @@
         return 1;
     }
     if (p.kx >= 0) {
-        launch_conv_x(a_, p.kx, p.splits, st, p.adjoint);
+        launch_conv_x(a_, p.kx, p.splits, st, p.adjoint, p.bn);
         if (p.splits > 1 && !defer) launch_splitk_reduce(a, p.splits, st);
         return p.splits;
     }
diff --git a/confild_amd/csrc/unet_kernels.hpp b/confild_amd/csrc/unet_kernels.hpp
--- a/confild_amd/csrc/unet_kernels.hpp
+++ b/confild_amd/csrc/unet_kernels.hpp
@@ -32,6 +32,9 @@
     int out_bf16;
     unsigned* amax_out;
     int plan_b;
+    const double* p1;
+    const double* p2;
+    int nt1, nt2;
 };
 
 struct ConvArgs {
@@ -68,6 +71,7 @@
     unsigned long long* stamps;
     int seq;
     int plan_b;
+    double* gnp;
 };
 constexpr int kPhaseMinCout = 128;
 
@@ -176,6 +180,9 @@
 void launch_gn(const GnArgs& a, int B, hipStream_t st);
 bool gn_takes_splitk(const GnArgs& a, int B);
 bool gn2_applies(const GnArgs& a);
+bool gn_takes_partials(const GnArgs& a);
+bool gn_partials_wanted(int HW, int C, int plan_b);
+bool conv_emits_gn_partials(const ConvArgs& a, const ConvPlan& p);
 ConvPlan plan_conv(const ConvArgs& a, size_t part_cap_floats);
 int launch_conv(const ConvArgs& a, const ConvPlan& p, hipStream_t st, bool defer = false);
 void launch_splitk_reduce(const ConvArgs& a, int splits, hipStream_t st);
@@ -198,7 +205,7 @@
         bx = Lp / (gz * gy);
     }
 }
-int launch_conv_x(const ConvArgs& a, int variant, int splits, hipStream_t st, bool adjoint = false);
+int launch_conv_x(const ConvArgs& a, int variant, int splits, hipStream_t st, bool adjoint = false, int bn = 0);
 int conv_h_tw(const ConvArgs& a);
 int conv_hp_tw(const ConvArgs& a);
 int k1h_shape(int tw, int bn, bool phase, bool adjoint);
diff --git a/include/confild.h b/include/confild.h
--- a/include/confild.h
+++ b/include/confild.h
@@ -48,6 +48,10 @@
 int  cfd_unet_check_finite(cfd_unet* h, int* nonfinite, void* stream);
 int  cfd_upsample_conv(const float* x, const float* w_host, const float* bias_host, float* out, int B, int H,
                        int W, int Cin, int Cout, int plan_b, int device, int* kx, void* stream);
+int  cfd_conv_gn_probe(const float* x, const float* w1_host, const float* b1_host, const float* w2_host,
+                       const float* b2_host, const float* gamma, const float* beta, float* y1, float* y2, float* out,
+                       float* ss, int B, int H, int W, int Cin, int C1, int C2, int plan_b, int flags, int device,
+                       int* info, void* stream);
 
 int  cfd_unet_tape_bytes(const cfd_unet* h, int B, size_t* bytes);
 int  cfd_unet_vjp_workspace_bytes(const cfd_unet* h, int B, size_t* bytes);
```

Measured after the change: 4.225. About the same (-0.9%).
